# facebookresearch/videoseal

Hardware: AMD Instinct MI355X
Metric: frames/sec embed+extract 256-bit @768x768 (higher is better)
Workload: dtype f32 (2 x f16 operand split, 3 products on v_mfma_f32_32x32x16_f16, fp32 accumulate); 1 GPU; videoseal_1.0 256-bit, 32 frames 768x768 per GPU, image mode (embedder on every frame, full-res JND), embed + detect; card=videoseal_1.0, weights=random-init (seeded), no checkpoint offline, batch_per_gpu=32, mode=image

## Files before the change

### include/videoseal_hip.h

```cpp
#ifndef VIDEOSEAL_HIP_H
#define VIDEOSEAL_HIP_H

#include <stdint.h>

#ifdef __cplusplus
extern "C" {
#endif

#define VS_OK 0
#define VS_ERR_BAD_ARG (-1)
#define VS_ERR_UNSUPPORTED (-2)
#define VS_ERR_LAUNCH (-3)

#define VS_ACT_NONE 0
#define VS_ACT_RELU 1
#define VS_ACT_GELU 2
#define VS_ACT_TANH 3
#define VS_ACT_SILU 4

#define VS_PAD_ZERO 0
#define VS_PAD_REFLECT 1

#define VS_VIDEO_REPEAT 0
#define VS_VIDEO_ALTERNATE 1
// ... 112 lines not shown
int vs_vit_attention_bwd(const float* qkv, const float* out, const float* dout, int frames, int H, int W, int heads, int hd, int window,
                         const float* rel_h, const float* rel_w, float* dqkv, float* scratch, float* drel_h, float* drel_w, void* stream);
int vs_reflect_fold1(const float* dxp, int B, int H, int W, int64_t ld, float* out, void* stream);
int vs_dwconv7(const float* x, int B, int H, int W, int C, int64_t ld, const float* w, const float* bias, int flip, const float* add,
               int64_t add_ld, float* out, int64_t out_ld, void* stream);
int64_t vs_dwconv7_wgrad_partial_floats(int B, int H, int64_t ld);
int vs_dwconv7_wgrad(const float* x, int64_t ld, const float* dy, int64_t dy_ld, int B, int H, int W, int C, float* partial, float* dw,
                     void* stream);
int64_t vs_colreduce_partial_floats(int B, int64_t HW, int64_t ld);
int vs_layernorm_bwd(const float* x, int64_t ld, const float* dy, int64_t dy_ld, const float* w, int64_t rows, int C, float eps, float* dx,
                     int64_t dx_ld, float* stats, float* partial, float* dw, float* db, void* stream);
int vs_gelu_grn_bwd(const float* h1, int64_t ld, const float* d3, int64_t d3_ld, const float* gamma, int B, int HW, int C, float* partial,
                    float* coef, float* dh1, int64_t dh1_ld, float* dgamma, float* dbeta, void* stream);
int vs_patchify(const float* x, int B, int H, int W, int64_t pld, int P, float* cols, void* stream);
int vs_unpatch(const float* dcols, int B, int H, int W, int64_t pld, int P, float* dx, void* stream);
int vs_patchify_s(const float* x, int B, int H, int W, int64_t pld, int P, int S, float* cols, void* stream);
int vs_unpatch_s(const float* dcols, int B, int H, int W, int64_t pld, int P, int S, float* dx, void* stream);
int vs_col2im3x3_reflect(const float* dcols, int B, int H, int W, int64_t ld, float* dx, void* stream);
int vs_colmean(const float* x, int B, int HW, int64_t ld, float* out, void* stream);
int vs_pool_gelu_bwd(const float* z, int64_t ld, const float* dpooled, int64_t dp_ld, int B, int HW, int C, float* dz, int64_t dz_ld,
                     void* stream);
int vs_matmul_small(const float* A, int64_t lda, const float* Bm, int64_t ldb, int M, int N, int K, float* C, int64_t ldc, void* stream);
int vs_bce_logits(const float* preds, const int32_t* msgs, int msg_rows, int B, int k, float temperature, float gscale, float* dpreds,
                  float* loss, void* stream);

int vs_bn_mean_rstd(const double* sums, int C, int64_t ld, float eps, float* mean, float* rstd, void* stream);
int64_t vs_bn_bwd_partial_floats(int64_t rows, int64_t ld);
int vs_bn_relu_bwd_sums(const float* raw, int64_t ld, const float* dy, int64_t dy_ld, const float* mean, const float* rstd, const float* scale,
                        const float* shift, int relu, int64_t rows, int C, float* partial, double* sums, float* dgamma, float* dbeta,
                        void* stream);
int vs_bn_relu_bwd_apply(const float* raw, int64_t ld, const float* dy, int64_t dy_ld, const float* mean, const float* rstd, const float* scale,
                         const float* shift, int relu, const double* sums, int64_t rows, int C, float* dx, int64_t dx_ld, void* stream);
int vs_dilate2(const float* dy, int B, int Ho, int Wo, int64_t ld, int H, int W, float* out, void* stream);
int vs_im2col3x3_strided(const float* x, int B, int H, int W, int64_t ld, int stride, float* cols, void* stream);
int vs_upcat2x_bwd(const float* dhi, int64_t hi_ld, int B, int H, int W, int C1, int C2, float skip_scale, float* dx, int64_t ld1,
                   float* dskip, int64_t ld2, void* stream);
int vs_msg_table_grad(const float* dlat, const int32_t* msgs, int Bm, int nbits, int hidden, float* dtable, void* stream);
int vs_relu_bwd(const float* z, int64_t ld, const float* dy, int64_t dy_ld, int64_t rows, int C, float* dz, int64_t dz_ld, void* stream);
int vs_outc_tanh_bwd(const float* delta, const float* ddelta, int64_t rows_per_frame, int B, int C, const float* w, int Cout, int use_tanh,
                     float* dx, int64_t dx_ld, float* dv, void* stream);

typedef struct vs_resblock_thin_desc {
  const float* x; int64_t x_ld;
  int32_t B, H, W, Cin;
  const void *w0_split, *w1_split, *wr_split;
  const float *b0, *b1, *br;
  int32_t arith;
  int32_t Cout;
  float a_mul, acc_mul0, acc_mul1, acc_mulr;
  float* out; int64_t out_ld;
} vs_resblock_thin_desc_t;
int vs_resblock_thin_supported(int cin_ld, int cmid, int cout);
int vs_resblock_thin(const vs_resblock_thin_desc_t* d, void* stream);

int vs_check_finite(const float* x, int64_t n, int* flag, void* stream);

int vs_absmax(const float* x, int64_t n, unsigned* bits, void* stream);

int vs_cnx_block_supported(int C, int64_t rows, int HW);
int64_t vs_cnx_block_image_bytes(int C);
int vs_cnx_block(const void* tn_planes, const void* wimg, int C, int64_t rows, int HW, int stats, float acc_mul1, float acc_mul2, const float* scale,
                 int64_t scale_ld, const float* bias2, const float* res, int64_t res_ld, float* out, int64_t out_ld, float* part32, void* stream);

int vs_split_block(const float* wt, int N, int64_t K, int ntaps, int arith, float w_mul, void* split, void* blk, void* stream);
int vs_pack_conv(const float* w, int Co, int Ci, int KH, int KW, int cinp, int transpose, float* out, void* stream);

int vs_resize_nchw_bwd(const float* dy, float* dx, int planes, int H, int W, int oh, int ow, int antialias, float* tmp, void* stream);
int vs_embed_tail_bwd(const float* imgs, const float* preds, const float* hmap_full, const float* d_imgs_w, const float* d_preds_w, int F, int H, int W,
                      int Cd, int clamp, float scaling_i, float scaling_w, float* g_full, void* stream);
int vs_tail_key_reduce(const float* g_low, const float* hmap_low, int F, int Cd, int S_h, int S_w, int step, int video_mode, int total_key,
                       float* d_delta, void* stream);
int vs_aug_crop_flip_bwd(const float* dy, float* dx, int planes, int H, int W, int i0, int j0, int h, int w, int flip, void* stream);
int vs_mask_mul(const float* dy, const float* mask, float* dx, int F, int C, int H, int W, int complement, void* stream);
int64_t vs_aug_color_bwd_scratch_floats(int F, int H, int W);
int vs_aug_color_bwd(const float* x, const float* dy, float* dx, int F, int H, int W, int op, float factor, const float* means, float* scratch,
                     void* stream);
int vs_clamp01_bwd(const float* x, const float* dy, float* dx, int64_t n, void* stream);
int vs_aug_gather_frames_bwd(const float* dy, const int32_t* start, const int32_t* outs, float* dx, int n_src, int64_t frame_floats, void* stream);
int vs_aug_window_average_bwd(const float* dy, float* dx, int F, int64_t frame_floats, int half_window, float alpha, void* stream);
int vs_gaussian_blur_bwd(const float* dy, float* tmp, float* dx, int planes, int H, int W, int k, float sigma, void* stream);
int vs_aug_warp_bwd(const float* dy, float* dx, int planes, int H, int W, int oh, int ow, int kind, const float* coeffs, int bilinear,
                    const float* inv, void* stream);
int vs_nhwc_to_nchw_scaled(const float* src, int F, int H, int W, int C, int64_t ld, float mul, float* dst, void* stream);
int64_t vs_percep_partial_doubles(int F, int H, int W);
int vs_percep_mse(const float* imgs, const float* imgs_w, int F, int H, int W, int yuv, double* partial, float* loss, void* stream);
int vs_percep_mse_grad(const float* imgs, const float* imgs_w, int F, int H, int W, int yuv, float upstream, float* d_imgs_w, void* stream);

int64_t vs_ssim_partial_doubles(int P, int H, int W);
int vs_ssim_stats(const float* x, const float* y, int P, int H, int W, float data_range, const float* win11, double* partial, double* out, void* stream);
int vs_ssim_grad(const float* x, const float* y, const float* g_ssim, const float* g_cs, const float* g_coarse, int P, int H, int W, float data_range,
                 const float* win11, float* dy, void* stream);
int vs_avgpool2_pad(const float* x, const float* y, int P, int H, int W, float* xo, float* yo, void* stream);
int64_t vs_jnd_loss_partial_doubles(int F, int H, int W);
int vs_jnd_loss(const float* imgs, const float* imgs_w, const float* hmap, int F, int H, int W, double* partial, float* loss, void* stream);
int vs_jnd_loss_grad(const float* imgs, const float* imgs_w, const float* hmap, int F, int H, int W, float upstream, float* d_imgs_w, void* stream);

int vs_upcat2x(const float* x, int C1, int64_t ld1, const float* skip, int C2, int64_t ld2, float skip_scale,
               int B, int H, int W, float* out, int64_t out_ld, void* stream);

int vs_upconv_supported(int Co);
int vs_upconv_gather_ln(const float* z, int64_t z_ld, int B, int H, int W, int Co, const float* lnw, const float* lnb, float eps,
                        int act, float* out, int64_t out_ld, void* stream);
int vs_cat2_scale(const float* x, int C1, int64_t ld1, const float* skip, int C2, int64_t ld2, float skip_scale, int64_t rows,
                  float* out, int64_t out_ld, void* stream);

int vs_upconv_fused_supported(int C1, int C2, int Co);
// ... 92 lines not shown
```

### videoseal_amd/csrc/model_api.hip

```cpp
#include <algorithm>
#include <cmath>
#include <cstring>
#include <map>
#include <string>
#include <vector>

#include "vs_common.h"

#pragma clang fp contract(off)

namespace {

inline int rup(int v, int m) { return (v + m - 1) / m * m; }

struct HostT { const float* p; int64_t n; };

struct CW {
  float* wt = nullptr; float* bias = nullptr; void* split = nullptr; void* blk = nullptr;
  int N = 0, KH = 0, KW = 0, CinP = 0;
  float w_mul = 1.f;
};
struct RB { CW c0, c1, res; int cout = 0; };
struct Up { CW conv; CW gemm; bool lowres = false; float* lnw = nullptr; float* lnb = nullptr; RB rb; };
struct Down { float* lnw = nullptr; float* lnb = nullptr; CW conv, gemm; };
// ... 297 lines not shown
    const float am = a_mul_override > 0.f ? a_mul_override : ((a_scale && !pre_table) ? A_MUL_GRN : A_MUL);
    d.arith = m->arith; d.a_mul = am; d.acc_mul = 1.f / (am * w.w_mul);
    if (in2) { d.wt2_split = w2->split; d.wt2_blk = w2->blk; d.acc_mul2 = 1.f / (am * w2->w_mul); }
    int split_k = 1;
    const bool dense_rows = d.in_sy == (int64_t)d.W * d.in_sx && d.in_sb == (int64_t)d.H * d.in_sy;
    const bool gemm_pc = d.KH == 1 && d.KW == 1 && sh == 1 && sw == 1 && ph == 0 && pw == 0 && !in2 && d.Ho == d.H && d.Wo == d.W &&
                         d.Cin % 32 == 0 && d.CinP == d.Cin && dense_rows && (!a_scale || d.H * d.W >= 128 || d.H * d.W == 64);
    const bool patch_pc = d.KH == 3 && d.KW == 3 && sh == 1 && sw == 1 && ph == 1 && pw == 1 && d.Ho == d.H && d.Wo == d.W && !a_scale &&
                          d.W % 16 == 0 && d.H % 8 == 0;
    if (pre_table) {
      d.tile_hint = (d.N % 192 == 0 ? (VS_CONV_TILE_HI | 0) : 15) | VS_CONV_PRE;
    } else if (sumsq) {
      d.sumsq_part = sumsq;
    } else if (gemm_pc && a_scale && m->arith == 2 && d.N % 96 == 0 && d.H * d.W >= 128 && d.CinP <= 3072 &&
               (((int64_t)d.B * d.H * d.W + 127) / 128) * ((d.N + 127) / 128) < 256 && (((int64_t)d.B * d.H * d.W + 127) / 128) * ((d.N + 95) / 96) >= 200) {
      d.tile_hint = VS_CONV_TILE_HI | 10;
    } else if (gemm_pc) {
      const int64_t rows = (int64_t)d.B * d.H * d.W;
      const int64_t blocks = ((rows + 127) / 128) * ((d.N + 127) / 128);
      const int pairs = d.CinP / 32;
      int sk = 1;
      while (blocks * sk < 256 && pairs % (sk * 2) == 0 && pairs / (sk * 2) >= 4) sk *= 2;
      if (!a_scale || d.CinP / sk <= 3072) split_k = sk;
    } else if (patch_pc && d.N >= 128 && d.CinP >= 128) {
      const int64_t blocks = (int64_t)d.B * (d.H / 8) * (d.W / 16) * (d.N % 192 == 0 ? (d.N + 191) / 192 : (d.N + 127) / 128);
      const int spt = d.CinP / 16;
      const int cands[5] = {2, 3, 4, 6, 8};
      for (int cand : cands) {
        if (blocks * split_k >= 192) break;
        if (spt % cand == 0 && spt / cand >= 2) split_k = cand;
      }
    }
    if (split_k > 1) {
      const int ws_ld = rup(w.N, 4);
      const int slices = split_k + ((patch_pc && in2) ? 1 : 0);
      d.splitk_ws = alloc((int64_t)slices * out.rows() * ws_ld);
      d.splitk_ld = ws_ld;
      d.split_k = split_k;
      d.tile_hint = d.KH == 3 ? (d.N % 192 == 0 ? VS_CONV_TILE_HI | 0 : 15) : (VS_CONV_TILE_HI | (d.N % 192 == 0 ? 2 : 1));
    }
    if (grn_part) {
      const int t = (d.tile_hint & 0xf) + ((d.tile_hint & VS_CONV_TILE_HI) ? 16 : 0);
      if ((t == 17 || t == 18 || t == 26) && grn_hw % 32 == 0 && grn_hw / 32 <= 16 && d.CinP == grn_c4 && a_scale_ld == grn_c4) {
        d.grn_part = grn_part; d.grn_gamma = grn_gamma; d.grn_nchunk = grn_hw / 32;
      } else if (live()) {
        chk(vs_grn_scale_from_partials(grn_part, d.B, grn_hw, grn_c4, grn_gamma, const_cast<float*>(a_scale), a_scale_ld, st));
      }
    }
    if (live()) chk(vs_conv_gemm(&d, st));
  }
  void layernorm(const Act& x, const float* w, const float* b, const Act& out, int act_ = VS_ACT_NONE) {
    if (live()) chk(vs_layernorm_act(x.p, x.rows(), x.C, x.ld, w, b, 1e-6f, act_, out.p, out.ld, st));
  }
  Act resblock(const Act& x, const RB& p, const Act* out_in = nullptr) {
    const int tk = p.cout == 16 ? 16 : 32;
    if ((p.cout == 16 || (p.cout == 32 && m->arith == 2)) && x.ld <= tk && p.c0.CinP == tk && p.c1.CinP == tk && p.res.CinP == tk &&
        (!out_in || out_in->ld == p.cout) && vs_resblock_thin_supported(x.ld, p.cout, p.cout)) {
      Act out = out_in ? *out_in : act(x.B, x.H, x.W, p.cout);
      vs_resblock_thin_desc_t d;
      std::memset(&d, 0, sizeof(d));
      d.x = x.p; d.x_ld = x.ld; d.B = x.B; d.H = x.H; d.W = x.W; d.Cin = x.ld;
      d.w0_split = p.c0.split; d.w1_split = p.c1.split; d.wr_split = p.res.split;
      d.b0 = p.c0.bias; d.b1 = p.c1.bias; d.br = p.res.bias;
      d.arith = m->arith; d.Cout = p.cout; d.a_mul = A_MUL;
      d.acc_mul0 = 1.f / (A_MUL * p.c0.w_mul); d.acc_mul1 = 1.f / (A_MUL * p.c1.w_mul); d.acc_mulr = 1.f / (A_MUL * p.res.w_mul);
      d.out = out.p; d.out_ld = out.ld;
      if (live()) chk(vs_resblock_thin(&d, st));
      return out;
    }
    Act t = act(x.B, x.H, x.W, p.cout);
    conv(x, p.c0, t, 1, 1, VS_PAD_ZERO, VS_ACT_RELU);
    Act out = out_in ? *out_in : act(x.B, x.H, x.W, p.cout);
    conv(t, p.c1, out, 1, 1, VS_PAD_ZERO, VS_ACT_RELU, 0, out.ld != rup(p.cout, 4) ? p.cout : -1, nullptr, &x, &p.res);
    return out;
  }
  void gemm_pl(int B, int H, int W, const CW& w, const void* in_pl, const Act& out, int act_, const Act* res, float* sumsq, int split_k,
               float am = A_MUL, int sumsq_hw = 0) {
    vs_conv_desc_t d;
    std::memset(&d, 0, sizeof(d));
    d.B = B; d.H = H; d.W = W; d.Cin = w.CinP; d.KH = d.KW = 1; d.SH = d.SW = 1; d.Ho = H; d.Wo = W;
    d.wt = w.wt; d.CinP = w.CinP; d.N = w.N; d.bias = w.bias; d.act = act_;
    d.wt_split = w.split; d.wt_blk = w.blk; d.arith = 2; d.a_mul = am; d.acc_mul = 1.f / (am * w.w_mul);
    d.in_pl = in_pl;
    d.out = out.p; d.out_ld = out.ld; d.n_store = out.ld;
    if (res) { d.res = res->p; d.res_ld = res->ld; }
    d.sumsq_part = sumsq;
    d.sumsq_hw = sumsq_hw;
    if (split_k > 1) {
      const int ws_ld = rup(w.N, 4);
      d.splitk_ws = alloc((int64_t)split_k * out.rows() * ws_ld);
      d.splitk_ld = ws_ld;
      d.split_k = split_k;
    }
    d.tile_hint = VS_CONV_TILE_HI | 8;
    if (live()) chk(vs_conv_gemm(&d, st));
  }
  void conv_pl(int B, int H, int W, const CW& w, const void* in_pl, void* out_pl, const Act* out, const CW* w2 = nullptr,
               const void* in2_pl = nullptr, const float* pre_table = nullptr, int64_t pre_ld = 0) {
    vs_conv_desc_t d;
    std::memset(&d, 0, sizeof(d));
    d.B = B; d.H = H; d.W = W; d.Cin = w.CinP; d.KH = d.KW = 3; d.SH = d.SW = 1; d.PH = d.PW = 1; d.pad_mode = VS_PAD_ZERO; d.Ho = H; d.Wo = W;
    d.wt = w.wt; d.CinP = w.CinP; d.N = w.N; d.bias = w.bias; d.act = VS_ACT_RELU;
    d.wt_split = w.split; d.wt_blk = w.blk; d.arith = 2; d.a_mul = A_MUL; d.acc_mul = 1.f / (A_MUL * w.w_mul);
    d.in_pl = in_pl; d.out_pl = out_pl;
    if (w2) {
      d.in2_pl = in2_pl; d.Cin2 = d.Cin2P = w2->CinP; d.wt2 = w2->wt; d.bias2 = w2->bias; d.wt2_split = w2->split; d.wt2_blk = w2->blk;
      d.acc_mul2 = 1.f / (A_MUL * w2->w_mul);
    }
    d.n_store = w.N;
    if (out) { d.out = out->p; d.out_ld = out->ld; d.n_store = out->ld != rup(w.N, 4) ? w.N : out->ld; }
    d.tile_hint = VS_CONV_TILE_HI | 6;
    if (pre_table) { d.a_scale = pre_table; d.a_scale_ld = pre_ld; d.tile_hint |= VS_CONV_PRE; }
    if (live()) chk(vs_conv_gemm(&d, st));
  }
  Act bottleneck_planes(const Act& x, int j0, const Act* last_out, void* xpl_in = nullptr) {
    const int B = x.B, H = x.H, W = x.W, C = x.C;
    const int64_t pl_floats = x.rows() * C;
    void* xpl = xpl_in ? xpl_in : alloc(pl_floats);
// ... 81 lines not shown
            chk(vs_to_planes(h3.p, h3.rows(), h3.C, h3.ld, A_MUL, h3pl, st));
          }
          conv_pl(B, h3.H, h3.W, m->b0_lat, latpl, tpl, nullptr, nullptr, nullptr, table, n_msgs == 1 ? 0 : 9 * (int64_t)N);
          conv_pl(B, h3.H, h3.W, rb.c1, tpl, xpl, nullptr, &rb.res, h3pl);
          cur = nxt;
          cur_pl = xpl;
          continue;
        }
        Act t = act(B, h3.H, h3.W, N);
        conv(h3, m->b0_lat, t, 1, 1, VS_PAD_ZERO, VS_ACT_RELU, 0, -1, nullptr, nullptr, nullptr, table, n_msgs == 1 ? 0 : 9 * (int64_t)N, nullptr,
             nullptr, nullptr, m->zc.back(), true);
        Act out = act(B, h3.H, h3.W, N);
        conv(t, rb.c1, out, 1, 1, VS_PAD_ZERO, VS_ACT_RELU, 0, -1, nullptr, &h3, &rb.res);
        cur = out;
        continue;
      }
      if (j >= 1 && planes_ok(cur, j)) {
        Act v2 = view;
        const bool d2 = j == c.num_blocks - 1 ? direct : lowres_cat(0, cur, v2);
        cur = bottleneck_planes(cur, j, d2 ? &v2 : nullptr, cur_pl);
        break;
      }
      cur = resblock(cur, rb, direct ? &view : nullptr);
    }
    for (int k = 0; k < nlev; ++k) {
      const Act skip = hid.back();
      hid.pop_back();
      const Up& up = m->ups[k];
      Act ln{};
      if (up.lowres && cur.ld == cur.C && fused_ok(k, cur.C, skip.C)) {
        const int co = up.gemm.N / 9;
        ln = act(B, 2 * cur.H, 2 * cur.W, co);
        if (live()) chk(vs_upconv_fused(cur.p, cur.C, cur.ld, skip.p, skip.C, skip.ld, 0.70710678118654752440f, up.gemm.split, B, cur.H, cur.W, co,
                                        up.lnw, up.lnb, 1e-6f, VS_ACT_RELU, ln.p, ln.ld, m->arith, A_MUL, 1.f / (A_MUL * up.gemm.w_mul), st));
      } else if (up.lowres) {
        const int co = up.gemm.N / 9;
        const bool direct = cur.ld == cur.C + skip.C;
        Act lc = direct ? Act{cur.p, B, cur.H, cur.W, cur.C + skip.C, cur.ld} : act(B, cur.H, cur.W, cur.C + skip.C);
        if (live()) chk(vs_cat2_scale(direct ? nullptr : cur.p, cur.C, cur.ld, skip.p, skip.C, skip.ld, 0.70710678118654752440f, lc.rows(), lc.p, lc.ld, st));
        Act z = act(B, lc.H, lc.W, 9 * co);
        conv(lc, up.gemm, z);
        ln = act(B, 2 * lc.H, 2 * lc.W, co);
        if (live()) chk(vs_upconv_gather_ln(z.p, z.ld, B, lc.H, lc.W, co, up.lnw, up.lnb, 1e-6f, VS_ACT_RELU, ln.p, ln.ld, st));
      } else {
        Act cat = act(B, 2 * cur.H, 2 * cur.W, cur.C + skip.C);
        if (live()) chk(vs_upcat2x(cur.p, cur.C, cur.ld, skip.p, skip.C, skip.ld, 0.70710678118654752440f, B, cur.H, cur.W, cat.p, cat.ld, st));
        Act cv = act(B, cat.H, cat.W, up.conv.N);
        conv(cat, up.conv, cv, 1, 1, VS_PAD_REFLECT);
        ln = act(B, cat.H, cat.W, up.conv.N);
        layernorm(cv, up.lnw, up.lnb, ln, VS_ACT_RELU);
      }
      Act view{};
      const bool direct = lowres_cat(k + 1, Act{nullptr, B, ln.H, ln.W, up.rb.cout, 0}, view);
      cur = resblock(ln, up.rb, direct ? &view : nullptr);
    }
    float* delta = alloc((int64_t)B * c.out_ch * cur.H * cur.W);
    if (live()) chk(vs_outc_tanh(cur.p, (int64_t)cur.H * cur.W, B, cur.C, cur.ld, m->outc_w, m->outc_b, c.out_ch, c.last_tanh ? 1 : 0, delta, st));
    Sh = cur.H; Sw = cur.W;
    return delta;
  }
  void extractor(const Act& x, float* logits) {
    const vs_model_cfg_t& c = m->c;
    const int B = x.B, s = c.stem_stride;
    int Ho = (x.H - 4) / s + 1, Wo = (x.W - 4) / s + 1;
    Act cur = act(B, Ho, Wo, c.dims[0], xld(c.dims[0]));
    const int co = c.dims[0];
    static const bool stem_fused = [] { const char* e = getenv("VIDEOSEAL_STEM_FUSED"); return e && e[0] == '1'; }();
    if (stem_fused && x.ld == 4 && cur.ld == co && (co == 64 || co == 96 || co == 128) && m->stem.bias) {
      if (live()) chk(vs_stem_conv_ln(x.p, B, x.H, x.W, s, m->stem.wt, m->stem.bias, m->stem_lnw, m->stem_lnb, 1e-6f, co, cur.p, cur.ld, st));
    } else {
      Act t = act(B, Ho, Wo, c.dims[0]);
      { const int geom[7] = {Wo, s * 4, 16, s, 1, 0, 0}; conv(x, m->stem, t, 1, 0, VS_PAD_ZERO, VS_ACT_NONE, 0, -1, nullptr, nullptr, nullptr, nullptr, 0, nullptr, geom); }
      layernorm(t, m->stem_lnw, m->stem_lnb, cur);
    }
    for (int sti = 0; sti < 4; ++sti) {
      if (sti > 0) {
        const Down& dn = m->down[sti - 1];
        Ho = cur.H / 2; Wo = cur.W / 2;
        if (cur.ld == cur.C && cur.C % 8 == 0 && dn.gemm.CinP == 4 * cur.C && Ho > 0 && Wo > 0) {
          Act lnp = act(B, Ho, Wo, 4 * cur.C, 4 * cur.C);
          Act nxt = act(B, Ho, Wo, c.dims[sti], xld(c.dims[sti]));
          if (live()) chk(vs_layernorm_patch2x2(cur.p, B, cur.H, cur.W, cur.C, cur.ld, dn.lnw, dn.lnb, 1e-6f, lnp.p, st));
          conv(lnp, dn.gemm, nxt);
          cur = nxt;
        } else {
          Act ln = act(B, cur.H, cur.W, cur.C, cur.ld);
          layernorm(cur, dn.lnw, dn.lnb, ln);
          Act nxt = act(B, Ho, Wo, c.dims[sti], xld(c.dims[sti]));
          const int geom[7] = {Wo, 2 * ln.ld, 2 * ln.ld, 2, 1, 0, 0};
          conv(ln, dn.conv, nxt, 1, 0, VS_PAD_ZERO, VS_ACT_NONE, 0, -1, nullptr, nullptr, nullptr, nullptr, 0, nullptr, geom);
          cur = nxt;
        }
      }
      const int Cc = c.dims[sti], HW = cur.H * cur.W;
      Act tn = act(B, cur.H, cur.W, Cc, xld(Cc));
      Act hh = act(B, cur.H, cur.W, 4 * Cc, xld(4 * Cc));
      float* part = alloc((int64_t)((HW + 63) / 64) * B * 4 * Cc);
      float* part32 = alloc((int64_t)B * ((HW + 31) / 32) * 4 * Cc);
      float* scale = alloc((int64_t)B * hh.ld + 16);
      float* parts = (HW % 32 != 0 && HW >= 32) ? alloc((((int64_t)B * HW + 31) / 32) * 2 * 4 * Cc) : nullptr;
      const int64_t rows = cur.rows();
      const CW& pw1w = m->stages[sti].empty() ? m->stem : m->stages[sti][0].pw1;
      const bool pl1 = m->arith == 2 && ((rows + 255) / 256) * ((4 * Cc + 191) / 192) >= 200 && pw1w.CinP % 16 == 0 && !m->stages[sti].empty();
      bool pl2 = false;
      int sk2 = 1;
      if (m->arith == 2 && hh.ld >= 2048 && hh.ld % 16 == 0) {
// ... 258 lines not shown
```

### videoseal_amd/csrc/net_ops.hip

```cpp
#include <algorithm>
#include <cstdlib>
#include <cstring>

#include "conv_common.h"

namespace {

__global__ __launch_bounds__(256) void layernorm_act_kernel(const float* __restrict__ x, int64_t rows, int C, int64_t ld,
                                                            const float* __restrict__ w, const float* __restrict__ b,
                                                            float eps, int act, float* __restrict__ out, int64_t out_ld) {
  const int lane = threadIdx.x & 63;
  const int64_t row = (int64_t)blockIdx.x * 4 + (threadIdx.x >> 6);
  if (row >= rows) return;
  const float* xr = x + row * ld;
  float s = 0.f;
  for (int c = lane; c < C; c += 64) s += xr[c];
  const float mean = wave_sum(s) / (float)C;
  float v = 0.f;
  for (int c = lane; c < C; c += 64) {
    const float dlt = xr[c] - mean;
    v += dlt * dlt;
  }
  const float var = wave_sum(v) / (float)C;
  const float den = sqrtf(var + eps);
  float* orow = out + row * out_ld;
  for (int c = lane; c < (int)out_ld; c += 64) {
    float y = 0.f;
    if (c < C) y = vs_apply_act(w[c] * ((xr[c] - mean) / den) + b[c], act);
    orow[c] = y;
  }
}

template <int LPP, int VMAX>
__global__ __launch_bounds__(256) void layernorm_act_lanes_kernel(const float* __restrict__ x, int64_t rows, int C, int64_t ld,
                                                                  const float* __restrict__ w, const float* __restrict__ b, float eps, int act,
                                                                  float* __restrict__ out, int64_t out_ld, int pH, int pW) {
  constexpr int RPB = 256 / LPP;
  const int q = threadIdx.x & (LPP - 1);
  const int64_t row = (int64_t)blockIdx.x * RPB + (threadIdx.x / LPP);
  bool live = row < rows;
  const int C4 = (C + 3) >> 2, O4 = (int)(out_ld >> 2);
  const float* xr = x + (live ? row : rows - 1) * ld;
  f32x4 v[VMAX];
  float s = 0.f;
#pragma unroll
  for (int k = 0; k < VMAX; ++k) {
    const int c4 = q + k * LPP;
    v[k] = f32x4{0.f, 0.f, 0.f, 0.f};
    if (c4 < C4) {
      v[k] = *reinterpret_cast<const f32x4*>(xr + 4 * c4);
#pragma unroll
      for (int e = 0; e < 4; ++e)
        if (4 * c4 + e < C) s += v[k][e];
    }
  }
#pragma unroll
  for (int o = LPP / 2; o > 0; o >>= 1) s += __shfl_xor(s, o, 64);
// ... 484 lines not shown
          scale[(int64_t)b * sld + c] = gx;
          local += gx;
        }
      }
    }
    __syncthreads();
  }
  if (kg == 0) red[cl] = local;
  __syncthreads();
  for (int o = 128; o > 0; o >>= 1) {
    if (threadIdx.x < o) red[threadIdx.x] += red[threadIdx.x + o];
    __syncthreads();
  }
  const float mean = red[0] / (float)C;
  for (int c = threadIdx.x; c < (int)sld; c += 1024) {
    float v = 0.f;
    if (c < C) v = 1.0f + gamma[c] * (scale[(int64_t)b * sld + c] / (mean + 1e-6f));
    scale[(int64_t)b * sld + c] = v;
  }
}

__global__ __launch_bounds__(256) void upcat2x_kernel(const float* __restrict__ x, int C1, int64_t ld1,
                                                      const float* __restrict__ skip, int C2, int64_t ld2, float sscale,
                                                      int B, int H, int W, float* __restrict__ out, int64_t old, int64_t total) {
  const int G = (int)(old >> 2);
  for (int64_t i = (int64_t)blockIdx.x * 256 + threadIdx.x; i < total; i += (int64_t)gridDim.x * 256) {
    const int cg = (int)(i % G);
    int64_t p = i / G;
    const int X = (int)(p % (2 * W)); p /= (2 * W);
    const int Y = (int)(p % (2 * H));
    const int b = (int)(p / (2 * H));
    const int c = cg * 4;
    float sy = fmaxf((Y + 0.5f) * 0.5f - 0.5f, 0.f), sx = fmaxf((X + 0.5f) * 0.5f - 0.5f, 0.f);
    const int y0 = (int)sy, x0 = (int)sx;
    const int y1 = y0 + (y0 < H - 1), x1 = x0 + (x0 < W - 1);
    const float ly1 = sy - y0, lx1 = sx - x0, ly0 = 1.f - ly1, lx0 = 1.f - lx1;
    const float* src; int64_t ld; int cc; float mul;
    if (c < C1) { src = x; ld = ld1; cc = c; mul = 1.f; }
    else { src = skip; ld = ld2; cc = c - C1; mul = sscale; }
    f32x4 v = {0.f, 0.f, 0.f, 0.f};
    if (c < C1 + C2) {
      const float* fb = src + (int64_t)b * H * W * ld + cc;
      const f32x4 p00 = *reinterpret_cast<const f32x4*>(fb + ((int64_t)y0 * W + x0) * ld);
      const f32x4 p01 = *reinterpret_cast<const f32x4*>(fb + ((int64_t)y0 * W + x1) * ld);
      const f32x4 p10 = *reinterpret_cast<const f32x4*>(fb + ((int64_t)y1 * W + x0) * ld);
      const f32x4 p11 = *reinterpret_cast<const f32x4*>(fb + ((int64_t)y1 * W + x1) * ld);
      v = (ly0 * (lx0 * (p00 * mul) + lx1 * (p01 * mul)) + ly1 * (lx0 * (p10 * mul) + lx1 * (p11 * mul)));
    }
    *reinterpret_cast<f32x4*>(out + (((int64_t)b * 2 * H + Y) * 2 * W + X) * old + c) = v;
  }
}

template <int CG>
__global__ __launch_bounds__(256) void upconv_gather_ln_kernel(const float* __restrict__ z, int64_t zld, int H, int W, int Co,
                                                               int tpp_log2, const float* __restrict__ lnw,
                                                               const float* __restrict__ lnb, float eps, int act,
                                                               float* __restrict__ out, int64_t old, int64_t npix, int nblk) {
  const int per = (nblk + 7) >> 3;
  const int64_t vb = (int64_t)(blockIdx.x & 7) * per + (blockIdx.x >> 3);
  const int64_t gid = vb * 256 + threadIdx.x;
  const int64_t pq = gid >> tpp_log2;
  const int g = (int)(gid & ((1 << tpp_log2) - 1));
  const bool live = pq < npix && vb < nblk;
  const int64_t p = live ? pq : 0;
  constexpr int NVP = CG / 4;
  f32x4 lwv[NVP], lbv[NVP];
#pragma unroll
  for (int j = 0; j < NVP; ++j) {
    lwv[j] = *reinterpret_cast<const f32x4*>(lnw + g * CG + 4 * j);
    lbv[j] = *reinterpret_cast<const f32x4*>(lnb + g * CG + 4 * j);
  }
  const int W2 = 2 * W, H2 = 2 * H;
  const int X = (int)(p % W2);
  const int64_t t0 = p / W2;
  const int Y = (int)(t0 % H2);
  const int64_t b = t0 / H2;
  int ys[3][2], xs[3][2];
  float wy[3][2], wx[3][2];
#pragma unroll
  for (int k = 0; k < 3; ++k) {
    int yr = Y + k - 1, xr = X + k - 1;
    yr = yr < 0 ? -yr : (yr >= H2 ? 2 * H2 - 2 - yr : yr);
    xr = xr < 0 ? -xr : (xr >= W2 ? 2 * W2 - 2 - xr : xr);
    const float sy = fmaxf((yr + 0.5f) * 0.5f - 0.5f, 0.f), sx = fmaxf((xr + 0.5f) * 0.5f - 0.5f, 0.f);
    const int y0 = (int)sy, x0 = (int)sx;
    ys[k][0] = y0; ys[k][1] = y0 + (y0 < H - 1);
    xs[k][0] = x0; xs[k][1] = x0 + (x0 < W - 1);
    wy[k][1] = sy - y0; wy[k][0] = 1.f - wy[k][1];
    wx[k][1] = sx - x0; wx[k][0] = 1.f - wx[k][1];
  }
  constexpr int NV = CG / 4;
  f32x4 acc[NV];
#pragma unroll
  for (int j = 0; j < NV; ++j) acc[j] = f32x4{0.f, 0.f, 0.f, 0.f};
  const float* zb = z + b * H * W * zld + g * CG;
#pragma unroll
  for (int ky = 0; ky < 3; ++ky)
#pragma unroll
    for (int a = 0; a < 2; ++a) {
      const float* zr = zb + (int64_t)ys[ky][a] * W * zld + ky * 3 * Co;
#pragma unroll
      for (int kx = 0; kx < 3; ++kx)
#pragma unroll
        for (int c = 0; c < 2; ++c) {
          const float w = wy[ky][a] * wx[kx][c];
          const float* q = zr + (int64_t)xs[kx][c] * zld + kx * Co;
#pragma unroll
          for (int j = 0; j < NV; ++j) acc[j] += w * *reinterpret_cast<const f32x4*>(q + 4 * j);
        }
    }
  float s = 0.f;
#pragma unroll
  for (int j = 0; j < NV; ++j) s += (acc[j][0] + acc[j][1]) + (acc[j][2] + acc[j][3]);
  for (int o = 1; o < (1 << tpp_log2); o <<= 1) s += __shfl_xor(s, o, 64);
  const float mean = s / (float)Co;
  float v = 0.f;
#pragma unroll
  for (int j = 0; j < NV; ++j)
#pragma unroll
    for (int e = 0; e < 4; ++e) { const float dl = acc[j][e] - mean; v += dl * dl; }
  for (int o = 1; o < (1 << tpp_log2); o <<= 1) v += __shfl_xor(v, o, 64);
  const float den = sqrtf(v / (float)Co + eps);
  if (!live) return;
  float* orow = out + p * old + g * CG;
#pragma unroll
  for (int j = 0; j < NV; ++j) {
    const f32x4 wv = lwv[j], bv = lbv[j];
    f32x4 o;
#pragma unroll
    for (int e = 0; e < 4; ++e) o[e] = vs_apply_act(wv[e] * ((acc[j][e] - mean) / den) + bv[e], act);
    *reinterpret_cast<f32x4*>(orow + 4 * j) = o;
  }
}

__global__ __launch_bounds__(256) void im2col3x3_kernel(const float* __restrict__ x, int H, int W, int64_t ld, int reflect,
                                                        float* __restrict__ out, int64_t total) {
  const int G = (int)(ld >> 2);
  for (int64_t i = (int64_t)blockIdx.x * 256 + threadIdx.x; i < total; i += (int64_t)gridDim.x * 256) {
    const int cg = (int)(i % G);
    int64_t r = i / G;
    const int t = (int)(r % 9);
    r /= 9;
    const int xx = (int)(r % W);
    const int yy = (int)((r / W) % H);
    const int64_t b = r / ((int64_t)W * H);
    int sy = yy + t / 3 - 1, sx = xx + t % 3 - 1;
    bool ok = true;
    if (reflect) {
      sy = sy < 0 ? -sy : (sy >= H ? 2 * H - 2 - sy : sy);
      sx = sx < 0 ? -sx : (sx >= W ? 2 * W - 2 - sx : sx);
    } else {
      ok = sy >= 0 && sy < H && sx >= 0 && sx < W;
    }
    f32x4 v = {0.f, 0.f, 0.f, 0.f};
    if (ok) v = *reinterpret_cast<const f32x4*>(x + ((b * H + sy) * W + sx) * ld + cg * 4);
    *reinterpret_cast<f32x4*>(out + (r * 9 + t) * ld + cg * 4) = v;
  }
}

__global__ __launch_bounds__(256) void msg_pre_kernel(const float* __restrict__ P, int N, float* __restrict__ T, int64_t total) {
  for (int64_t i = (int64_t)blockIdx.x * 256 + threadIdx.x; i < total; i += (int64_t)gridDim.x * 256) {
    const int n = (int)(i % N);
    const int cls = (int)((i / N) % 9);
    const int64_t bm = i / ((int64_t)9 * N);
    const int cy = cls / 3, cx = cls % 3;
    const float* pb = P + bm * 9 * N + n;
    float v = 0.f;
    for (int ky = (cy == 0 ? 1 : 0); ky <= (cy == 2 ? 1 : 2); ++ky)
      for (int kx = (cx == 0 ? 1 : 0); kx <= (cx == 2 ? 1 : 2); ++kx) v += pb[(ky * 3 + kx) * N];
    T[i] = v;
  }
}

__global__ __launch_bounds__(256) void cat2_scale_kernel(const float* __restrict__ x, int C1, int64_t ld1, const float* __restrict__ skip,
                                                         int C2, int64_t ld2, float s, int64_t rows, float* __restrict__ out,
                                                         int64_t old) {
  const int g1 = x ? C1 >> 2 : 0, G = g1 + (C2 >> 2);
  const int64_t total = rows * G;
  for (int64_t i = (int64_t)blockIdx.x * 256 + threadIdx.x; i < total; i += (int64_t)gridDim.x * 256) {
    const int cg = (int)(i % G);
    const int64_t r = i / G;
    f32x4 v;
    int c;
    if (cg < g1) { c = cg * 4; v = *reinterpret_cast<const f32x4*>(x + r * ld1 + c); }
    else { const int c2 = (cg - g1) * 4; c = C1 + c2; v = *reinterpret_cast<const f32x4*>(skip + r * ld2 + c2) * s; }
// ... 1 lines not shown
  }
}

__global__ __launch_bounds__(256) void msg_latent_kernel(const float* __restrict__ table, const int32_t* __restrict__ msgs,
                                                         int nbits, int hidden, float* __restrict__ lat) {
  __shared__ int rowsel[1024];
  const int b = blockIdx.y;
  for (int k = threadIdx.x; k < nbits; k += 256) rowsel[k] = 2 * k + (msgs[(int64_t)b * nbits + k] != 0);
  __syncthreads();
  const int c = blockIdx.x * 256 + threadIdx.x;
  if (c >= hidden) return;
  float s = 0.f;
  int k = 0;
  for (; k + 16 <= nbits; k += 16) {
    float v[16];
#pragma unroll
    for (int j = 0; j < 16; ++j) v[j] = table[(int64_t)rowsel[k + j] * hidden + c];
#pragma unroll
    for (int j = 0; j < 16; ++j) s += v[j];
  }
  for (; k < nbits; ++k) s += table[(int64_t)rowsel[k] * hidden + c];
  lat[(int64_t)b * hidden + c] = s;
}
__global__ __launch_bounds__(256) void broadcast_channels4_kernel(const float* __restrict__ lat, int Bm, int hidden4,
                                                                  float* __restrict__ dst, int HW, int64_t ld, int coff,
                                                                  int64_t total4) {
  for (int64_t i = (int64_t)blockIdx.x * 256 + threadIdx.x; i < total4; i += (int64_t)gridDim.x * 256) {
    const int c4 = (int)(i % hidden4);
    const int64_t p = i / hidden4;
    const int b = (int)(p / HW);
    *reinterpret_cast<f32x4*>(dst + p * ld + coff + 4 * c4) = *reinterpret_cast<const f32x4*>(lat + ((int64_t)(Bm == 1 ? 0 : b) * hidden4 + c4) * 4);
  }
}
__global__ __launch_bounds__(256) void broadcast_channels_kernel(const float* __restrict__ lat, int Bm, int hidden,
                                                                 float* __restrict__ dst, int HW, int64_t ld, int coff,
                                                                 int64_t total) {
  for (int64_t i = (int64_t)blockIdx.x * 256 + threadIdx.x; i < total; i += (int64_t)gridDim.x * 256) {
    const int c = (int)(i % hidden);
    const int64_t p = i / hidden;
    const int b = (int)(p / HW);
    dst[p * ld + coff + c] = lat[(int64_t)(Bm == 1 ? 0 : b) * hidden + c];
  }
}

__global__ __launch_bounds__(256) void outc_tanh_kernel(const float* __restrict__ x, int64_t rpf, int64_t rows, int C,
                                                        int64_t ld, const float* __restrict__ w, const float* __restrict__ bias,
                                                        int Cout, int use_tanh, float* __restrict__ out) {
  const int64_t row = (int64_t)blockIdx.x * 256 + threadIdx.x;
  if (row >= rows) return;
  float acc[4] = {0.f, 0.f, 0.f, 0.f};
  const float* xr = x + row * ld;
  for (int c = 0; c < C; c += 4) {
    const f32x4 v = *reinterpret_cast<const f32x4*>(xr + c);
    for (int o = 0; o < Cout; ++o) {
      const float* wr = w + (int64_t)o * C + c;
      acc[o] += v[0] * wr[0];
      if (c + 1 < C) acc[o] += v[1] * wr[1];
      if (c + 2 < C) acc[o] += v[2] * wr[2];
      if (c + 3 < C) acc[o] += v[3] * wr[3];
    }
  }
  const int64_t b = row / rpf, p = row - b * rpf;
  for (int o = 0; o < Cout; ++o) {
    float v = acc[o] + bias[o];
    out[(b * Cout + o) * rpf + p] = use_tanh ? tanhf(v) : v;
  }
}

__global__ __launch_bounds__(256) void pool_linear_kernel(const float* __restrict__ x, int HW, int C, int64_t ld,
                                                          const float* __restrict__ w, const float* __restrict__ bias, int N,
                                                          float* __restrict__ out) {
  extern __shared__ float pooled[];
  const int b = blockIdx.x;
  const float* xb = x + (int64_t)b * HW * ld;
  const int C4 = (C + 3) >> 2;
  const bool vec = (ld & 3) == 0 && (reinterpret_cast<uintptr_t>(x) & 15) == 0;
  if (vec) {
    for (int g = threadIdx.x; g < C4; g += 256) {
      f32x4 s = {0.f, 0.f, 0.f, 0.f};
      const float* xg = xb + 4 * g;
      int r = 0;
      for (; r + 16 <= HW; r += 16) {
        f32x4 v[16];
#pragma unroll
        for (int q = 0; q < 16; ++q) v[q] = *reinterpret_cast<const f32x4*>(xg + (int64_t)(r + q) * ld);
#pragma unroll
        for (int q = 0; q < 16; ++q) s += v[q];
      }
      for (; r < HW; ++r) s += *reinterpret_cast<const f32x4*>(xg + (int64_t)r * ld);
#pragma unroll
      for (int e = 0; e < 4; ++e)
        if (4 * g + e < C) pooled[4 * g + e] = s[e] / (float)HW;
    }
  } else {
    for (int c = threadIdx.x; c < C; c += 256) {
      float s = 0.f;
      for (int r = 0; r < HW; ++r) s += xb[(int64_t)r * ld + c];
      pooled[c] = s / (float)HW;
    }
  }
  __syncthreads();
  const int lane = threadIdx.x & 63, wv = threadIdx.x >> 6;
  constexpr int CM = 16;
  for (int n = blockIdx.y * 4 + wv; n < N; n += 4 * gridDim.y) {
    const float* wr = w + (int64_t)n * C;
    float s = 0.f;
    if (C <= 64 * CM) {
      float wv_[CM];
#pragma unroll
      for (int j = 0; j < CM; ++j) {
        const int c = lane + 64 * j;
        wv_[j] = c < C ? wr[c] : 0.f;
      }
#pragma unroll
      for (int j = 0; j < CM; ++j) {
        const int c = lane + 64 * j;
        if (c < C) s += pooled[c] * wv_[j];
      }
    } else {
// ... 454 lines not shown
  return vs_launch_status();
}

extern "C" int vs_upcat2x(const float* x, int C1, int64_t ld1, const float* skip, int C2, int64_t ld2, float skip_scale,
                          int B, int H, int W, float* out, int64_t out_ld, void* stream) {
  VS_REQUIRE(x && skip && out && C1 > 0 && C2 > 0 && C1 % 4 == 0 && C2 % 4 == 0 && ld1 % 4 == 0 && ld2 % 4 == 0);
  VS_REQUIRE(out_ld % 4 == 0 && out_ld >= C1 + C2 && B > 0 && H > 0 && W > 0);
  const int64_t total = (int64_t)B * 2 * H * 2 * W * (out_ld / 4);
  hipLaunchKernelGGL(upcat2x_kernel, dim3(grid_for(total, 256, 1 << 20)), dim3(256), 0, (hipStream_t)stream, x, C1, ld1, skip,
                     C2, ld2, skip_scale, B, H, W, out, out_ld, total);
  return vs_launch_status();
}

extern "C" int vs_cat2_scale(const float* x, int C1, int64_t ld1, const float* skip, int C2, int64_t ld2, float skip_scale,
                             int64_t rows, float* out, int64_t out_ld, void* stream) {
  VS_REQUIRE(skip && out && rows > 0 && C1 >= 0 && C2 > 0 && C1 % 4 == 0 && C2 % 4 == 0 && ld2 % 4 == 0 && out_ld % 4 == 0 &&
             out_ld >= C1 + C2 && (!x || (ld1 % 4 == 0 && ld1 >= C1)));
  const int64_t total = rows * ((x ? C1 : 0) + C2) / 4;
  hipLaunchKernelGGL(cat2_scale_kernel, dim3((unsigned)std::min<int64_t>(cdiv64(total, 256), 1 << 16)), dim3(256), 0, (hipStream_t)stream,
                     x, C1, ld1, skip, C2, ld2, skip_scale, rows, out, out_ld);
  return vs_launch_status();
}

extern "C" int vs_im2col3x3(const float* x, int B, int H, int W, int64_t ld, int pad_mode, float* out, void* stream) {
  VS_REQUIRE(x && out && B > 0 && H > 1 && W > 1 && ld > 0 && ld % 4 == 0);
  const int64_t total = (int64_t)B * H * W * 9 * (ld / 4);
  hipLaunchKernelGGL(im2col3x3_kernel, dim3((unsigned)std::min<int64_t>(cdiv64(total, 256), 1 << 16)), dim3(256), 0, (hipStream_t)stream, x, H,
                     W, ld, pad_mode == VS_PAD_REFLECT ? 1 : 0, out, total);
  return vs_launch_status();
}

extern "C" int vs_msg_pre(const float* P, int Bm, int N, float* table, void* stream) {
  VS_REQUIRE(P && table && Bm > 0 && N > 0);
  const int64_t total = (int64_t)Bm * 9 * N;
  hipLaunchKernelGGL(msg_pre_kernel, dim3((unsigned)std::min<int64_t>(cdiv64(total, 256), 1 << 16)), dim3(256), 0, (hipStream_t)stream, P, N, table,
                     total);
  return vs_launch_status();
}

extern "C" int vs_upconv_supported(int Co) {
  if (Co < 16 || Co % 16) return 0;
  const int cg = Co >= 64 ? 16 : Co / 4;
  const int tpp = Co / cg;
  return (cg == 4 || cg == 8 || cg == 16) && tpp <= 64 && (tpp & (tpp - 1)) == 0;
}

extern "C" int vs_upconv_gather_ln(const float* z, int64_t z_ld, int B, int H, int W, int Co, const float* lnw, const float* lnb,
                                   float eps, int act, float* out, int64_t out_ld, void* stream) {
  VS_REQUIRE(z && lnw && lnb && out && B > 0 && H > 0 && W > 0 && vs_upconv_supported(Co) && z_ld >= 9 * (int64_t)Co && z_ld % 4 == 0 &&
             out_ld >= Co && out_ld % 4 == 0);
  const int cg = Co >= 64 ? 16 : Co / 4;
  int tl = 0;
  while ((cg << tl) < Co) ++tl;
  const int64_t npix = (int64_t)B * 4 * H * W;
  const int64_t nblk64 = cdiv64(npix << tl, 256);
  VS_REQUIRE(nblk64 < (1 << 30));
  const int nblk = (int)nblk64;
  const int grid = ((nblk + 7) / 8) * 8;
  hipStream_t st = (hipStream_t)stream;
#define VS_UPG(CG_) hipLaunchKernelGGL(upconv_gather_ln_kernel<CG_>, dim3(grid), dim3(256), 0, st, z, z_ld, H, W, Co, tl, lnw, lnb, eps, act, out, out_ld, npix, nblk)
  if (cg == 4) VS_UPG(4);
  else if (cg == 8) VS_UPG(8);
  else VS_UPG(16);
#undef VS_UPG
  return vs_launch_status();
}

extern "C" int vs_msg_latent(const float* table, const int32_t* msgs, int Bm, int nbits, int hidden, float* lat, void* stream) {
  VS_REQUIRE(table && msgs && lat && Bm > 0 && nbits > 0 && nbits <= 1024 && hidden > 0);
  hipLaunchKernelGGL(msg_latent_kernel, dim3((unsigned)((hidden + 255) / 256), (unsigned)Bm), dim3(256), 0, (hipStream_t)stream,
                     table, msgs, nbits, hidden, lat);
  return vs_launch_status();
}

extern "C" int vs_broadcast_channels(const float* lat, int Bm, int hidden, float* dst, int B, int HW, int64_t ld, int coff,
                                     void* stream) {
  VS_REQUIRE(lat && dst && (Bm == 1 || Bm == B) && hidden > 0 && B > 0 && HW > 0 && coff >= 0 && coff + hidden <= ld);
  const int64_t total = (int64_t)B * HW * hidden;
  if ((hidden & 3) == 0 && (ld & 3) == 0 && (coff & 3) == 0 && (((uintptr_t)lat | (uintptr_t)dst) & 15) == 0) {
    hipLaunchKernelGGL(broadcast_channels4_kernel, dim3(grid_for(total / 4, 256, 1 << 20)), dim3(256), 0, (hipStream_t)stream, lat, Bm,
                       hidden / 4, dst, HW, ld, coff, total / 4);
    return vs_launch_status();
  }
  hipLaunchKernelGGL(broadcast_channels_kernel, dim3(grid_for(total, 256, 1 << 20)), dim3(256), 0, (hipStream_t)stream, lat, Bm,
                     hidden, dst, HW, ld, coff, total);
  return vs_launch_status();
}

extern "C" int vs_outc_tanh(const float* x, int64_t rows_per_frame, int B, int C, int64_t ld, const float* w, const float* bias,
                            int Cout, int use_tanh, float* out, void* stream) {
  VS_REQUIRE(x && w && bias && out && rows_per_frame > 0 && B > 0 && C > 0 && ld % 4 == 0 && ld >= C && Cout > 0 && Cout <= 4);
  const int64_t rows = rows_per_frame * B;
  hipLaunchKernelGGL(outc_tanh_kernel, dim3((unsigned)cdiv64(rows, 256)), dim3(256), 0, (hipStream_t)stream, x, rows_per_frame,
                     rows, C, ld, w, bias, Cout, use_tanh, out);
  return vs_launch_status();
}

extern "C" int vs_pool_linear(const float* x, int B, int HW, int C, int64_t ld, const float* w, const float* bias, int N,
                              float* out, void* stream) {
  VS_REQUIRE(x && w && bias && out && B > 0 && HW > 0 && C > 0 && ld >= C && N > 0);
  const size_t smem = (size_t)C * sizeof(float);
  if (smem > 64 * 1024) return VS_ERR_UNSUPPORTED;
  hipLaunchKernelGGL(pool_linear_kernel, dim3((unsigned)B, 16), dim3(256), smem, (hipStream_t)stream, x, HW, C, ld, w, bias, N, out);
  return vs_launch_status();
}

extern "C" int64_t vs_bn_partial_doubles(int64_t rows, int64_t ld) { return ld >= 4 ? cdiv64(rows, bn_chunk_rows(ld)) * 2 * ld : 0; }

extern "C" int vs_bn_batch_stats(const float* x, int64_t rows, int C, int64_t ld, const float* gamma, const float* beta, float eps,
                                 float momentum, float* running_mean, float* running_var, double* partial, float* scale, float* shift,
                                 void* stream) {
  VS_REQUIRE(x && gamma && beta && partial && scale && shift && rows > 0 && C > 0 && ld >= C && (ld & 3) == 0);
// ... 50 lines not shown
```

### videoseal_amd/csrc/resblock_thin.hip

```cpp
#include "conv_common.h"

namespace {

using namespace vsconv;

constexpr int TH = 8, TW = 16;
constexpr int T_W = TW + 2, T_H = TH + 2, T_PX = T_W * T_H;
constexpr int X_W = TW + 4, X_H = TH + 4, X_PX = X_W * X_H;
constexpr int XITEMS = X_PX * 4;
constexpr int NXI = (XITEMS + 255) / 256;
constexpr int G0_PER_WAVE = 3;
constexpr int G1_PER_WAVE = 2;
constexpr int ROWB16 = 32;

template <int NP> struct Arith16;
template <> struct Arith16<3> {
  static __device__ __forceinline__ f32x4 mfma(const bf16x8& a, const bf16x8& b, const f32x4& c) {
    return __builtin_amdgcn_mfma_f32_16x16x32_bf16(a, b, c, 0, 0, 0);
  }
};
template <> struct Arith16<2> {
  static __device__ __forceinline__ f32x4 mfma(const bf16x8& a, const bf16x8& b, const f32x4& c) {
    return __builtin_amdgcn_mfma_f32_16x16x32_f16(__builtin_bit_cast(f16x8, a), __builtin_bit_cast(f16x8, b), c, 0, 0, 0);
  }
};

struct RbArgs {
  const float* x; int64_t x_sb, x_sy, x_sx; int B, H, W, Cin;
  const void *w0, *w1, *wr;
  const float *b0, *b1, *br;
  float a_mul, acc_mul0, acc_mul1, acc_mulr;
  float* out; int64_t out_ld;
};

__device__ __forceinline__ bf16x8 zero_frag() {
  const u32x4 z = {0u, 0u, 0u, 0u};
  return __builtin_bit_cast(bf16x8, z);
}

template <int NP, int NBUF, int OCC>
__global__ __launch_bounds__(256, OCC) void resblock_thin_kernel(const RbArgs d, const int tiles_x, const int tiles_y, const int ntiles_total,
                                                                 const int tiles_per_wg) {
  using AR = Arith<NP>;
  using A16 = Arith16<NP>;
  constexpr int XP_BYTES = NP * X_PX * ROWB16;
  constexpr int TT_BYTES = NP * T_PX * ROWB16;
  __shared__ __attribute__((aligned(16))) unsigned char smem[NBUF * XP_BYTES + TT_BYTES];
  unsigned char* const Tt = smem + NBUF * XP_BYTES;
  const int tid = threadIdx.x;
  const int lane = tid & 63;
  const int wave = tid >> 6;
  const int n = lane & 15, kb = lane >> 4;
  const int hi = kb >> 1;
  const int kh = (kb & 1) * 8;

  bf16x8 w0f[5][NP], w1f[5][NP], wrf[NP];
#pragma unroll
  for (int s = 0; s < 5; ++s) {
    const int tap = 2 * s + hi;
#pragma unroll
    for (int p = 0; p < NP; ++p) {
      if (tap < 9) {
        w0f[s][p] = *reinterpret_cast<const bf16x8*>(static_cast<const char*>(d.w0) + ((int64_t)p * 16 * 144 + n * 144 + tap * 16 + kh) * 2);
        w1f[s][p] = *reinterpret_cast<const bf16x8*>(static_cast<const char*>(d.w1) + ((int64_t)p * 16 * 144 + n * 144 + tap * 16 + kh) * 2);
      } else {
        w0f[s][p] = zero_frag();
        w1f[s][p] = zero_frag();
      }
    }
  }
#pragma unroll
  for (int p = 0; p < NP; ++p)
    wrf[p] = hi == 0 ? *reinterpret_cast<const bf16x8*>(static_cast<const char*>(d.wr) + ((int64_t)p * 16 * 16 + n * 16 + kh) * 2) : zero_frag();
  float b0v[4], b1v[4], brv[4];
#pragma unroll
  for (int e = 0; e < 4; ++e) {
    b0v[e] = d.b0 ? d.b0[4 * kb + e] : 0.f;
    b1v[e] = d.b1 ? d.b1[4 * kb + e] : 0.f;
    brv[e] = d.br ? d.br[4 * kb + e] : 0.f;
  }

  int p_dy[NXI], p_dx[NXI], p_lds[NXI];
  bool p_have[NXI];
  const int k4 = (tid & 3) * 4;
  const bool cok = k4 < d.Cin;
#pragma unroll
  for (int i = 0; i < NXI; ++i) {
    const int item = tid + i * 256;
    p_have[i] = item < XITEMS;
    const int prow = p_have[i] ? item >> 2 : 0;
    p_dy[i] = prow / X_W - 2;
    p_dx[i] = prow % X_W - 2;
    p_lds[i] = prow * ROWB16 + k4 * 2;
  }
  int toffx[5], tofft[5];
#pragma unroll
  for (int s5 = 0; s5 < 5; ++s5) {
    const int tap = 2 * s5 + hi < 9 ? 2 * s5 + hi : 8;
    toffx[s5] = ((tap / 3) * X_W + tap % 3) * ROWB16;
    tofft[s5] = ((tap / 3) * T_W + tap % 3) * ROWB16;
  }
  int a0[G0_PER_WAVE], t_i[G0_PER_WAVE];
#pragma unroll
  for (int gi = 0; gi < G0_PER_WAVE; ++gi) {
    int i = 16 * (wave * G0_PER_WAVE + gi) + n;
    t_i[gi] = i;
    i = i < T_PX ? i : T_PX - 1;
    a0[gi] = ((i / T_W) * X_W + (i % T_W)) * ROWB16 + kh * 2;
  }
  int a1[G1_PER_WAVE], ar[G1_PER_WAVE];
#pragma unroll
  for (int gi = 0; gi < G1_PER_WAVE; ++gi) {
    const int row = wave * G1_PER_WAVE + gi;
    a1[gi] = (row * T_W + n) * ROWB16 + kh * 2;
    ar[gi] = ((row + 2) * X_W + (n + 2)) * ROWB16 + kh * 2;
  }
  const float amul = NP == 2 ? d.a_mul : 1.f;
  const float am0 = NP == 2 ? d.acc_mul0 : 1.f, am1 = NP == 2 ? d.acc_mul1 : 1.f, amr = NP == 2 ? d.acc_mulr : 1.f;

  f32x4 rp[NXI];
  auto load_tile = [&](const int fb, const int y0, const int x0) __attribute__((always_inline)) {
#pragma unroll
    for (int i = 0; i < NXI; ++i) {
      const int iy = y0 + p_dy[i], ix = x0 + p_dx[i];
      const bool ok = p_have[i] && cok && iy >= 0 && iy < d.H && ix >= 0 && ix < d.W;
      const int cy = iy < 0 ? 0 : (iy >= d.H ? d.H - 1 : iy), cx = ix < 0 ? 0 : (ix >= d.W ? d.W - 1 : ix);
      const f32x4 v = *reinterpret_cast<const f32x4*>(d.x + (int64_t)fb * d.x_sb + (int64_t)cy * d.x_sy + (int64_t)cx * d.x_sx + (cok ? k4 : 0));
      rp[i] = ok ? v : f32x4{0.f, 0.f, 0.f, 0.f};
    }
  };
  auto store_tile = [&](const int buf) __attribute__((always_inline)) {
    unsigned char* Ps = smem + buf * XP_BYTES;
#pragma unroll
    for (int i = 0; i < NXI; ++i)
      if (p_have[i]) {
        u32x2 pl[NP];
        split4n<NP>(rp[i], amul, pl);
#pragma unroll
        for (int p = 0; p < NP; ++p) *reinterpret_cast<u32x2*>(Ps + p * X_PX * ROWB16 + p_lds[i]) = pl[p];
      }
  };

  const int t_begin = blockIdx.x * tiles_per_wg;
  const int t_end = min(ntiles_total, t_begin + tiles_per_wg);
  if (t_begin >= t_end) return;
  int tx = t_begin % tiles_x, ty = (t_begin / tiles_x) % tiles_y, fb = t_begin / (tiles_x * tiles_y);
  load_tile(fb, ty * TH, tx * TW);
  store_tile(0);
  __syncthreads();
  for (int t = t_begin; t < t_end; ++t) {
    const int buf = NBUF == 2 ? (t - t_begin) & 1 : 0;
    int ntx = tx + 1, nty = ty, nfb = fb;
    if (ntx == tiles_x) { ntx = 0; if (++nty == tiles_y) { nty = 0; ++nfb; } }
    {
      const bool more = t + 1 < t_end;
      load_tile(more ? nfb : fb, (more ? nty : ty) * TH, (more ? ntx : tx) * TW);
    }
    const unsigned char* Ps = smem + buf * XP_BYTES;
    const int y0 = ty * TH, x0 = tx * TW;

#pragma unroll
    for (int gi = 0; gi < G0_PER_WAVE; ++gi) {
      f32x4 acc = {0.f, 0.f, 0.f, 0.f};
#pragma unroll
      for (int s = 0; s < 5; ++s) {
        const int off = a0[gi] + toffx[s];
        bf16x8 xf[NP];
#pragma unroll
        for (int p = 0; p < NP; ++p) xf[p] = *reinterpret_cast<const bf16x8*>(Ps + p * X_PX * ROWB16 + off);
#pragma unroll
        for (int q = 0; q < AR::NPROD; ++q) acc = A16::mfma(w0f[s][AR::PB[q]], xf[AR::PA[q]], acc);
      }
      const int i = t_i[gi];
      if (i < T_PX) {
        const int gy = y0 - 1 + i / T_W, gx = x0 - 1 + i % T_W;
        const bool in = gy >= 0 && gy < d.H && gx >= 0 && gx < d.W;
        f32x4 v;
#pragma unroll
        for (int e = 0; e < 4; ++e) {
          const float a = NP == 2 ? acc[e] * am0 : acc[e];
          v[e] = in ? vs_relu(a + b0v[e]) : 0.f;
        }
        u32x2 pl[NP];
        split4n<NP>(v, amul, pl);
#pragma unroll
        for (int p = 0; p < NP; ++p) *reinterpret_cast<u32x2*>(Tt + p * T_PX * ROWB16 + i * ROWB16 + 8 * kb) = pl[p];
      }
    }
    if (NBUF == 2 && t + 1 < t_end) store_tile(buf ^ 1);
    __syncthreads();

#pragma unroll
    for (int gi = 0; gi < G1_PER_WAVE; ++gi) {
      f32x4 acc = {0.f, 0.f, 0.f, 0.f}, accr = {0.f, 0.f, 0.f, 0.f};
#pragma unroll
      for (int s = 0; s < 5; ++s) {
        const int off = a1[gi] + tofft[s];
        bf16x8 tf[NP];
#pragma unroll
        for (int p = 0; p < NP; ++p) tf[p] = *reinterpret_cast<const bf16x8*>(Tt + p * T_PX * ROWB16 + off);
#pragma unroll
        for (int q = 0; q < AR::NPROD; ++q) acc = A16::mfma(w1f[s][AR::PB[q]], tf[AR::PA[q]], acc);
      }
      {
        bf16x8 xf[NP];
#pragma unroll
        for (int p = 0; p < NP; ++p) xf[p] = *reinterpret_cast<const bf16x8*>(Ps + p * X_PX * ROWB16 + ar[gi]);
#pragma unroll
        for (int q = 0; q < AR::NPROD; ++q) accr = A16::mfma(wrf[AR::PB[q]], xf[AR::PA[q]], accr);
      }
      const int y = y0 + wave * G1_PER_WAVE + gi, x = x0 + n;
      if (y < d.H && x < d.W) {
        f32x4 v;
#pragma unroll
        for (int e = 0; e < 4; ++e) {
          const float a = NP == 2 ? acc[e] * am1 : acc[e];
          const float r = NP == 2 ? accr[e] * amr : accr[e];
          v[e] = vs_relu(a + b1v[e]) + (r + brv[e]);
        }
        *reinterpret_cast<f32x4*>(d.out + (((int64_t)fb * d.H + y) * d.W + x) * d.out_ld + 4 * kb) = v;
      }
    }
    if (NBUF == 1) {
      __syncthreads();
      if (t + 1 < t_end) store_tile(0);
    }
    __syncthreads();
    tx = ntx; ty = nty; fb = nfb;
  }
}

constexpr int ROWB32 = 96;
constexpr int NW32 = 8, NT32 = NW32 * 64;
constexpr int XITEMS32 = X_PX * 8;
constexpr int NXI32 = (XITEMS32 + NT32 - 1) / NT32;
constexpr int G0N = (12 + NW32 - 1) / NW32, G1N = 8 / NW32;
constexpr int XP32_BYTES = 2 * X_PX * ROWB32, TT32_BYTES = 2 * T_PX * ROWB32;
constexpr int W32_CONV = 9 * 2 * 2 * 16 * 64, W32_RES = 2 * 2 * 16 * 64;

__global__ __launch_bounds__(NT32) void resblock_thin32_kernel(const RbArgs d, const int tiles_x, const int tiles_y, const int ntiles_total,
                                                               const int tiles_per_wg) {
  using AR = Arith<2>;
  using A16 = Arith16<2>;
  __shared__ __attribute__((aligned(16))) unsigned char smem[XP32_BYTES + TT32_BYTES + 2 * W32_CONV + W32_RES];
  unsigned char* const Ps = smem;
  unsigned char* const Tt = smem + XP32_BYTES;
  unsigned char* const Wl = Tt + TT32_BYTES;
  const int tid = threadIdx.x;
  const int lane = tid & 63;
  const int wave = __builtin_amdgcn_readfirstlane(tid >> 6);
  const int n = lane & 15, kb = lane >> 4;

  for (int u = tid; u < 2 * 2304; u += NT32) {
    const int conv = u / 2304, r = u - conv * 2304;
    const int tap = r >> 8, r2 = r & 255;
    const int half = r2 >> 7, plane = (r2 >> 6) & 1, nn = (r2 >> 2) & 15, kbu = r2 & 3;
    const char* src = static_cast<const char*>(conv ? d.w1 : d.w0) + ((int64_t)(plane * 32 + half * 16 + nn) * 288 + tap * 32 + kbu * 8) * 2;
    unsigned char* dst = Wl + conv * W32_CONV + ((((tap * 2 + half) * 2 + plane) * 16 + nn) * 64) + ((kbu ^ ((nn >> 3) << 1)) * 16);
    *reinterpret_cast<u32x4*>(dst) = *reinterpret_cast<const u32x4*>(src);
  }
  if (tid < 256) {
    const int u = tid;
    const int half = u >> 7, plane = (u >> 6) & 1, nn = (u >> 2) & 15, kbu = u & 3;
    const char* src = static_cast<const char*>(d.wr) + ((int64_t)(plane * 32 + half * 16 + nn) * 32 + kbu * 8) * 2;
    *reinterpret_cast<u32x4*>(Wl + 2 * W32_CONV + (((half * 2 + plane) * 16 + nn) * 64) + ((kbu ^ ((nn >> 3) << 1)) * 16)) = *reinterpret_cast<const u32x4*>(src);
  }
  const int aw = n * 64 + ((kb ^ ((n >> 3) << 1)) * 16);
  float b0v[2][4], b1v[2][4], brv[2][4];
#pragma unroll
  for (int h = 0; h < 2; ++h)
#pragma unroll
    for (int e = 0; e < 4; ++e) {
      const int c = h * 16 + 4 * kb + e;
      b0v[h][e] = d.b0 ? d.b0[c] : 0.f;
      b1v[h][e] = d.b1 ? d.b1[c] : 0.f;
      brv[h][e] = d.br ? d.br[c] : 0.f;
    }

  const int k4 = (tid & 7) * 4;
  const bool cok = k4 < d.Cin;
  int p_dy[NXI32], p_dx[NXI32], p_lds[NXI32];
  bool p_have[NXI32];
// ... 119 lines not shown
        bf16x8 tf[2];
#pragma unroll
        for (int p = 0; p < 2; ++p) tf[p] = *reinterpret_cast<const bf16x8*>(Tt + p * T_PX * ROWB32 + a1 + toff);
#pragma unroll
        for (int h = 0; h < 2; ++h) {
          bf16x8 wf[2];
#pragma unroll
          for (int p = 0; p < 2; ++p) wf[p] = *reinterpret_cast<const bf16x8*>(Wl + W32_CONV + ((tap * 2 + h) * 2 + p) * 1024 + aw);
#pragma unroll
          for (int q = 0; q < AR::NPROD; ++q) acc[h] = A16::mfma(wf[AR::PB[q]], tf[AR::PA[q]], acc[h]);
        }
      }
      {
        bf16x8 xf[2];
#pragma unroll
        for (int p = 0; p < 2; ++p) xf[p] = *reinterpret_cast<const bf16x8*>(Ps + p * X_PX * ROWB32 + ar);
#pragma unroll
        for (int h = 0; h < 2; ++h) {
          bf16x8 wf[2];
#pragma unroll
          for (int p = 0; p < 2; ++p) wf[p] = *reinterpret_cast<const bf16x8*>(Wl + 2 * W32_CONV + (h * 2 + p) * 1024 + aw);
#pragma unroll
          for (int q = 0; q < AR::NPROD; ++q) accr[h] = A16::mfma(wf[AR::PB[q]], xf[AR::PA[q]], accr[h]);
        }
      }
#pragma unroll
      for (int h = 0; h < 2; ++h)
#pragma unroll
        for (int e = 0; e < 4; ++e) outv[h][e] = vs_relu(acc[h][e] * am1 + b1v[h][e]) + (accr[h][e] * amr + brv[h][e]);
    }
    __syncthreads();
    if (t + 1 < t_end) store_tile();
    __syncthreads();
    {
      const int y = y0 + row1, x = x0 + n;
      if (y < d.H && x < d.W) {
        float* orow = d.out + (((int64_t)fb * d.H + y) * d.W + x) * d.out_ld;
#pragma unroll
        for (int h = 0; h < 2; ++h) *reinterpret_cast<f32x4*>(orow + h * 16 + 4 * kb) = outv[h];
      }
    }
    tx = ntx; ty = nty; fb = nfb;
  }
}

}

extern "C" int vs_resblock_thin_supported(int cin_ld, int cmid, int cout) {
  if (cin_ld < 4 || (cin_ld & 3)) return 0;
  if (cmid == 32 && cout == 32 && cin_ld <= 32) return vs_max_lds_bytes() >= (int)(XP32_BYTES + TT32_BYTES + 2 * W32_CONV + W32_RES) ? 1 : 0;
  return (cmid == 16 && cout == 16 && cin_ld <= 16) ? 1 : 0;
}

extern "C" int vs_resblock_thin(const vs_resblock_thin_desc_t* d, void* stream) {
  VS_REQUIRE(d && d->x && d->out && d->w0_split && d->w1_split && d->wr_split && d->B > 0 && d->H > 0 && d->W > 0);
  const int C = d->Cout == 32 ? 32 : 16;
  VS_REQUIRE(d->Cout == 0 || d->Cout == 16 || d->Cout == 32);
  VS_REQUIRE(vs_resblock_thin_supported(d->Cin, C, C) && d->x_ld >= d->Cin && (d->x_ld & 3) == 0 && d->out_ld >= C && (d->out_ld & 3) == 0);
  VS_REQUIRE(d->arith == 2 || (d->arith == 3 && C == 16));
  VS_REQUIRE((((uintptr_t)d->x | (uintptr_t)d->out | (uintptr_t)d->w0_split | (uintptr_t)d->w1_split | (uintptr_t)d->wr_split) & 15) == 0);
  RbArgs a{d->x, (int64_t)d->H * d->W * d->x_ld, (int64_t)d->W * d->x_ld, d->x_ld, d->B, d->H, d->W, d->Cin,
           d->w0_split, d->w1_split, d->wr_split, d->b0, d->b1, d->br, d->a_mul, d->acc_mul0, d->acc_mul1, d->acc_mulr, d->out, d->out_ld};
  const int tiles_x = (d->W + TW - 1) / TW, tiles_y = (d->H + TH - 1) / TH;
  const int64_t nt = (int64_t)d->B * tiles_x * tiles_y;
  if (nt > 0x7fffffffLL) return VS_ERR_UNSUPPORTED;
  const int64_t want = (int64_t)vs_num_cus() * (C == 32 ? 1 : 2);
  const int per = (int)((nt + want - 1) / want);
  const int tpw = per < 1 ? 1 : per;
  const unsigned grid = (unsigned)((nt + tpw - 1) / tpw);
  if (C == 32) hipLaunchKernelGGL(resblock_thin32_kernel, dim3(grid), dim3(NT32), 0, (hipStream_t)stream, a, tiles_x, tiles_y, (int)nt, tpw);
  else if (d->arith == 2) hipLaunchKernelGGL((resblock_thin_kernel<2, 2, 2>), dim3(grid), dim3(256), 0, (hipStream_t)stream, a, tiles_x, tiles_y, (int)nt, tpw);
  else hipLaunchKernelGGL((resblock_thin_kernel<3, 1, 2>), dim3(grid), dim3(256), 0, (hipStream_t)stream, a, tiles_x, tiles_y, (int)nt, tpw);
  return vs_launch_status();
}
```

### videoseal_amd/csrc/upconv_fused.hip

```cpp
#include <algorithm>
#include <cstdlib>

#include "conv_common.h"

namespace {

using namespace vsconv;

constexpr int UT = 8;
constexpr int UH = UT + 2;
constexpr int UROWS = 128;

template <int NB, int CG, int NP>
__global__ __launch_bounds__(256, (NB <= 5 ? 2 : 1)) void upconv_fused_kernel(const float* __restrict__ x, int C1, int64_t ld1, const float* __restrict__ skip,
                                                           int C2, int64_t ld2, float sscale, const unsigned short* __restrict__ wsplit,
                                                           int H, int W, int Co, const float* __restrict__ lnw,
                                                           const float* __restrict__ lnb, float eps, int act, float* __restrict__ out,
                                                           int64_t old, int tiles_x, int tiles_y, int nblk, int abl, float a_mul, float acc_mul) {
  using AR = Arith<NP>;
  constexpr int BN = NB * 32;
  constexpr int A_BYTES = NP * UROWS * ROWB;
  extern __shared__ __attribute__((aligned(16))) unsigned char smem_u[];
  unsigned char* const As = smem_u;
  unsigned char* const Bs = smem_u + A_BYTES;
  float* const Z = reinterpret_cast<float*>(smem_u);
  const int N = 9 * Co, K = C1 + C2, ZS = N + 4;
  const int tid = threadIdx.x, lane = tid & 63, wave = tid >> 6;
  const int r = lane & 31, g = lane >> 5;
  const int per = (nblk + 7) >> 3;
  const int vb = (blockIdx.x & 7) * per + (blockIdx.x >> 3);
  if (vb >= nblk) return;
  const int tx = vb % tiles_x;
  const int t1 = vb / tiles_x;
  const int ty = t1 % tiles_y;
  const int b = t1 / tiles_y;
  const int y0 = ty * UT - 1, x0 = tx * UT - 1;

  int64_t a_pix[2];
  int a_lds[2];
#pragma unroll
  for (int i = 0; i < 2; ++i) {
    const int s = tid + i * 256;
    const int row = s >> 2;
    const int hy = row < UH * UH ? row / UH : 0, hx = row < UH * UH ? row % UH : 0;
    const int py = min(max(y0 + hy, 0), H - 1), px = min(max(x0 + hx, 0), W - 1);
    a_pix[i] = ((int64_t)b * H + py) * W + px;
    a_lds[i] = row * ROWB + (s & 3) * 8;
  }
  const int k4 = (tid & 3) * 4;
  constexpr int BSLOT = BN * 2;
  constexpr int NBL = (BSLOT + 255) / 256;

  f32x16 acc[NB];
#pragma unroll
  for (int j = 0; j < NB; ++j)
#pragma unroll
    for (int e = 0; e < 16; ++e) acc[j][e] = 0.f;

  constexpr int KG = NB <= 5 ? 4 : 8;
  u32x4 rb[NBL][NP];
  auto fetch_b = [&](const int kc) __attribute__((always_inline)) {
#pragma unroll
    for (int i = 0; i < NBL; ++i) {
      const int s = tid + i * 256;
      const int row = s >> 1, sub = s & 1;
#pragma unroll
      for (int p = 0; p < NP; ++p) {
        rb[i][p] = u32x4{0u, 0u, 0u, 0u};
        if (s < BSLOT && row < N) rb[i][p] = *reinterpret_cast<const u32x4*>(wsplit + ((int64_t)p * N + row) * K + kc + sub * 8);
      }
    }
// ... 21 lines not shown
        for (int i = 0; i < 2; ++i) {
          u32x2 pl[NP];
          split4n<NP>(ra[c][i], a_mul, pl);
#pragma unroll
          for (int p = 0; p < NP; ++p) *reinterpret_cast<u32x2*>(As + p * UROWS * ROWB + a_lds[i]) = pl[p];
        }
#pragma unroll
        for (int i = 0; i < NBL; ++i) {
          const int s = tid + i * 256;
          if (s < BSLOT) {
#pragma unroll
            for (int p = 0; p < NP; ++p) *reinterpret_cast<u32x4*>(Bs + p * BN * ROWB + (s >> 1) * ROWB + (s & 1) * 16) = rb[i][p];
          }
        }
        __syncthreads();
        if (kc + BK < K) fetch_b(kc + BK);
        bf16x8 af[NP], bf[NB][NP];
#pragma unroll
        for (int p = 0; p < NP; ++p) af[p] = *reinterpret_cast<const bf16x8*>(As + p * UROWS * ROWB + (wave * 32 + r) * ROWB + g * 16);
#pragma unroll
        for (int j = 0; j < NB; ++j)
#pragma unroll
          for (int p = 0; p < NP; ++p) bf[j][p] = *reinterpret_cast<const bf16x8*>(Bs + p * BN * ROWB + (j * 32 + r) * ROWB + g * 16);
#pragma unroll
        for (int q = 0; q < AR::NPROD; ++q) {
#pragma unroll
          for (int j = 0; j < NB; ++j) acc[j] = AR::mfma(af[AR::PA[q]], bf[j][AR::PB[q]], acc[j]);
        }
      }
    }
  }
  __syncthreads();
#pragma unroll
  for (int j = 0; j < NB; ++j) {
    const int n = j * 32 + r;
#pragma unroll
    for (int e = 0; e < 16; ++e) {
      const int m = wave * 32 + (e & 3) + 8 * (e >> 2) + 4 * g;
      if (m < UH * UH && n < N) Z[m * ZS + n] = NP == 2 ? acc[j][e] * acc_mul : acc[j][e];
    }
  }
  __syncthreads();

  constexpr int NV = CG / 4;
  const int q4 = tid & 3;
  f32x4 lwv[NV], lbv[NV];
#pragma unroll
  for (int j = 0; j < NV; ++j) {
    lwv[j] = *reinterpret_cast<const f32x4*>(lnw + q4 * CG + 4 * j);
    lbv[j] = *reinterpret_cast<const f32x4*>(lnb + q4 * CG + 4 * j);
  }
  const int H2 = 2 * H, W2 = 2 * W;
  const float invC = 1.0f / (float)Co;
  for (int it = tid >> 2; it < ((abl & 2) ? 0 : 4 * UT * UT); it += 64) {
    const int oy = it / (2 * UT), ox = it % (2 * UT);
    const int Y = (y0 + 1) * 2 + oy, X = (x0 + 1) * 2 + ox;
    const bool live = Y < H2 && X < W2;
    const int Yc = min(Y, H2 - 1), Xc = min(X, W2 - 1);
    int ys[3][2], xs[3][2];
    float wy[3][2], wx[3][2];
#pragma unroll
    for (int k = 0; k < 3; ++k) {
      int yr = Yc + k - 1, xr = Xc + k - 1;
      yr = yr < 0 ? -yr : (yr >= H2 ? 2 * H2 - 2 - yr : yr);
      xr = xr < 0 ? -xr : (xr >= W2 ? 2 * W2 - 2 - xr : xr);
      const float sy = fmaxf((yr + 0.5f) * 0.5f - 0.5f, 0.f), sx = fmaxf((xr + 0.5f) * 0.5f - 0.5f, 0.f);
      const int yl = (int)sy, xl = (int)sx;
      ys[k][0] = yl - y0; ys[k][1] = yl + (yl < H - 1) - y0;
      xs[k][0] = xl - x0; xs[k][1] = xl + (xl < W - 1) - x0;
      wy[k][1] = sy - yl; wy[k][0] = 1.f - wy[k][1];
      wx[k][1] = sx - xl; wx[k][0] = 1.f - wx[k][1];
    }
    f32x4 v[NV];
#pragma unroll
    for (int j = 0; j < NV; ++j) v[j] = f32x4{0.f, 0.f, 0.f, 0.f};
    const float* zb = Z + q4 * CG;
#pragma unroll
    for (int ky = 0; ky < 3; ++ky)
#pragma unroll
      for (int a = 0; a < 2; ++a) {
        const float* zr = zb + ys[ky][a] * UH * ZS + ky * 3 * Co;
#pragma unroll
        for (int kx = 0; kx < 3; ++kx)
#pragma unroll
          for (int c = 0; c < 2; ++c) {
            const float w = wy[ky][a] * wx[kx][c];
            const float* qz = zr + xs[kx][c] * ZS + kx * Co;
#pragma unroll
            for (int j = 0; j < NV; ++j) v[j] += w * *reinterpret_cast<const f32x4*>(qz + 4 * j);
          }
      }
    float s = 0.f;
#pragma unroll
    for (int j = 0; j < NV; ++j) s += (v[j][0] + v[j][1]) + (v[j][2] + v[j][3]);
    s += __shfl_xor(s, 1, 64);
    s += __shfl_xor(s, 2, 64);
    const float mean = s * invC;
    float var = 0.f;
#pragma unroll
    for (int j = 0; j < NV; ++j)
#pragma unroll
      for (int e = 0; e < 4; ++e) { const float dl = v[j][e] - mean; var += dl * dl; }
    var += __shfl_xor(var, 1, 64);
    var += __shfl_xor(var, 2, 64);
    const float den = sqrtf(var * invC + eps);
    if (!live) continue;
    float* orow = out + (((int64_t)b * H2 + Y) * W2 + X) * old + q4 * CG;
#pragma unroll
    for (int j = 0; j < NV; ++j) {
      const f32x4 wv = lwv[j], bv = lbv[j];
      f32x4 o;
#pragma unroll
      for (int e = 0; e < 4; ++e) o[e] = vs_apply_act(wv[e] * ((v[j][e] - mean) / den) + bv[e], act);
      *reinterpret_cast<f32x4*>(orow + 4 * j) = o;
    }
  }
}

template <int NB, int CG>
int launch_fused(const float* x, int C1, int64_t ld1, const float* skip, int C2, int64_t ld2, float s, const void* wsplit, int B, int H, int W,
                 int Co, const float* lnw, const float* lnb, float eps, int act, float* out, int64_t old, int arith, float a_mul, float acc_mul,
                 hipStream_t st) {
  const size_t stage = 3 * (size_t)(UROWS + NB * 32) * ROWB, ztile = (size_t)UH * UH * (9 * Co + 4) * sizeof(float);
  const size_t smem = std::max(stage, ztile);
  if (smem > 160 * 1024) return VS_ERR_UNSUPPORTED;
  auto kern = arith == 2 ? upconv_fused_kernel<NB, CG, 2> : upconv_fused_kernel<NB, CG, 3>;
  static bool attr[2] = {false, false};
  if (smem > 64 * 1024 && !attr[arith == 2]) {
    (void)hipFuncSetAttribute((const void*)kern, hipFuncAttributeMaxDynamicSharedMemorySize, 160 * 1024);
    attr[arith == 2] = true;
  }
  const int tiles_x = (W + UT - 1) / UT, tiles_y = (H + UT - 1) / UT;
  const int64_t nblk = (int64_t)B * tiles_x * tiles_y;
  if (nblk >= (1 << 30)) return VS_ERR_UNSUPPORTED;
  static const int abl = [] { const char* e = getenv("VS_UPCONV_ABL"); return e ? atoi(e) : 0; }();
  hipLaunchKernelGGL(kern, dim3((unsigned)((nblk + 7) / 8 * 8)), dim3(256), smem, st, x, C1, ld1, skip, C2, ld2, s,
                     static_cast<const unsigned short*>(wsplit), H, W, Co, lnw, lnb, eps, act, out, old, tiles_x, tiles_y, (int)nblk, abl, a_mul, acc_mul);
  return vs_launch_status();
}

}

extern "C" int vs_upconv_fused_supported(int C1, int C2, int Co) {
  return (Co == 16 || Co == 32) && C1 > 0 && C2 > 0 && C1 % 16 == 0 && C2 % 16 == 0 && C1 + C2 <= 256;
}
extern "C" int vs_upconv_fused_preferred(int C1, int C2, int Co) { return vs_upconv_fused_supported(C1, C2, Co) && Co == 16; }

extern "C" int vs_upconv_fused(const float* x, int C1, int64_t ld1, const float* skip, int C2, int64_t ld2, float skip_scale,
                               const void* wt_split, int B, int H, int W, int Co, const float* lnw, const float* lnb, float eps, int act,
                               float* out, int64_t out_ld, int arith, float a_mul, float acc_mul, void* stream) {
  VS_REQUIRE((arith == 0 || arith == 3) || (arith == 2 && a_mul > 0.f && acc_mul > 0.f));
  VS_REQUIRE(x && skip && wt_split && lnw && lnb && out && B > 0 && H > 0 && W > 0 && vs_upconv_fused_supported(C1, C2, Co));
  VS_REQUIRE(ld1 % 4 == 0 && ld2 % 4 == 0 && ld1 >= C1 && ld2 >= C2 && out_ld % 4 == 0 && out_ld >= Co && ((uintptr_t)wt_split & 15) == 0);
  hipStream_t st = (hipStream_t)stream;
  if (Co == 16) return launch_fused<5, 4>(x, C1, ld1, skip, C2, ld2, skip_scale, wt_split, B, H, W, Co, lnw, lnb, eps, act, out, out_ld, arith, a_mul, acc_mul, st);
  return launch_fused<9, 8>(x, C1, ld1, skip, C2, ld2, skip_scale, wt_split, B, H, W, Co, lnw, lnb, eps, act, out, out_ld, arith, a_mul, acc_mul, st);
}
```

### videoseal_amd/csrc/vs_common.h

```cpp
#pragma once
#include <hip/hip_runtime.h>
#include <stdint.h>
#include <stdlib.h>
#include <string.h>

#include "videoseal_hip.h"

typedef float f32x4 __attribute__((ext_vector_type(4)));
typedef float f32x16 __attribute__((ext_vector_type(16)));

#define VS_REQUIRE(cond)                  \
  do {                                    \
    if (!(cond)) return VS_ERR_BAD_ARG;   \
  } while (0)

static inline int vs_launch_status() { return hipGetLastError() == hipSuccess ? VS_OK : VS_ERR_LAUNCH; }

static inline int64_t cdiv64(int64_t a, int64_t b) { return (a + b - 1) / b; }

#define VS_DEFAULT_ARITH 2
static inline int vs_default_arith() {
  static const int a = [] {
    const char* e = getenv("VIDEOSEAL_CONV");
    if (e && !strcmp(e, "f16x2")) return 2;
    if (e && !strcmp(e, "bf16x3")) return 3;
    return VS_DEFAULT_ARITH;
  }();
  return a;
}

enum { VS_DBG_RESIZE_FORM = 0 , VS_DBG_RESIZE_STRIP = 1 , VS_DBG_TAIL_STRIP = 2 , VS_DBG_JPEG_FORM = 3 , VS_DBG_CROP_RESIZE_FORM = 4 , VS_DBG_TO_PLANES_FORM = 5 , VS_DBG_DWCONV_ROWS = 6 , VS_DBG_LN_FORM = 7 , VS_DBG_SPLITK_EPI = 8 , VS_DBG_COUNT = 9 };
int vs_debug_get(int key);

static inline int vs_max_lds_bytes() {
  static const int n = [] {
    int dev = 0, v = 0;
    if (hipGetDevice(&dev) != hipSuccess || hipDeviceGetAttribute(&v, hipDeviceAttributeMaxSharedMemoryPerBlock, dev) != hipSuccess || v <= 0) v = 64 * 1024;
    return v;
  }();
  return n;
}

static inline int vs_num_cus() {
  static const int n = [] {
    int dev = 0, v = 0;
    if (hipGetDevice(&dev) != hipSuccess || hipDeviceGetAttribute(&v, hipDeviceAttributeMultiprocessorCount, dev) != hipSuccess || v <= 0) v = 256;
    return v;
  }();
  return n;
}

__device__ __forceinline__ float vs_erfc_sqrt2(float a) {
  const float u = fminf(a, 5.65685424949238f);
  float q = 5.128553084e-07f;
  q = __builtin_fmaf(q, u, -9.560153558e-06f);
  q = __builtin_fmaf(q, u, 7.497344632e-05f);
  q = __builtin_fmaf(q, u, -2.843466646e-04f);
  q = __builtin_fmaf(q, u, 1.498938855e-05f);
  q = __builtin_fmaf(q, u, 6.931120995e-03f);
  q = __builtin_fmaf(q, u, -5.243476480e-02f);
  q = __builtin_fmaf(q, u, -4.592214525e-01f);
  q = __builtin_fmaf(q, u, -1.151104212e+00f);
  return __builtin_amdgcn_exp2f(q * u);
}
__device__ __forceinline__ float vs_gelu(float v) {
  const float a = fabsf(v);
  const float e = vs_erfc_sqrt2(a);
  return fmaxf(v, 0.f) - (0.5f * a) * e;
}
typedef float vs_f32x2 __attribute__((ext_vector_type(2)));
__device__ __forceinline__ vs_f32x2 vs_gelu2(const vs_f32x2 v) {
#pragma clang fp contract(off)
  const vs_f32x2 a = {fabsf(v[0]), fabsf(v[1])};
  const vs_f32x2 u = {fminf(a[0], 5.65685424949238f), fminf(a[1], 5.65685424949238f)};
  vs_f32x2 q = {5.128553084e-07f, 5.128553084e-07f};
  q = __builtin_elementwise_fma(q, u, vs_f32x2{-9.560153558e-06f, -9.560153558e-06f});
  q = __builtin_elementwise_fma(q, u, vs_f32x2{7.497344632e-05f, 7.497344632e-05f});
  q = __builtin_elementwise_fma(q, u, vs_f32x2{-2.843466646e-04f, -2.843466646e-04f});
  q = __builtin_elementwise_fma(q, u, vs_f32x2{1.498938855e-05f, 1.498938855e-05f});
  q = __builtin_elementwise_fma(q, u, vs_f32x2{6.931120995e-03f, 6.931120995e-03f});
  q = __builtin_elementwise_fma(q, u, vs_f32x2{-5.243476480e-02f, -5.243476480e-02f});
  q = __builtin_elementwise_fma(q, u, vs_f32x2{-4.592214525e-01f, -4.592214525e-01f});
  q = __builtin_elementwise_fma(q, u, vs_f32x2{-1.151104212e+00f, -1.151104212e+00f});
  const vs_f32x2 t = q * u;
  const vs_f32x2 e = {__builtin_amdgcn_exp2f(t[0]), __builtin_amdgcn_exp2f(t[1])};
  const vs_f32x2 m = {fmaxf(v[0], 0.f), fmaxf(v[1], 0.f)};
  return __builtin_elementwise_fma(a * -0.5f, e, m);
}
__device__ __forceinline__ float vs_gelu_grad(float v) {
  const float e = vs_erfc_sqrt2(fabsf(v));
  const float Phi = v >= 0.f ? 1.f - 0.5f * e : 0.5f * e;
  return Phi + v * (0.3989422804014327f * __expf(-0.5f * v * v));
}

__device__ __forceinline__ float vs_relu(float v) { return v <= 0.f ? 0.f : v; }

__device__ __forceinline__ float vs_apply_act(float v, int act) {
  switch (act) {
    case VS_ACT_RELU: return vs_relu(v);
    case VS_ACT_GELU: return vs_gelu(v);
    case VS_ACT_TANH: return tanhf(v);
    case VS_ACT_SILU: return v / (1.0f + __expf(-v));
    default: return v;
  }
}

__device__ __forceinline__ float wave_sum(float v) {
#pragma unroll
  for (int o = 32; o > 0; o >>= 1) v += __shfl_xor(v, o, 64);
  return v;
}
```

### videoseal_amd/engine.py

```python
from __future__ import annotations

import ctypes as C
import math
import os
from dataclasses import dataclass
from typing import Dict, List, Optional, Tuple

import torch

from . import native as N


def rup(x: int, m: int) -> int:
    return (x + m - 1) // m * m


TUNED_TILES = os.path.join(os.path.dirname(os.path.abspath(__file__)), "tuned_tiles_gfx950.json")


@dataclass
class Act:
    t: torch.Tensor
    B: int
    H: int
# ... 680 lines not shown
            tpl = self.buf("bott.plt", h3.rows * cout).view(torch.int16)
            xpl = self.buf("bott.pl0", h3.rows * cout).view(torch.int16)
            if sk == 1:
                latpl = self.buf(tag + ".latpl", h3.rows * nlat).view(torch.int16)[: 2 * h3.rows * nlat]
                N.check(self.lib.vs_to_planes(N.ptr(h3.t), h3.rows, nlat, h3.ld, A_MUL, N.ptr(latpl), N.stream()), "vs_to_planes")
                self.conv(Act(None, h3.B, h3.H, h3.W, nlat, nlat), p["c0_lat"], ghost, pad=1, act=N.ACT_RELU, a_scale=pre, a_scale_ld=pre_ld,
                          tile_hint=ptile | N.CONV_PRE, in_pl=latpl, out_pl=tpl, prof=prof0)
            else:
                t = self.new_act(tag + ".t", h3.B, h3.H, h3.W, cout)
                self.conv(h3, p["c0_lat"], t, pad=1, act=N.ACT_RELU, cin=nlat, a_scale=pre, a_scale_ld=pre_ld, tile_hint=tile | N.CONV_PRE, prof=prof0)
                N.check(self.lib.vs_to_planes(N.ptr(t.t), t.rows, cout, t.ld, A_MUL, N.ptr(tpl), N.stream()), "vs_to_planes")
            self.conv(ghost, p["c1"], ghost, pad=1, act=N.ACT_RELU, in2=Act(None, h3.B, h3.H, h3.W, h3.C, h3.C), w2=p["res"], tile_hint=ptile,
                      in_pl=tpl, in2_pl=h3pl, out_pl=xpl, **(dict(split_k=sk) if sk > 1 else {}))
            self.planes_chain_ran = True
            return ghost, xpl
        t = self.new_act(tag + ".t", h3.B, h3.H, h3.W, cout)
        self.conv(h3, p["c0_lat"], t, pad=1, act=N.ACT_RELU, cin=nlat, a_scale=pre, a_scale_ld=pre_ld, tile_hint=tile | N.CONV_PRE, prof=prof0)
        out = self.new_act(tag + ".o", h3.B, h3.H, h3.W, cout)
        self.conv(t, p["c1"], out, pad=1, act=N.ACT_RELU, in2=h3, w2=p["res"])
        return (out, None) if planes_out else out

    def _msg0_ok(self, h3: Act, p, nlat: int) -> bool:
        hidden = h3.C - nlat
        return (self.use_split and self.msg_table_conv and "bn" not in p and "rms" not in p and nlat % 16 == 0 and hidden % 32 == 0 and
                h3.ld == h3.C and p["c0"].CinP == h3.C and h3.W % 16 == 0 and h3.H % 8 == 0 and p["cout"] >= 128 and
                h3.B * (h3.H // 8) * (h3.W // 16) >= 128)

    def resblock(self, x: Act, p, tag: str, out: Optional[Act] = None, out_coff=0) -> Act:
        if "rms" in p:
            assert out_coff == 0
            return self.resblock_rms(x, p, tag, out)
        if "bn" in p:
            assert out_coff == 0
            return self.resblock_train(x, p, tag, out)
        cout = p["cout"]
        if out_coff == 0 and self._thin_ok(x, p, out):
            return self.resblock_thin(x, p, tag, out)
        t = self.new_act(tag + ".t", x.B, x.H, x.W, cout)
        self.conv(x, p["c0"], t, pad=1, act=N.ACT_RELU, prof=("bott.conv3x3" if tag.startswith("bott") else None))
        if out is None:
            out = self.new_act(tag + ".o", x.B, x.H, x.W, cout)
        self.conv(t, p["c1"], out, pad=1, act=N.ACT_RELU, in2=x, w2=p["res"], out_coff=out_coff,
                  n_store=(cout if out.ld != rup(cout, 4) else None))
        return out

    def _thin_ok(self, x: Act, p, out: Optional[Act]) -> bool:
        c = p["cout"]
        if not (self.thin_fused and self.use_split and "bn" not in p and "rms" not in p and c in (16, 32)):
            return False
        k = 16 if c == 16 else 32
        return (x.ld <= k and p["c0"].CinP == k and p["c1"].CinP == k and p["res"].CinP == k and (out is None or out.ld == c) and
                (c == 16 or self.arith == 2) and bool(self.lib.vs_resblock_thin_supported(x.ld, c, c)))

    def resblock_thin(self, x: Act, p, tag: str, out: Optional[Act] = None) -> Act:
        ar, c = self.arith, p["cout"]
        c0, c1, cr = p["c0"].with_split(ar), p["c1"].with_split(ar), p["res"].with_split(ar)
        if out is None:
            out = self.new_act(tag + ".o", x.B, x.H, x.W, c)
        d = N.ResblockThinDesc()
        d.x, d.x_ld, d.B, d.H, d.W, d.Cin = N.ptr(x.t), x.ld, x.B, x.H, x.W, x.ld
        d.w0_split, d.w1_split, d.wr_split = N.ptr(c0.split), N.ptr(c1.split), N.ptr(cr.split)
        d.b0, d.b1, d.br = N.ptr(c0.bias), N.ptr(c1.bias), N.ptr(cr.bias)
        d.arith, d.Cout, d.a_mul = ar, c, A_MUL
        d.acc_mul0, d.acc_mul1, d.acc_mulr = 1.0 / (A_MUL * c0.w_mul), 1.0 / (A_MUL * c1.w_mul), 1.0 / (A_MUL * cr.w_mul)
        d.out, d.out_ld = N.ptr(out.t), out.ld
        timed = self.kernel_timers is not None and self.time_all_convs and not torch.cuda.is_current_stream_capturing()
        if timed:
            ev0, ev1 = torch.cuda.Event(enable_timing=True), torch.cuda.Event(enable_timing=True)
            ev0.record()
        N.check(self.lib.vs_resblock_thin(C.byref(d), N.stream()), "vs_resblock_thin")
        if timed:
            ev1.record()
            self.kernel_timers.append((f"resblock_thin {x.C}->{c}->{c} @{x.H}x{x.W}", ev0, ev1, 2.0 * x.rows * c * (2 * 9 * c + c)))
        return out

    _WHY = (f"with the 2 x f16 arithmetic an activation outside the f16 range of the operand split (|a| >= {65520.0 / A_MUL:.0f}; "
            f"{65520.0 / A_MUL_GRN:.0f} for the GRN-scaled pwconv2 input) becomes inf; VIDEOSEAL_CONV=bf16x3 selects the range-free exact split")

    def _guard(self, net: str, t: torch.Tensor) -> bool:
        idx = 0 if net == "E" else 1
        guarded = self.use_split and self.arith_net[net] == 2 and self.auto_arith
        if not guarded:
            if self.check_finite and not bool(torch.isfinite(t).all()):
                raise N.NativeError(f"{'embedder' if net == 'E' else 'extractor'}: non-finite output -- " + self._WHY)
            return True
        N.check(self.lib.vs_check_finite(N.ptr(t), t.numel(), self._nf_flag.data_ptr() + 4 * idx, N.stream()), "vs_check_finite")
        if torch.cuda.is_current_stream_capturing():
            return True
        if not self.verified[net]:
            if int(self._nf_flag[idx].item()):
                self._nf_flag[idx] = 0
                self.arith_net[net] = 3
                import warnings
                warnings.warn(f"{'embedder' if net == 'E' else 'extractor'}: activations leave the f16 range of the 2 x f16 operand split with these "
                              f"weights; this network now runs on the exact, range-free 3 x bf16 split (twice the matrix work)")
                return False
            self.verified[net] = True
            return True
        self.note_guard()
        return True

    def note_guard(self) -> None:
        if not (self.use_split and self.auto_arith) or self._nf_host is None:
            return
        self._nf_host.copy_(self._nf_flag, non_blocking=True)
        self._nf_event = torch.cuda.Event()
        self._nf_event.record()

    def _take_guard(self) -> List[str]:
        self._nf_event = None
        bad = [n for i, n in enumerate(("E", "X")) if int(self._nf_host[i]) and self.arith_net[n] == 2]
        if bad:
            for n in bad:
                self.arith_net[n] = 3
            self._nf_flag.zero_()
            self._nf_host.zero_()
        return bad
# ... 119 lines not shown
            return bool(self.upconv_fused and self.use_split and "gemm" in up_ and L.vs_upconv_fused_preferred(c1, c2, up_["gemm"].N // 9)
                        and up_["gemm"].CinP == c1 + c2)

        def lowres_cat(k: int, like: Act) -> Optional[Act]:
            if k >= nlev or "gemm" not in E["ups"][k] or bn_train or rms or fused_ok(k, like.C, hid[nlev - k].C):
                return None
            return self.new_act(f"up{k}.lcat", B, like.H, like.W, like.C + hid[nlev - k].C)

        xcur_pl = None
        for j in range(c.num_blocks):
            lc = lowres_cat(0, xcur) if j == c.num_blocks - 1 else None
            if j == 0 and lc is None and self._msg0_ok(h3, E["bott"][0], c.zc[-1]):
                nxt = Act(None, B, h3.H, h3.W, E["bott"][0]["cout"], E["bott"][0]["cout"])
                chain = c.num_blocks > 1 and not bn_train and self._planes_ok(nxt, E["bott"][1:])
                r0 = self.resblock_msg0(h3, E["bott"][0], "bott0", lat, Bm, c.zc[-1], planes_out=chain)
                xcur, xcur_pl = r0 if chain else (r0, None)
                continue
            if j >= 1 and not bn_train and self._planes_ok(xcur, E["bott"][j:]):
                lc = lowres_cat(0, xcur)
                xcur = self.bottleneck_planes(xcur, E["bott"][j:], Act(lc.t, B, lc.H, lc.W, xcur.C, lc.ld) if lc else None, xpl=xcur_pl)
                break
            xcur = self.resblock(xcur, E["bott"][j], f"bott{j & 1}", out=(Act(lc.t, B, lc.H, lc.W, xcur.C, lc.ld) if lc else None))
        for k in range(nlev):
            skip = hid.pop()
            up = E["ups"][k]
            if "gemm" in up and xcur.ld == xcur.C and fused_ok(k, xcur.C, skip.C):
                co = up["gemm"].N // 9
                ln = self.new_act(f"up{k}.ln", B, 2 * xcur.H, 2 * xcur.W, co)
                gw = up["gemm"].with_split(self.arith)
                N.check(L.vs_upconv_fused(N.ptr(xcur.t), xcur.C, xcur.ld, N.ptr(skip.t), skip.C, skip.ld, 2 ** -0.5,
                                          N.ptr(gw.split), B, xcur.H, xcur.W, co, N.ptr(up["lnw"]), N.ptr(up["lnb"]),
                                          1e-6, up_act, N.ptr(ln.t), ln.ld, self.arith, A_MUL, 1.0 / (A_MUL * gw.w_mul), st), "vs_upconv_fused")
            elif "gemm" in up:
                co = up["gemm"].N // 9
                direct = xcur.ld == xcur.C + skip.C
                lc = Act(xcur.t, B, xcur.H, xcur.W, xcur.C + skip.C, xcur.ld) if direct else \
                    self.new_act(f"up{k}.lcat", B, xcur.H, xcur.W, xcur.C + skip.C)
                N.check(L.vs_cat2_scale(None if direct else N.ptr(xcur.t), xcur.C, xcur.ld, N.ptr(skip.t), skip.C, skip.ld, 2 ** -0.5,
                                        lc.rows, N.ptr(lc.t), lc.ld, st), "vs_cat2_scale")
                z = self.new_act(f"up{k}.z", B, lc.H, lc.W, 9 * co)
                self.conv(lc, up["gemm"], z, prof=(f"up{k}.gemm9" if self.time_all_convs else None))
                ln = self.new_act(f"up{k}.ln", B, 2 * lc.H, 2 * lc.W, co)
                N.check(L.vs_upconv_gather_ln(N.ptr(z.t), z.ld, B, lc.H, lc.W, co, N.ptr(up["lnw"]), N.ptr(up["lnb"]), 1e-6, up_act,
                                              N.ptr(ln.t), ln.ld, st), "vs_upconv_gather_ln")
            else:
                cat = self.new_act(f"up{k}.cat", B, 2 * xcur.H, 2 * xcur.W, xcur.C + skip.C)
                N.check(L.vs_upcat2x(N.ptr(xcur.t), xcur.C, xcur.ld, N.ptr(skip.t), skip.C, skip.ld, 2 ** -0.5, B, xcur.H, xcur.W,
                                     N.ptr(cat.t), cat.ld, st), "vs_upcat2x")
                cv = self.new_act(f"up{k}.conv", B, cat.H, cat.W, up["conv"].N)
                self.conv(cat, up["conv"], cv, pad=1, pad_mode=N.PAD_REFLECT)
                ln = self.new_act(f"up{k}.ln", B, cat.H, cat.W, up["conv"].N)
                self.layernorm(cv, up["lnw"], up["lnb"], ln, act=up_act)
            lc = lowres_cat(k + 1, ln)
            xcur = self.resblock(ln, up["rb"], f"up{k}", out=(Act(lc.t, B, lc.H, lc.W, up["rb"]["cout"], lc.ld) if lc else None))
        delta = self.buf("delta", B * c.out_ch * xcur.H * xcur.W)
        N.check(L.vs_outc_tanh(N.ptr(xcur.t), xcur.H * xcur.W, B, xcur.C, xcur.ld, N.ptr(E["outc_w"]), N.ptr(E["outc_b"]), c.out_ch,
                               1 if c.last_tanh else 0, N.ptr(delta), st), "vs_outc_tanh")
        return delta.view(B, c.out_ch, xcur.H, xcur.W)

    def extractor_forward(self, x: Act) -> torch.Tensor:
        for attempt in range(3):
            self.arith = self.arith_net["X"]
            logits = self.vit_extractor_forward(x) if self.cfg.extractor == "sam" else self._extractor_forward(x)
            if self._guard("X", logits):
                break
            if self.layer_arith:
                self.layer_arith.clear()
            elif attempt == 0 and self.per_layer_arith and self.cfg.extractor != "sam":
                self._calibrate_extractor(x)
        return logits

    def _note_absmax(self, key: tuple, t: torch.Tensor, numel: int) -> None:
        if self._calib is None:
            return
        slot = self._calib.setdefault(key, len(self._calib))
        N.check(self.lib.vs_absmax(N.ptr(t), numel, self._calib_bits.data_ptr() + 4 * slot, N.stream()), "vs_absmax")

    def _calibrate_extractor(self, x: Act) -> None:
        self._calib, self._calib_bits = {}, torch.zeros(4096, dtype=torch.int32, device=self.dev)
        try:
            self.arith = 3
            self._extractor_forward(x)
            bits = self._calib_bits.cpu()
            keys = dict(self._calib)
        finally:
            self._calib = self._calib_bits = None
        amax = {k: float(bits[slot:slot + 1].view(torch.float32)) for k, slot in keys.items()}
        limit = 65504.0 / 4.0
        over = {k for k, v in amax.items() if not (v * (A_MUL_GRN if k[-1] == "pw2" else A_MUL) < limit)}
        self.calib_absmax = amax
        if over and len(over) < len(amax):
            self.layer_arith = {k: 3 for k in over}
            self.arith_net["X"], self.verified["X"] = 2, False
            import warnings
            warnings.warn(f"extractor: {len(over)} of {len(amax)} block GEMMs keep the exact 3 x bf16 split (operands beyond the f16 range of the "
                          f"2 x f16 split: {sorted(over)[:6]}{' ...' if len(over) > 6 else ''}); the other layers stay on the fast split")

    def _extractor_forward(self, x: Act) -> torch.Tensor:
        if self.X is None:
            self._pack_extractor(self._g)
        c, X, L = self.cfg, self.X, self.lib
        st = N.stream()
        B = x.B
        s = c.stem_stride
        Ho, Wo = (x.H - 4) // s + 1, (x.W - 4) // s + 1
        d = c.dims
# ... 306 lines not shown
```

### videoseal_amd/native.py

```python
from __future__ import annotations

import ctypes as C
import os
from typing import Optional

import torch

_HERE = os.path.dirname(os.path.abspath(__file__))
LIB_PATH = os.environ.get("VIDEOSEAL_LIB") or os.path.join(_HERE, "csrc", "libvideoseal_hip.so")

ACT_NONE, ACT_RELU, ACT_GELU, ACT_TANH, ACT_SILU = 0, 1, 2, 3, 4
PAD_ZERO, PAD_REFLECT = 0, 1
CONV_FORCE_F32, CONV_FORCE_SPLIT, CONV_TILE_HI, CONV_PRE = 0x10, 0x20, 0x40, 0x80
VIDEO_MODES = {"repeat": 0, "alternate": 1, "interpolate": 2}

EXPORTS = [
    "vs_version", "vs_arch", "vs_error_string", "vs_sizeof_conv_desc", "vs_sizeof_tail_desc", "vs_debug_set",
    "vs_model_create", "vs_model_destroy", "vs_model_workspace_bytes", "vs_model_embed", "vs_model_detect", "vs_conv_gemm", "vs_to_planes", "vs_to_planes_affine", "vs_layernorm_act", "vs_layernorm_patch2x2", "vs_stem_conv_ln", "vs_rmsnorm_act", "vs_vit_attention", "vs_dwconv7_ln", "vs_dwconv7_ln_planes", "vs_grn_scale", "vs_grn_scale_from_partials", "vs_grn_scale_from_straddle_partials", "vs_grn_apply",
    "vs_upcat2x", "vs_upconv_supported", "vs_upconv_gather_ln", "vs_cat2_scale", "vs_msg_pre", "vs_upconv_fused_supported", "vs_upconv_fused_preferred", "vs_upconv_fused", "vs_im2col3x3", "vs_msg_latent", "vs_broadcast_channels", "vs_outc_tanh", "vs_pool_linear", "vs_resize_pre", "vs_resize_pre_u8",
    "vs_jnd_heatmap", "vs_embed_tail", "vs_aug_color_scratch_floats", "vs_aug_color", "vs_aug_color_chain", "vs_aug_crop_resize_color", "vs_aug_crop_flip", "vs_aug_warp", "vs_resize_nchw",
    "vs_gaussian_blur", "vs_median_filter", "vs_jpeg_workspace_bytes", "vs_jpeg_roundtrip", "vs_h264_proxy_workspace_bytes", "vs_h264_proxy_roundtrip",
    "vs_bn_partial_doubles", "vs_bn_batch_stats", "vs_bn_partial_sums", "vs_bn_finish_sums", "vs_scale_shift_act", "vs_aug_mask_blend", "vs_aug_add_scaled", "vs_aug_gather_frames", "vs_aug_window_average",
    "vs_gemm_wgrad_partial_floats", "vs_gemm_wgrad", "vs_conv3x3_wgrad", "vs_conv3x3_wgrad_supported", "vs_conv3x3_wgrad_partial_floats", "vs_pad_embed1", "vs_reflect_fold1", "vs_pack_conv", "vs_gaussian_blur_bwd", "vs_aug_warp_bwd", "vs_aug_gather_frames_bwd", "vs_aug_window_average_bwd", "vs_gelu_bwd", "vs_act_bwd", "vs_rmsnorm_act_bwd", "vs_vit_attention_bwd_scratch_floats", "vs_vit_attention_bwd", "vs_dwconv7", "vs_dwconv7_wgrad_partial_floats", "vs_dwconv7_wgrad", "vs_colreduce_partial_floats",
    "vs_layernorm_bwd", "vs_gelu_grn_bwd", "vs_patchify", "vs_unpatch", "vs_patchify_s", "vs_unpatch_s", "vs_col2im3x3_reflect", "vs_colmean", "vs_pool_gelu_bwd", "vs_matmul_small",
    "vs_bce_logits",
    "vs_bn_mean_rstd", "vs_bn_bwd_partial_floats", "vs_bn_relu_bwd_sums", "vs_bn_relu_bwd_apply", "vs_dilate2", "vs_im2col3x3_strided", "vs_upcat2x_bwd",
    "vs_msg_table_grad", "vs_outc_tanh_bwd", "vs_relu_bwd",
    "vs_resize_nchw_bwd", "vs_embed_tail_bwd", "vs_tail_key_reduce", "vs_aug_crop_flip_bwd", "vs_mask_mul", "vs_aug_color_bwd_scratch_floats",
    "vs_aug_color_bwd", "vs_clamp01_bwd", "vs_nhwc_to_nchw_scaled", "vs_percep_partial_doubles", "vs_percep_mse", "vs_percep_mse_grad",
    "vs_ssim_partial_doubles", "vs_ssim_stats", "vs_ssim_grad", "vs_avgpool2_pad", "vs_jnd_loss_partial_doubles", "vs_jnd_loss", "vs_jnd_loss_grad",
    "vs_split_block", "vs_check_finite", "vs_absmax", "vs_resblock_thin", "vs_resblock_thin_supported", "vs_cnx_block_supported", "vs_cnx_block_image_bytes", "vs_cnx_block",
]


class NativeError(RuntimeError):
    pass


class ConvDesc(C.Structure):
    _fields_ = [
        ("inp", C.c_void_p), ("in_sb", C.c_int64), ("in_sy", C.c_int64), ("in_sx", C.c_int64),
        ("B", C.c_int32), ("H", C.c_int32), ("W", C.c_int32), ("Cin", C.c_int32),
        ("KH", C.c_int32), ("KW", C.c_int32), ("SH", C.c_int32), ("SW", C.c_int32), ("PH", C.c_int32), ("PW", C.c_int32),
        ("pad_mode", C.c_int32), ("Ho", C.c_int32), ("Wo", C.c_int32),
        ("wt", C.c_void_p), ("CinP", C.c_int32), ("N", C.c_int32),
        ("a_scale", C.c_void_p), ("a_scale_ld", C.c_int64), ("a_shift", C.c_void_p),
        ("bias", C.c_void_p), ("act", C.c_int32), ("n_store", C.c_int32),
        ("res", C.c_void_p), ("res_ld", C.c_int64),
        ("in2", C.c_void_p), ("in2_ld", C.c_int64), ("Cin2", C.c_int32), ("Cin2P", C.c_int32),
        ("wt2", C.c_void_p), ("bias2", C.c_void_p),
        ("out", C.c_void_p), ("out_ld", C.c_int64), ("out_coff", C.c_int32), ("tile_hint", C.c_int32),
        ("wt_split", C.c_void_p), ("wt2_split", C.c_void_p), ("wt_blk", C.c_void_p), ("wt2_blk", C.c_void_p),
        ("splitk_ws", C.c_void_p), ("splitk_ld", C.c_int64), ("split_k", C.c_int32), ("arith", C.c_int32),
        ("sumsq_part", C.c_void_p), ("in_pl", C.c_void_p), ("in2_pl", C.c_void_p), ("out_pl", C.c_void_p), ("a_mul", C.c_float), ("acc_mul", C.c_float), ("acc_mul2", C.c_float), ("grn_nchunk", C.c_int32), ("grn_part", C.c_void_p), ("grn_gamma", C.c_void_p), ("sumsq_hw", C.c_int32), ("reserved_", C.c_int32),
    ]


class TailDesc(C.Structure):
    _fields_ = [
        ("imgs", C.c_void_p), ("out", C.c_void_p), ("preds_w", C.c_void_p),
        ("delta", C.c_void_p), ("hmap_lowres", C.c_void_p), ("taps43", C.c_void_p),
        ("F", C.c_int32), ("H", C.c_int32), ("W", C.c_int32), ("S_h", C.c_int32), ("S_w", C.c_int32), ("Cd", C.c_int32),
        ("step", C.c_int32), ("video_mode", C.c_int32), ("total_key", C.c_int32),
        ("attenuate", C.c_int32), ("clamp", C.c_int32), ("antialias", C.c_int32),
        ("scaling_i", C.c_float), ("scaling_w", C.c_float), ("io_u8", C.c_int32), ("variant", C.c_int32),
    ]


class ResblockThinDesc(C.Structure):
    _fields_ = [
        ("x", C.c_void_p), ("x_ld", C.c_int64), ("B", C.c_int32), ("H", C.c_int32), ("W", C.c_int32), ("Cin", C.c_int32),
        ("w0_split", C.c_void_p), ("w1_split", C.c_void_p), ("wr_split", C.c_void_p),
        ("b0", C.c_void_p), ("b1", C.c_void_p), ("br", C.c_void_p),
        ("arith", C.c_int32), ("Cout", C.c_int32),
        ("a_mul", C.c_float), ("acc_mul0", C.c_float), ("acc_mul1", C.c_float), ("acc_mulr", C.c_float),
        ("out", C.c_void_p), ("out_ld", C.c_int64),
    ]


_lib: Optional[C.CDLL] = None


def lib() -> C.CDLL:
    global _lib
# ... 64 lines not shown
        "vs_pad_embed1": [P, I, I, I, I64, P, P],
        "vs_reflect_fold1": [P, I, I, I, I64, P, P],
        "vs_pack_conv": [P, I, I, I, I, I, I, P, P],
        "vs_gaussian_blur_bwd": [P, P, P, I, I, I, I, F, P],
        "vs_aug_warp_bwd": [P, P, I, I, I, I, I, I, P, I, P, P],
        "vs_aug_gather_frames_bwd": [P, P, P, P, I, I64, P],
        "vs_aug_window_average_bwd": [P, P, I, I64, I, F, P],
        "vs_gelu_bwd": [P, I64, P, I64, I64, I, P, I64, P],
        "vs_act_bwd": [P, I64, P, I64, I64, I, I, P, I64, P],
        "vs_rmsnorm_act_bwd": [P, I64, I, I64, P, I, P, I64, P, I64, P, I64, P],
        "vs_vit_attention_bwd": [P, P, P, I, I, I, I, I, I, P, P, P, P, P, P, P],
        "vs_dwconv7": [P, I, I, I, I, I64, P, P, I, P, I64, P, I64, P],
        "vs_dwconv7_wgrad": [P, I64, P, I64, I, I, I, I, P, P, P],
        "vs_layernorm_bwd": [P, I64, P, I64, P, I64, I, F, P, I64, P, P, P, P, P],
        "vs_gelu_grn_bwd": [P, I64, P, I64, P, I, I, I, P, P, P, I64, P, P, P],
        "vs_patchify": [P, I, I, I, I64, I, P, P],
        "vs_unpatch": [P, I, I, I, I64, I, P, P],
        "vs_patchify_s": [P, I, I, I, I64, I, I, P, P],
        "vs_unpatch_s": [P, I, I, I, I64, I, I, P, P],
        "vs_col2im3x3_reflect": [P, I, I, I, I64, P, P],
        "vs_colmean": [P, I, I, I64, P, P],
        "vs_pool_gelu_bwd": [P, I64, P, I64, I, I, I, P, I64, P],
        "vs_matmul_small": [P, I64, P, I64, I, I, I, P, I64, P],
        "vs_bce_logits": [P, P, I, I, I, F, F, P, P, P],
        "vs_bn_mean_rstd": [P, I, I64, F, P, P, P],
        "vs_bn_relu_bwd_sums": [P, I64, P, I64, P, P, P, P, I, I64, I, P, P, P, P, P],
        "vs_bn_relu_bwd_apply": [P, I64, P, I64, P, P, P, P, I, P, I64, I, P, I64, P],
        "vs_dilate2": [P, I, I, I, I64, I, I, P, P],
        "vs_im2col3x3_strided": [P, I, I, I, I64, I, P, P],
        "vs_upcat2x_bwd": [P, I64, I, I, I, I, I, F, P, I64, P, I64, P],
        "vs_msg_table_grad": [P, P, I, I, I, P, P],
        "vs_outc_tanh_bwd": [P, P, I64, I, I, P, I, I, P, I64, P, P],
        "vs_relu_bwd": [P, I64, P, I64, I64, I, P, I64, P],
        "vs_resize_nchw_bwd": [P, P, I, I, I, I, I, I, P, P],
        "vs_embed_tail_bwd": [P, P, P, P, P, I, I, I, I, I, F, F, P, P],
        "vs_tail_key_reduce": [P, P, I, I, I, I, I, I, I, P, P],
        "vs_aug_crop_flip_bwd": [P, P, I, I, I, I, I, I, I, I, P],
        "vs_mask_mul": [P, P, P, I, I, I, I, I, P],
        "vs_aug_color_bwd": [P, P, P, I, I, I, I, F, P, P, P],
        "vs_clamp01_bwd": [P, P, P, I64, P],
        "vs_nhwc_to_nchw_scaled": [P, I, I, I, I, I64, F, P, P],
        "vs_percep_mse": [P, P, I, I, I, I, P, P, P],
        "vs_percep_mse_grad": [P, P, I, I, I, I, F, P, P],
        "vs_ssim_stats": [P, P, I, I, I, F, P, P, P, P],
        "vs_ssim_grad": [P, P, P, P, P, I, I, I, F, P, P, P],
        "vs_avgpool2_pad": [P, P, I, I, I, P, P, P],
        "vs_jnd_loss": [P, P, P, I, I, I, P, P, P],
        "vs_jnd_loss_grad": [P, P, P, I, I, I, F, P, P],
        "vs_split_block": [P, I, I64, I, I, F, P, P, P],
        "vs_check_finite": [P, I64, P, P],
        "vs_absmax": [P, I64, P, P],
        "vs_resblock_thin": [P, P],
        "vs_resblock_thin_supported": [I, I, I],
        "vs_cnx_block": [P, P, I, I64, I, I, F, F, P, I64, P, P, I64, P, I64, P, P],
        "vs_cnx_block_supported": [I, I64, I],
    }
    for name, args in sig.items():
        fn = getattr(L, name)
        fn.argtypes = args
        fn.restype = C.c_int
    L.vs_aug_color_scratch_floats.restype = C.c_int64
    L.vs_aug_color_scratch_floats.argtypes = [I, I, I]
    L.vs_jpeg_workspace_bytes.restype = C.c_int64
    L.vs_jpeg_workspace_bytes.argtypes = [I, I, I]
    L.vs_h264_proxy_workspace_bytes.restype = C.c_int64
    L.vs_h264_proxy_workspace_bytes.argtypes = [I, I, I]
    L.vs_vit_attention_bwd_scratch_floats.restype = C.c_int64
    L.vs_vit_attention_bwd_scratch_floats.argtypes = [I, I, I, I, I]
    for name in ("vs_aug_color_bwd_scratch_floats", "vs_percep_partial_doubles", "vs_ssim_partial_doubles", "vs_jnd_loss_partial_doubles"):
        getattr(L, name).restype = C.c_int64
        getattr(L, name).argtypes = [I, I, I]
    L.vs_cnx_block_image_bytes.restype = C.c_int64
    L.vs_cnx_block_image_bytes.argtypes = [I]
    L.vs_bn_partial_doubles.restype = C.c_int64
    L.vs_bn_partial_doubles.argtypes = [I64, I64]
    for name, args in (("vs_gemm_wgrad_partial_floats", [I64, I, I]), ("vs_conv3x3_wgrad_partial_floats", [I, I64, I, I, I, I]), ("vs_dwconv7_wgrad_partial_floats", [I, I, I64]),
                       ("vs_colreduce_partial_floats", [I, I64, I64]), ("vs_bn_bwd_partial_floats", [I64, I64])):
        getattr(L, name).restype = C.c_int64
        getattr(L, name).argtypes = args
    L.vs_sizeof_conv_desc.restype = C.c_int
    L.vs_sizeof_tail_desc.restype = C.c_int
    if L.vs_version() != 3:
        raise NativeError(f"{LIB_PATH} has ABI version {L.vs_version()}, this binding is written for 3: rebuild (make -C videoseal_amd/csrc)")
    if L.vs_sizeof_conv_desc() != C.sizeof(ConvDesc) or L.vs_sizeof_tail_desc() != C.sizeof(TailDesc):
        raise NativeError("ctypes mirrors of vs_conv_desc_t / vs_tail_desc_t are out of date with the shared library")
    _lib = L
    return L


ERR_UNSUPPORTED = -2


def check(code: int, what: str) -> None:
    if code != 0:
        raise NativeError(f"{what} failed: {lib().vs_error_string(code).decode()} (code {code})")


def ptr(t: Optional[torch.Tensor]) -> Optional[int]:
    if t is None:
        return None
    if not t.is_cuda:
        raise NativeError("HIP kernels need device tensors (got a CPU tensor); move the model/inputs to cuda first")
    return t.data_ptr()


def stream() -> int:
# ... 8 lines not shown
```

Baseline: 4076 frames/s.

## Fuse final thin resblock with output conv and block upconv-gather LayerNorm by 2x2 cells

Adds a resblock_thin_outc path that computes the last decoder resblock and the 1x1 output conv with optional tanh in one kernel. This removes the intermediate activation write and read and one launch at full resolution. It also adds a blocked upconv-gather+LayerNorm kernel: each thread handles a 2x2 output cell from interior low-res positions with fixed bilinear weights, reusing loaded z values across four outputs, while border ring pixels take the per-pixel path. The blocked kernel raises register pressure and changes FMA ordering, so results may differ slightly from the old path.

```diff
diff --git a/include/videoseal_hip.h b/include/videoseal_hip.h
--- a/include/videoseal_hip.h
+++ b/include/videoseal_hip.h
@@ -188,6 +188,9 @@
 } vs_resblock_thin_desc_t;
 int vs_resblock_thin_supported(int cin_ld, int cmid, int cout);
 int vs_resblock_thin(const vs_resblock_thin_desc_t* d, void* stream);
+int vs_resblock_thin_outc_supported(int cin_ld, int cmid, int cout, int out_ch);
+int vs_resblock_thin_outc(const vs_resblock_thin_desc_t* d, const float* outc_w, const float* outc_b, int out_ch, int use_tanh, float* delta,
+                          void* stream);
 
 int vs_check_finite(const float* x, int64_t n, int* flag, void* stream);
 
diff --git a/videoseal_amd/csrc/model_api.hip b/videoseal_amd/csrc/model_api.hip
--- a/videoseal_amd/csrc/model_api.hip
+++ b/videoseal_amd/csrc/model_api.hip
@@ -373,18 +373,34 @@
   void layernorm(const Act& x, const float* w, const float* b, const Act& out, int act_ = VS_ACT_NONE) {
     if (live()) chk(vs_layernorm_act(x.p, x.rows(), x.C, x.ld, w, b, 1e-6f, act_, out.p, out.ld, st));
   }
+  bool thin_ok(const Act& x, const RB& p, const Act* out_in) const {
+    const int tk = p.cout == 16 ? 16 : 32;
+    return (p.cout == 16 || (p.cout == 32 && m->arith == 2)) && x.ld <= tk && p.c0.CinP == tk && p.c1.CinP == tk && p.res.CinP == tk &&
+           (!out_in || out_in->ld == p.cout) && vs_resblock_thin_supported(x.ld, p.cout, p.cout);
+  }
+  vs_resblock_thin_desc_t thin_desc(const Act& x, const RB& p) const {
+    vs_resblock_thin_desc_t d;
+    std::memset(&d, 0, sizeof(d));
+    d.x = x.p; d.x_ld = x.ld; d.B = x.B; d.H = x.H; d.W = x.W; d.Cin = x.ld;
+    d.w0_split = p.c0.split; d.w1_split = p.c1.split; d.wr_split = p.res.split;
+    d.b0 = p.c0.bias; d.b1 = p.c1.bias; d.br = p.res.bias;
+    d.arith = m->arith; d.Cout = p.cout; d.a_mul = A_MUL;
+    d.acc_mul0 = 1.f / (A_MUL * p.c0.w_mul); d.acc_mul1 = 1.f / (A_MUL * p.c1.w_mul); d.acc_mulr = 1.f / (A_MUL * p.res.w_mul);
+    return d;
+  }
+  bool thin_outc_ok(const Act& x, const RB& p) const {
+    return thin_ok(x, p, nullptr) && vs_resblock_thin_outc_supported(x.ld, p.cout, p.cout, m->c.out_ch);
+  }
+  float* resblock_outc(const Act& x, const RB& p) {
+    float* delta = alloc((int64_t)x.B * m->c.out_ch * x.H * x.W);
+    const vs_resblock_thin_desc_t d = thin_desc(x, p);
+    if (live()) chk(vs_resblock_thin_outc(&d, m->outc_w, m->outc_b, m->c.out_ch, m->c.last_tanh ? 1 : 0, delta, st));
+    return delta;
+  }
   Act resblock(const Act& x, const RB& p, const Act* out_in = nullptr) {
-    const int tk = p.cout == 16 ? 16 : 32;
-    if ((p.cout == 16 || (p.cout == 32 && m->arith == 2)) && x.ld <= tk && p.c0.CinP == tk && p.c1.CinP == tk && p.res.CinP == tk &&
-        (!out_in || out_in->ld == p.cout) && vs_resblock_thin_supported(x.ld, p.cout, p.cout)) {
+    if (thin_ok(x, p, out_in)) {
       Act out = out_in ? *out_in : act(x.B, x.H, x.W, p.cout);
-      vs_resblock_thin_desc_t d;
-      std::memset(&d, 0, sizeof(d));
-      d.x = x.p; d.x_ld = x.ld; d.B = x.B; d.H = x.H; d.W = x.W; d.Cin = x.ld;
-      d.w0_split = p.c0.split; d.w1_split = p.c1.split; d.wr_split = p.res.split;
-      d.b0 = p.c0.bias; d.b1 = p.c1.bias; d.br = p.res.bias;
-      d.arith = m->arith; d.Cout = p.cout; d.a_mul = A_MUL;
-      d.acc_mul0 = 1.f / (A_MUL * p.c0.w_mul); d.acc_mul1 = 1.f / (A_MUL * p.c1.w_mul); d.acc_mulr = 1.f / (A_MUL * p.res.w_mul);
+      vs_resblock_thin_desc_t d = thin_desc(x, p);
       d.out = out.p; d.out_ld = out.ld;
       if (live()) chk(vs_resblock_thin(&d, st));
       return out;
@@ -572,6 +588,10 @@
       }
       Act view{};
       const bool direct = lowres_cat(k + 1, Act{nullptr, B, ln.H, ln.W, up.rb.cout, 0}, view);
+      if (k == nlev - 1 && !direct && thin_outc_ok(ln, up.rb)) {
+        Sh = ln.H; Sw = ln.W;
+        return resblock_outc(ln, up.rb);
+      }
       cur = resblock(ln, up.rb, direct ? &view : nullptr);
     }
     float* delta = alloc((int64_t)B * c.out_ch * cur.H * cur.W);
diff --git a/videoseal_amd/csrc/net_ops.hip b/videoseal_amd/csrc/net_ops.hip
--- a/videoseal_amd/csrc/net_ops.hip
+++ b/videoseal_amd/csrc/net_ops.hip
@@ -3,6 +3,7 @@
 #include <cstring>
 
 #include "conv_common.h"
+#include "upconv_gather.h"
 
 namespace {
 
@@ -593,6 +594,105 @@
 }
 
 template <int CG>
+__device__ __forceinline__ void upg_pixel_gather(const float* __restrict__ z, const int64_t zld, const int H, const int W, const int Co, const int64_t b,
+                                                 const int Y, const int X, const int g, f32x4 (&acc)[CG / 4]) {
+  const int W2 = 2 * W, H2 = 2 * H;
+  int ys[3][2], xs[3][2];
+  float wy[3][2], wx[3][2];
+#pragma unroll
+  for (int k = 0; k < 3; ++k) {
+    int yr = Y + k - 1, xr = X + k - 1;
+    yr = yr < 0 ? -yr : (yr >= H2 ? 2 * H2 - 2 - yr : yr);
+    xr = xr < 0 ? -xr : (xr >= W2 ? 2 * W2 - 2 - xr : xr);
+    const float sy = fmaxf((yr + 0.5f) * 0.5f - 0.5f, 0.f), sx = fmaxf((xr + 0.5f) * 0.5f - 0.5f, 0.f);
+    const int y0 = (int)sy, x0 = (int)sx;
+    ys[k][0] = y0; ys[k][1] = y0 + (y0 < H - 1);
+    xs[k][0] = x0; xs[k][1] = x0 + (x0 < W - 1);
+    wy[k][1] = sy - y0; wy[k][0] = 1.f - wy[k][1];
+    wx[k][1] = sx - x0; wx[k][0] = 1.f - wx[k][1];
+  }
+  constexpr int NV = CG / 4;
+#pragma unroll
+  for (int j = 0; j < NV; ++j) acc[j] = f32x4{0.f, 0.f, 0.f, 0.f};
+  const float* zb = z + b * H * W * zld + g * CG;
+#pragma unroll
+  for (int ky = 0; ky < 3; ++ky)
+#pragma unroll
+    for (int a = 0; a < 2; ++a) {
+      const float* zr = zb + (int64_t)ys[ky][a] * W * zld + ky * 3 * Co;
+#pragma unroll
+      for (int kx = 0; kx < 3; ++kx)
+#pragma unroll
+        for (int c = 0; c < 2; ++c) {
+          const float w = wy[ky][a] * wx[kx][c];
+          const float* q = zr + (int64_t)xs[kx][c] * zld + kx * Co;
+#pragma unroll
+          for (int j = 0; j < NV; ++j) acc[j] = vs_upconv_fma(w, *reinterpret_cast<const f32x4*>(q + 4 * j), acc[j]);
+        }
+    }
+}
+__device__ __attribute__((noinline)) f32x4 upg_act4(f32x4 v, const int act) {
+#pragma unroll
+  for (int e = 0; e < 4; ++e) v[e] = vs_apply_act(v[e], act);
+  return v;
+}
+template <int CG, int NPX>
+__device__ __forceinline__ void upg_ln_store(const f32x4 (&acc)[NPX][CG / 4], const int tpp_log2, const int Co, const float eps, const int act,
+                                             const f32x4 (&lwv)[CG / 4], const f32x4 (&lbv)[CG / 4], const bool live, float* const (&orow)[NPX]) {
+#pragma clang fp contract(off)
+  constexpr int NV = CG / 4;
+  constexpr int NFUSED = CG == 16 ? 4 : 1;
+  float s[NPX], v[NPX], mean[NPX], den[NPX];
+#pragma unroll
+  for (int q = 0; q < NPX; ++q) {
+    s[q] = 0.f;
+#pragma unroll
+    for (int j = 0; j < NV; ++j) s[q] += (acc[q][j][0] + acc[q][j][1]) + (acc[q][j][2] + acc[q][j][3]);
+  }
+  for (int o = 1; o < (1 << tpp_log2); o <<= 1) {
+#pragma unroll
+    for (int q = 0; q < NPX; ++q) s[q] += __shfl_xor(s[q], o, 64);
+  }
+#pragma unroll
+  for (int q = 0; q < NPX; ++q) {
+    mean[q] = s[q] / (float)Co;
+    v[q] = 0.f;
+#pragma unroll
+    for (int j = 0; j < NV; ++j)
+#pragma unroll
+      for (int e = 0; e < 4; ++e) {
+        const float dl = acc[q][j][e] - mean[q];
+        if (4 * j + e == 0) v[q] = dl * dl;
+        else if (4 * j + e < NFUSED) v[q] = __builtin_fmaf(dl, dl, v[q]);
+        else v[q] = v[q] + dl * dl;
+      }
+  }
+  for (int o = 1; o < (1 << tpp_log2); o <<= 1) {
+#pragma unroll
+    for (int q = 0; q < NPX; ++q) v[q] += __shfl_xor(v[q], o, 64);
+  }
+#pragma unroll
+  for (int q = 0; q < NPX; ++q) den[q] = sqrtf(v[q] / (float)Co + eps);
+  if (!live) return;
+#pragma unroll
+  for (int q = 0; q < NPX; ++q)
+#pragma unroll
+    for (int j = 0; j < NV; ++j) {
+      const f32x4 wv = lwv[j], bv = lbv[j];
+      f32x4 o;
+#pragma unroll
+      for (int e = 0; e < 4; ++e) o[e] = __builtin_fmaf(wv[e], (acc[q][j][e] - mean[q]) / den[q], bv[e]);
+      if (act == VS_ACT_RELU) {
+#pragma unroll
+        for (int e = 0; e < 4; ++e) o[e] = vs_relu(o[e]);
+      } else {
+        o = upg_act4(o, act);
+      }
+      *reinterpret_cast<f32x4*>(orow[q] + 4 * j) = o;
+    }
+}
+
+template <int CG>
 __global__ __launch_bounds__(256) void upconv_gather_ln_kernel(const float* __restrict__ z, int64_t zld, int H, int W, int Co,
                                                                int tpp_log2, const float* __restrict__ lnw,
                                                                const float* __restrict__ lnb, float eps, int act,
@@ -604,10 +704,10 @@
   const int g = (int)(gid & ((1 << tpp_log2) - 1));
   const bool live = pq < npix && vb < nblk;
   const int64_t p = live ? pq : 0;
-  constexpr int NVP = CG / 4;
-  f32x4 lwv[NVP], lbv[NVP];
-#pragma unroll
-  for (int j = 0; j < NVP; ++j) {
+  constexpr int NV = CG / 4;
+  f32x4 lwv[NV], lbv[NV];
+#pragma unroll
+  for (int j = 0; j < NV; ++j) {
     lwv[j] = *reinterpret_cast<const f32x4*>(lnw + g * CG + 4 * j);
     lbv[j] = *reinterpret_cast<const f32x4*>(lnb + g * CG + 4 * j);
   }
@@ -616,62 +716,64 @@
   const int64_t t0 = p / W2;
   const int Y = (int)(t0 % H2);
   const int64_t b = t0 / H2;
-  int ys[3][2], xs[3][2];
-  float wy[3][2], wx[3][2];
-#pragma unroll
-  for (int k = 0; k < 3; ++k) {
-    int yr = Y + k - 1, xr = X + k - 1;
-    yr = yr < 0 ? -yr : (yr >= H2 ? 2 * H2 - 2 - yr : yr);
-    xr = xr < 0 ? -xr : (xr >= W2 ? 2 * W2 - 2 - xr : xr);
-    const float sy = fmaxf((yr + 0.5f) * 0.5f - 0.5f, 0.f), sx = fmaxf((xr + 0.5f) * 0.5f - 0.5f, 0.f);
-    const int y0 = (int)sy, x0 = (int)sx;
-    ys[k][0] = y0; ys[k][1] = y0 + (y0 < H - 1);
-    xs[k][0] = x0; xs[k][1] = x0 + (x0 < W - 1);
-    wy[k][1] = sy - y0; wy[k][0] = 1.f - wy[k][1];
-    wx[k][1] = sx - x0; wx[k][0] = 1.f - wx[k][1];
-  }
+  f32x4 acc[1][NV];
+  float* const orow[1] = {out + p * old + g * CG};
+  upg_pixel_gather<CG>(z, zld, H, W, Co, b, Y, X, g, acc[0]);
+  upg_ln_store<CG, 1>(acc, tpp_log2, Co, eps, act, lwv, lbv, live, orow);
+}
+
+template <int CG>
+__global__ __launch_bounds__(256, (CG == 4 ? 7 : CG == 8 ? 4 : 2)) void upconv_gather_ln_blocked_kernel(const float* __restrict__ z, int64_t zld, int H, int W, int Co,
+                                                                       int tpp_log2, const float* __restrict__ lnw,
+                                                                       const float* __restrict__ lnb, float eps, int act,
+                                                                       float* __restrict__ out, int64_t old, int64_t ncell, int grid_int,
+                                                                       int64_t nring) {
   constexpr int NV = CG / 4;
-  f32x4 acc[NV];
-#pragma unroll
-  for (int j = 0; j < NV; ++j) acc[j] = f32x4{0.f, 0.f, 0.f, 0.f};
-  const float* zb = z + b * H * W * zld + g * CG;
-#pragma unroll
-  for (int ky = 0; ky < 3; ++ky)
-#pragma unroll
-    for (int a = 0; a < 2; ++a) {
-      const float* zr = zb + (int64_t)ys[ky][a] * W * zld + ky * 3 * Co;
-#pragma unroll
-      for (int kx = 0; kx < 3; ++kx)
-#pragma unroll
-        for (int c = 0; c < 2; ++c) {
-          const float w = wy[ky][a] * wx[kx][c];
-          const float* q = zr + (int64_t)xs[kx][c] * zld + kx * Co;
-#pragma unroll
-          for (int j = 0; j < NV; ++j) acc[j] += w * *reinterpret_cast<const f32x4*>(q + 4 * j);
-        }
-    }
-  float s = 0.f;
-#pragma unroll
-  for (int j = 0; j < NV; ++j) s += (acc[j][0] + acc[j][1]) + (acc[j][2] + acc[j][3]);
-  for (int o = 1; o < (1 << tpp_log2); o <<= 1) s += __shfl_xor(s, o, 64);
-  const float mean = s / (float)Co;
-  float v = 0.f;
-#pragma unroll
-  for (int j = 0; j < NV; ++j)
-#pragma unroll
-    for (int e = 0; e < 4; ++e) { const float dl = acc[j][e] - mean; v += dl * dl; }
-  for (int o = 1; o < (1 << tpp_log2); o <<= 1) v += __shfl_xor(v, o, 64);
-  const float den = sqrtf(v / (float)Co + eps);
-  if (!live) return;
-  float* orow = out + p * old + g * CG;
+  const int g = (int)(threadIdx.x & ((1 << tpp_log2) - 1));
+  f32x4 lwv[NV], lbv[NV];
 #pragma unroll
   for (int j = 0; j < NV; ++j) {
-    const f32x4 wv = lwv[j], bv = lbv[j];
-    f32x4 o;
-#pragma unroll
-    for (int e = 0; e < 4; ++e) o[e] = vs_apply_act(wv[e] * ((acc[j][e] - mean) / den) + bv[e], act);
-    *reinterpret_cast<f32x4*>(orow + 4 * j) = o;
-  }
+    lwv[j] = *reinterpret_cast<const f32x4*>(lnw + g * CG + 4 * j);
+    lbv[j] = *reinterpret_cast<const f32x4*>(lnb + g * CG + 4 * j);
+  }
+  const int W2 = 2 * W, H2 = 2 * H;
+  if ((int)blockIdx.x < grid_int) {
+    const int per = grid_int >> 3;
+    const int64_t vb = (int64_t)(blockIdx.x & 7) * per + (blockIdx.x >> 3);
+    const int64_t cq = (vb * 256 + threadIdx.x) >> tpp_log2;
+    const bool live = cq < ncell;
+    const int64_t cidx = live ? cq : 0;
+    const int Wi = W - 2, Hi = H - 2;
+    const int j = 1 + (int)(cidx % Wi);
+    const int64_t t0 = cidx / Wi;
+    const int i = 1 + (int)(t0 % Hi);
+    const int64_t b = t0 / Hi;
+    f32x4 acc[4][NV];
+#pragma unroll
+    for (int q = 0; q < 4; ++q)
+#pragma unroll
+      for (int jv = 0; jv < NV; ++jv) acc[q][jv] = f32x4{0.f, 0.f, 0.f, 0.f};
+    vs_upconv_gather_cell<NV, false, int64_t>(z + ((b * H + i) * W + j) * zld + g * CG, (int64_t)W * zld, zld, Co, acc);
+    float* const o00 = out + ((b * H2 + 2 * i) * W2 + 2 * j) * old + g * CG;
+    float* const orow[4] = {o00, o00 + old, o00 + W2 * old, o00 + (W2 + 1) * old};
+    upg_ln_store<CG, 4>(acc, tpp_log2, Co, eps, act, lwv, lbv, live, orow);
+    return;
+  }
+  const int64_t pq = ((int64_t)((int)blockIdx.x - grid_int) * 256 + threadIdx.x) >> tpp_log2;
+  const bool live = pq < nring;
+  const int64_t pr = live ? pq : 0;
+  const int R = 2 * W + 2 * (H - 2);
+  const int c = (int)((pr >> 2) % R);
+  const int64_t b = (pr >> 2) / R;
+  int i, j;
+  if (c < W) { i = 0; j = c; }
+  else if (c < 2 * W) { i = H - 1; j = c - W; }
+  else { i = 1 + ((c - 2 * W) >> 1); j = ((c - 2 * W) & 1) ? W - 1 : 0; }
+  const int Y = 2 * i + (int)((pr >> 1) & 1), X = 2 * j + (int)(pr & 1);
+  f32x4 acc[1][NV];
+  float* const orow[1] = {out + ((b * H2 + Y) * W2 + X) * old + g * CG};
+  upg_pixel_gather<CG>(z, zld, H, W, Co, b, Y, X, g, acc[0]);
+  upg_ln_store<CG, 1>(acc, tpp_log2, Co, eps, act, lwv, lbv, live, orow);
 }
 
 __global__ __launch_bounds__(256) void im2col3x3_kernel(const float* __restrict__ x, int H, int W, int64_t ld, int reflect,
@@ -779,19 +881,10 @@
   const float* xr = x + row * ld;
   for (int c = 0; c < C; c += 4) {
     const f32x4 v = *reinterpret_cast<const f32x4*>(xr + c);
-    for (int o = 0; o < Cout; ++o) {
-      const float* wr = w + (int64_t)o * C + c;
-      acc[o] += v[0] * wr[0];
-      if (c + 1 < C) acc[o] += v[1] * wr[1];
-      if (c + 2 < C) acc[o] += v[2] * wr[2];
-      if (c + 3 < C) acc[o] += v[3] * wr[3];
-    }
+    for (int o = 0; o < Cout; ++o) acc[o] = vs_outc_mac4(acc[o], v, w + (int64_t)o * C + c, C - c);
   }
   const int64_t b = row / rpf, p = row - b * rpf;
-  for (int o = 0; o < Cout; ++o) {
-    float v = acc[o] + bias[o];
-    out[(b * Cout + o) * rpf + p] = use_tanh ? tanhf(v) : v;
-  }
+  for (int o = 0; o < Cout; ++o) out[(b * Cout + o) * rpf + p] = vs_outc_act(acc[o], bias[o], use_tanh);
 }
 
 __global__ __launch_bounds__(256) void pool_linear_kernel(const float* __restrict__ x, int HW, int C, int64_t ld,
@@ -1352,12 +1445,24 @@
   const int cg = Co >= 64 ? 16 : Co / 4;
   int tl = 0;
   while ((cg << tl) < Co) ++tl;
+  hipStream_t st = (hipStream_t)stream;
+  if (H >= 3 && W >= 3 && vs_debug_get(VS_DBG_UPCONV_GATHER) != 1) {
+    const int64_t ncell = (int64_t)B * (H - 2) * (W - 2);
+    const int64_t nring = (int64_t)B * (2 * W + 2 * (H - 2)) * 4;
+    const int64_t nbi = cdiv64(cdiv64(ncell << tl, 256), 8) * 8, nbr = cdiv64(nring << tl, 256);
+    VS_REQUIRE(nbi + nbr < (1 << 30));
+#define VS_UPGB(CG_) hipLaunchKernelGGL(upconv_gather_ln_blocked_kernel<CG_>, dim3((unsigned)(nbi + nbr)), dim3(256), 0, st, z, z_ld, H, W, Co, tl, lnw, lnb, eps, act, out, out_ld, ncell, (int)nbi, nring)
+    if (cg == 4) VS_UPGB(4);
+    else if (cg == 8) VS_UPGB(8);
+    else VS_UPGB(16);
+#undef VS_UPGB
+    return vs_launch_status();
+  }
   const int64_t npix = (int64_t)B * 4 * H * W;
   const int64_t nblk64 = cdiv64(npix << tl, 256);
   VS_REQUIRE(nblk64 < (1 << 30));
   const int nblk = (int)nblk64;
   const int grid = ((nblk + 7) / 8) * 8;
-  hipStream_t st = (hipStream_t)stream;
 #define VS_UPG(CG_) hipLaunchKernelGGL(upconv_gather_ln_kernel<CG_>, dim3(grid), dim3(256), 0, st, z, z_ld, H, W, Co, tl, lnw, lnb, eps, act, out, out_ld, npix, nblk)
   if (cg == 4) VS_UPG(4);
   else if (cg == 8) VS_UPG(8);
diff --git a/videoseal_amd/csrc/resblock_thin.hip b/videoseal_amd/csrc/resblock_thin.hip
--- a/videoseal_amd/csrc/resblock_thin.hip
+++ b/videoseal_amd/csrc/resblock_thin.hip
@@ -38,196 +38,20 @@
   return __builtin_bit_cast(bf16x8, z);
 }
 
+struct OutcArgs { const float* w; const float* bias; int out_ch, use_tanh; float* delta; };
+
 template <int NP, int NBUF, int OCC>
 __global__ __launch_bounds__(256, OCC) void resblock_thin_kernel(const RbArgs d, const int tiles_x, const int tiles_y, const int ntiles_total,
                                                                  const int tiles_per_wg) {
-  using AR = Arith<NP>;
-  using A16 = Arith16<NP>;
-  constexpr int XP_BYTES = NP * X_PX * ROWB16;
-  constexpr int TT_BYTES = NP * T_PX * ROWB16;
-  __shared__ __attribute__((aligned(16))) unsigned char smem[NBUF * XP_BYTES + TT_BYTES];
-  unsigned char* const Tt = smem + NBUF * XP_BYTES;
-  const int tid = threadIdx.x;
-  const int lane = tid & 63;
-  const int wave = tid >> 6;
-  const int n = lane & 15, kb = lane >> 4;
-  const int hi = kb >> 1;
-  const int kh = (kb & 1) * 8;
-
-  bf16x8 w0f[5][NP], w1f[5][NP], wrf[NP];
-#pragma unroll
-  for (int s = 0; s < 5; ++s) {
-    const int tap = 2 * s + hi;
-#pragma unroll
-    for (int p = 0; p < NP; ++p) {
-      if (tap < 9) {
-        w0f[s][p] = *reinterpret_cast<const bf16x8*>(static_cast<const char*>(d.w0) + ((int64_t)p * 16 * 144 + n * 144 + tap * 16 + kh) * 2);
-        w1f[s][p] = *reinterpret_cast<const bf16x8*>(static_cast<const char*>(d.w1) + ((int64_t)p * 16 * 144 + n * 144 + tap * 16 + kh) * 2);
-      } else {
-        w0f[s][p] = zero_frag();
-        w1f[s][p] = zero_frag();
-      }
-    }
-  }
-#pragma unroll
-  for (int p = 0; p < NP; ++p)
-    wrf[p] = hi == 0 ? *reinterpret_cast<const bf16x8*>(static_cast<const char*>(d.wr) + ((int64_t)p * 16 * 16 + n * 16 + kh) * 2) : zero_frag();
-  float b0v[4], b1v[4], brv[4];
-#pragma unroll
-  for (int e = 0; e < 4; ++e) {
-    b0v[e] = d.b0 ? d.b0[4 * kb + e] : 0.f;
-    b1v[e] = d.b1 ? d.b1[4 * kb + e] : 0.f;
-    brv[e] = d.br ? d.br[4 * kb + e] : 0.f;
-  }
-
-  int p_dy[NXI], p_dx[NXI], p_lds[NXI];
-  bool p_have[NXI];
-  const int k4 = (tid & 3) * 4;
-  const bool cok = k4 < d.Cin;
-#pragma unroll
-  for (int i = 0; i < NXI; ++i) {
-    const int item = tid + i * 256;
-    p_have[i] = item < XITEMS;
-    const int prow = p_have[i] ? item >> 2 : 0;
-    p_dy[i] = prow / X_W - 2;
-    p_dx[i] = prow % X_W - 2;
-    p_lds[i] = prow * ROWB16 + k4 * 2;
-  }
-  int toffx[5], tofft[5];
-#pragma unroll
-  for (int s5 = 0; s5 < 5; ++s5) {
-    const int tap = 2 * s5 + hi < 9 ? 2 * s5 + hi : 8;
-    toffx[s5] = ((tap / 3) * X_W + tap % 3) * ROWB16;
-    tofft[s5] = ((tap / 3) * T_W + tap % 3) * ROWB16;
-  }
-  int a0[G0_PER_WAVE], t_i[G0_PER_WAVE];
-#pragma unroll
-  for (int gi = 0; gi < G0_PER_WAVE; ++gi) {
-    int i = 16 * (wave * G0_PER_WAVE + gi) + n;
-    t_i[gi] = i;
-    i = i < T_PX ? i : T_PX - 1;
-    a0[gi] = ((i / T_W) * X_W + (i % T_W)) * ROWB16 + kh * 2;
-  }
-  int a1[G1_PER_WAVE], ar[G1_PER_WAVE];
-#pragma unroll
-  for (int gi = 0; gi < G1_PER_WAVE; ++gi) {
-    const int row = wave * G1_PER_WAVE + gi;
-    a1[gi] = (row * T_W + n) * ROWB16 + kh * 2;
-    ar[gi] = ((row + 2) * X_W + (n + 2)) * ROWB16 + kh * 2;
-  }
-  const float amul = NP == 2 ? d.a_mul : 1.f;
-  const float am0 = NP == 2 ? d.acc_mul0 : 1.f, am1 = NP == 2 ? d.acc_mul1 : 1.f, amr = NP == 2 ? d.acc_mulr : 1.f;
-
-  f32x4 rp[NXI];
-  auto load_tile = [&](const int fb, const int y0, const int x0) __attribute__((always_inline)) {
-#pragma unroll
-    for (int i = 0; i < NXI; ++i) {
-      const int iy = y0 + p_dy[i], ix = x0 + p_dx[i];
-      const bool ok = p_have[i] && cok && iy >= 0 && iy < d.H && ix >= 0 && ix < d.W;
-      const int cy = iy < 0 ? 0 : (iy >= d.H ? d.H - 1 : iy), cx = ix < 0 ? 0 : (ix >= d.W ? d.W - 1 : ix);
-      const f32x4 v = *reinterpret_cast<const f32x4*>(d.x + (int64_t)fb * d.x_sb + (int64_t)cy * d.x_sy + (int64_t)cx * d.x_sx + (cok ? k4 : 0));
-      rp[i] = ok ? v : f32x4{0.f, 0.f, 0.f, 0.f};
-    }
-  };
-  auto store_tile = [&](const int buf) __attribute__((always_inline)) {
-    unsigned char* Ps = smem + buf * XP_BYTES;
-#pragma unroll
-    for (int i = 0; i < NXI; ++i)
-      if (p_have[i]) {
-        u32x2 pl[NP];
-        split4n<NP>(rp[i], amul, pl);
-#pragma unroll
-        for (int p = 0; p < NP; ++p) *reinterpret_cast<u32x2*>(Ps + p * X_PX * ROWB16 + p_lds[i]) = pl[p];
-      }
-  };
-
-  const int t_begin = blockIdx.x * tiles_per_wg;
-  const int t_end = min(ntiles_total, t_begin + tiles_per_wg);
-  if (t_begin >= t_end) return;
-  int tx = t_begin % tiles_x, ty = (t_begin / tiles_x) % tiles_y, fb = t_begin / (tiles_x * tiles_y);
-  load_tile(fb, ty * TH, tx * TW);
-  store_tile(0);
-  __syncthreads();
-  for (int t = t_begin; t < t_end; ++t) {
-    const int buf = NBUF == 2 ? (t - t_begin) & 1 : 0;
-    int ntx = tx + 1, nty = ty, nfb = fb;
-    if (ntx == tiles_x) { ntx = 0; if (++nty == tiles_y) { nty = 0; ++nfb; } }
-    {
-      const bool more = t + 1 < t_end;
-      load_tile(more ? nfb : fb, (more ? nty : ty) * TH, (more ? ntx : tx) * TW);
-    }
-    const unsigned char* Ps = smem + buf * XP_BYTES;
-    const int y0 = ty * TH, x0 = tx * TW;
-
-#pragma unroll
-    for (int gi = 0; gi < G0_PER_WAVE; ++gi) {
-      f32x4 acc = {0.f, 0.f, 0.f, 0.f};
-#pragma unroll
-      for (int s = 0; s < 5; ++s) {
-        const int off = a0[gi] + toffx[s];
-        bf16x8 xf[NP];
-#pragma unroll
-        for (int p = 0; p < NP; ++p) xf[p] = *reinterpret_cast<const bf16x8*>(Ps + p * X_PX * ROWB16 + off);
-#pragma unroll
-        for (int q = 0; q < AR::NPROD; ++q) acc = A16::mfma(w0f[s][AR::PB[q]], xf[AR::PA[q]], acc);
-      }
-      const int i = t_i[gi];
-      if (i < T_PX) {
-        const int gy = y0 - 1 + i / T_W, gx = x0 - 1 + i % T_W;
-        const bool in = gy >= 0 && gy < d.H && gx >= 0 && gx < d.W;
-        f32x4 v;
-#pragma unroll
-        for (int e = 0; e < 4; ++e) {
-          const float a = NP == 2 ? acc[e] * am0 : acc[e];
-          v[e] = in ? vs_relu(a + b0v[e]) : 0.f;
-        }
-        u32x2 pl[NP];
-        split4n<NP>(v, amul, pl);
-#pragma unroll
-        for (int p = 0; p < NP; ++p) *reinterpret_cast<u32x2*>(Tt + p * T_PX * ROWB16 + i * ROWB16 + 8 * kb) = pl[p];
-      }
-    }
-    if (NBUF == 2 && t + 1 < t_end) store_tile(buf ^ 1);
-    __syncthreads();
-
-#pragma unroll
-    for (int gi = 0; gi < G1_PER_WAVE; ++gi) {
-      f32x4 acc = {0.f, 0.f, 0.f, 0.f}, accr = {0.f, 0.f, 0.f, 0.f};
-#pragma unroll
-      for (int s = 0; s < 5; ++s) {
-        const int off = a1[gi] + tofft[s];
-        bf16x8 tf[NP];
-#pragma unroll
-        for (int p = 0; p < NP; ++p) tf[p] = *reinterpret_cast<const bf16x8*>(Tt + p * T_PX * ROWB16 + off);
-#pragma unroll
-        for (int q = 0; q < AR::NPROD; ++q) acc = A16::mfma(w1f[s][AR::PB[q]], tf[AR::PA[q]], acc);
-      }
-      {
-        bf16x8 xf[NP];
-#pragma unroll
-        for (int p = 0; p < NP; ++p) xf[p] = *reinterpret_cast<const bf16x8*>(Ps + p * X_PX * ROWB16 + ar[gi]);
-#pragma unroll
-        for (int q = 0; q < AR::NPROD; ++q) accr = A16::mfma(wrf[AR::PB[q]], xf[AR::PA[q]], accr);
-      }
-      const int y = y0 + wave * G1_PER_WAVE + gi, x = x0 + n;
-      if (y < d.H && x < d.W) {
-        f32x4 v;
-#pragma unroll
-        for (int e = 0; e < 4; ++e) {
-          const float a = NP == 2 ? acc[e] * am1 : acc[e];
-          const float r = NP == 2 ? accr[e] * amr : accr[e];
-          v[e] = vs_relu(a + b1v[e]) + (r + brv[e]);
-        }
-        *reinterpret_cast<f32x4*>(d.out + (((int64_t)fb * d.H + y) * d.W + x) * d.out_ld + 4 * kb) = v;
-      }
-    }
-    if (NBUF == 1) {
-      __syncthreads();
-      if (t + 1 < t_end) store_tile(0);
-    }
-    __syncthreads();
-    tx = ntx; ty = nty; fb = nfb;
-  }
+  constexpr bool OUTC = false;
+  const OutcArgs oc{};
+#include "resblock_thin_body.inc"
+}
+template <int NP, int NBUF, int OCC>
+__global__ __launch_bounds__(256, OCC) void resblock_thin_outc_kernel(const RbArgs d, const OutcArgs oc, const int tiles_x, const int tiles_y,
+                                                                      const int ntiles_total, const int tiles_per_wg) {
+  constexpr bool OUTC = true;
+#include "resblock_thin_body.inc"
 }
 
 constexpr int ROWB32 = 96;
@@ -453,15 +277,16 @@
   return (cmid == 16 && cout == 16 && cin_ld <= 16) ? 1 : 0;
 }
 
-extern "C" int vs_resblock_thin(const vs_resblock_thin_desc_t* d, void* stream) {
-  VS_REQUIRE(d && d->x && d->out && d->w0_split && d->w1_split && d->wr_split && d->B > 0 && d->H > 0 && d->W > 0);
+static int launch_thin(const vs_resblock_thin_desc_t* d, const OutcArgs* oc, void* stream) {
+  VS_REQUIRE(d && d->x && (oc || d->out) && d->w0_split && d->w1_split && d->wr_split && d->B > 0 && d->H > 0 && d->W > 0);
   const int C = d->Cout == 32 ? 32 : 16;
   VS_REQUIRE(d->Cout == 0 || d->Cout == 16 || d->Cout == 32);
-  VS_REQUIRE(vs_resblock_thin_supported(d->Cin, C, C) && d->x_ld >= d->Cin && (d->x_ld & 3) == 0 && d->out_ld >= C && (d->out_ld & 3) == 0);
+  VS_REQUIRE(vs_resblock_thin_supported(d->Cin, C, C) && d->x_ld >= d->Cin && (d->x_ld & 3) == 0 && (oc || (d->out_ld >= C && (d->out_ld & 3) == 0)));
   VS_REQUIRE(d->arith == 2 || (d->arith == 3 && C == 16));
-  VS_REQUIRE((((uintptr_t)d->x | (uintptr_t)d->out | (uintptr_t)d->w0_split | (uintptr_t)d->w1_split | (uintptr_t)d->wr_split) & 15) == 0);
+  VS_REQUIRE((((uintptr_t)d->x | (uintptr_t)(oc ? nullptr : d->out) | (uintptr_t)d->w0_split | (uintptr_t)d->w1_split | (uintptr_t)d->wr_split) & 15) == 0);
+  if (oc) VS_REQUIRE(C == 16 && oc->w && oc->bias && oc->delta && oc->out_ch >= 1 && oc->out_ch <= 4);
   RbArgs a{d->x, (int64_t)d->H * d->W * d->x_ld, (int64_t)d->W * d->x_ld, d->x_ld, d->B, d->H, d->W, d->Cin,
-           d->w0_split, d->w1_split, d->wr_split, d->b0, d->b1, d->br, d->a_mul, d->acc_mul0, d->acc_mul1, d->acc_mulr, d->out, d->out_ld};
+           d->w0_split, d->w1_split, d->wr_split, d->b0, d->b1, d->br, d->a_mul, d->acc_mul0, d->acc_mul1, d->acc_mulr, oc ? nullptr : d->out, d->out_ld};
   const int tiles_x = (d->W + TW - 1) / TW, tiles_y = (d->H + TH - 1) / TH;
   const int64_t nt = (int64_t)d->B * tiles_x * tiles_y;
   if (nt > 0x7fffffffLL) return VS_ERR_UNSUPPORTED;
@@ -469,8 +294,24 @@
   const int per = (int)((nt + want - 1) / want);
   const int tpw = per < 1 ? 1 : per;
   const unsigned grid = (unsigned)((nt + tpw - 1) / tpw);
-  if (C == 32) hipLaunchKernelGGL(resblock_thin32_kernel, dim3(grid), dim3(NT32), 0, (hipStream_t)stream, a, tiles_x, tiles_y, (int)nt, tpw);
-  else if (d->arith == 2) hipLaunchKernelGGL((resblock_thin_kernel<2, 2, 2>), dim3(grid), dim3(256), 0, (hipStream_t)stream, a, tiles_x, tiles_y, (int)nt, tpw);
-  else hipLaunchKernelGGL((resblock_thin_kernel<3, 1, 2>), dim3(grid), dim3(256), 0, (hipStream_t)stream, a, tiles_x, tiles_y, (int)nt, tpw);
+  hipStream_t st = (hipStream_t)stream;
+  if (oc) {
+    if (d->arith == 2) hipLaunchKernelGGL((resblock_thin_outc_kernel<2, 2, 2>), dim3(grid), dim3(256), 0, st, a, *oc, tiles_x, tiles_y, (int)nt, tpw);
+    else hipLaunchKernelGGL((resblock_thin_outc_kernel<3, 1, 2>), dim3(grid), dim3(256), 0, st, a, *oc, tiles_x, tiles_y, (int)nt, tpw);
+  } else if (C == 32) hipLaunchKernelGGL(resblock_thin32_kernel, dim3(grid), dim3(NT32), 0, st, a, tiles_x, tiles_y, (int)nt, tpw);
+  else if (d->arith == 2) hipLaunchKernelGGL((resblock_thin_kernel<2, 2, 2>), dim3(grid), dim3(256), 0, st, a, tiles_x, tiles_y, (int)nt, tpw);
+  else hipLaunchKernelGGL((resblock_thin_kernel<3, 1, 2>), dim3(grid), dim3(256), 0, st, a, tiles_x, tiles_y, (int)nt, tpw);
   return vs_launch_status();
 }
+
+extern "C" int vs_resblock_thin(const vs_resblock_thin_desc_t* d, void* stream) { return launch_thin(d, nullptr, stream); }
+
+extern "C" int vs_resblock_thin_outc_supported(int cin_ld, int cmid, int cout, int out_ch) {
+  return cmid == 16 && cout == 16 && out_ch >= 1 && out_ch <= 4 && vs_resblock_thin_supported(cin_ld, cmid, cout);
+}
+
+extern "C" int vs_resblock_thin_outc(const vs_resblock_thin_desc_t* d, const float* outc_w, const float* outc_b, int out_ch, int use_tanh, float* delta,
+                                     void* stream) {
+  const OutcArgs oc{outc_w, outc_b, out_ch, use_tanh ? 1 : 0, delta};
+  return launch_thin(d, &oc, stream);
+}
diff --git a/videoseal_amd/csrc/resblock_thin_body.inc b/videoseal_amd/csrc/resblock_thin_body.inc
--- /dev/null
+++ b/videoseal_amd/csrc/resblock_thin_body.inc
@@ -0,0 +1,216 @@
+  using AR = Arith<NP>;
+  using A16 = Arith16<NP>;
+  constexpr int XP_BYTES = NP * X_PX * ROWB16;
+  constexpr int TT_BYTES = NP * T_PX * ROWB16;
+  constexpr int OC_BYTES = OUTC ? 4 * 16 * 4 : 0;
+  __shared__ __attribute__((aligned(16))) unsigned char smem[NBUF * XP_BYTES + TT_BYTES + OC_BYTES];
+  unsigned char* const Tt = smem + NBUF * XP_BYTES;
+  const int tid = threadIdx.x;
+  const int lane = tid & 63;
+  const int wave = tid >> 6;
+  const int n = lane & 15, kb = lane >> 4;
+  const int hi = kb >> 1;
+  const int kh = (kb & 1) * 8;
+
+  bf16x8 w0f[5][NP], w1f[5][NP], wrf[NP];
+#pragma unroll
+  for (int s = 0; s < 5; ++s) {
+    const int tap = 2 * s + hi;
+#pragma unroll
+    for (int p = 0; p < NP; ++p) {
+      if (tap < 9) {
+        w0f[s][p] = *reinterpret_cast<const bf16x8*>(static_cast<const char*>(d.w0) + ((int64_t)p * 16 * 144 + n * 144 + tap * 16 + kh) * 2);
+        w1f[s][p] = *reinterpret_cast<const bf16x8*>(static_cast<const char*>(d.w1) + ((int64_t)p * 16 * 144 + n * 144 + tap * 16 + kh) * 2);
+      } else {
+        w0f[s][p] = zero_frag();
+        w1f[s][p] = zero_frag();
+      }
+    }
+  }
+#pragma unroll
+  for (int p = 0; p < NP; ++p)
+    wrf[p] = hi == 0 ? *reinterpret_cast<const bf16x8*>(static_cast<const char*>(d.wr) + ((int64_t)p * 16 * 16 + n * 16 + kh) * 2) : zero_frag();
+  float b0v[4], b1v[4], brv[4];
+#pragma unroll
+  for (int e = 0; e < 4; ++e) {
+    b0v[e] = d.b0 ? d.b0[4 * kb + e] : 0.f;
+    b1v[e] = d.b1 ? d.b1[4 * kb + e] : 0.f;
+    brv[e] = d.br ? d.br[4 * kb + e] : 0.f;
+  }
+
+  int p_dy[NXI], p_dx[NXI], p_lds[NXI];
+  bool p_have[NXI];
+  const int k4 = (tid & 3) * 4;
+  const bool cok = k4 < d.Cin;
+#pragma unroll
+  for (int i = 0; i < NXI; ++i) {
+    const int item = tid + i * 256;
+    p_have[i] = item < XITEMS;
+    const int prow = p_have[i] ? item >> 2 : 0;
+    p_dy[i] = prow / X_W - 2;
+    p_dx[i] = prow % X_W - 2;
+    p_lds[i] = prow * ROWB16 + k4 * 2;
+  }
+  int toffx[5], tofft[5];
+#pragma unroll
+  for (int s5 = 0; s5 < 5; ++s5) {
+    const int tap = 2 * s5 + hi < 9 ? 2 * s5 + hi : 8;
+    toffx[s5] = ((tap / 3) * X_W + tap % 3) * ROWB16;
+    tofft[s5] = ((tap / 3) * T_W + tap % 3) * ROWB16;
+  }
+  int a0[G0_PER_WAVE], t_i[G0_PER_WAVE];
+#pragma unroll
+  for (int gi = 0; gi < G0_PER_WAVE; ++gi) {
+    int i = 16 * (wave * G0_PER_WAVE + gi) + n;
+    t_i[gi] = i;
+    i = i < T_PX ? i : T_PX - 1;
+    a0[gi] = ((i / T_W) * X_W + (i % T_W)) * ROWB16 + kh * 2;
+  }
+  int a1[G1_PER_WAVE], ar[G1_PER_WAVE];
+#pragma unroll
+  for (int gi = 0; gi < G1_PER_WAVE; ++gi) {
+    const int row = wave * G1_PER_WAVE + gi;
+    a1[gi] = (row * T_W + n) * ROWB16 + kh * 2;
+    ar[gi] = ((row + 2) * X_W + (n + 2)) * ROWB16 + kh * 2;
+  }
+  const float amul = NP == 2 ? d.a_mul : 1.f;
+  const float am0 = NP == 2 ? d.acc_mul0 : 1.f, am1 = NP == 2 ? d.acc_mul1 : 1.f, amr = NP == 2 ? d.acc_mulr : 1.f;
+  const float* const ocw = OUTC ? reinterpret_cast<const float*>(smem + NBUF * XP_BYTES + TT_BYTES) + 16 * kb : nullptr;
+  float ocb = 0.f;
+  if (OUTC) {
+    if (tid < 64) reinterpret_cast<float*>(smem + NBUF * XP_BYTES + TT_BYTES)[tid] = tid < 16 * oc.out_ch ? oc.w[tid] : 0.f;
+    ocb = kb < oc.out_ch ? oc.bias[kb] : 0.f;
+  }
+
+  f32x4 rp[NXI];
+  auto load_tile = [&](const int fb, const int y0, const int x0) __attribute__((always_inline)) {
+#pragma unroll
+    for (int i = 0; i < NXI; ++i) {
+      const int iy = y0 + p_dy[i], ix = x0 + p_dx[i];
+      const bool ok = p_have[i] && cok && iy >= 0 && iy < d.H && ix >= 0 && ix < d.W;
+      const int cy = iy < 0 ? 0 : (iy >= d.H ? d.H - 1 : iy), cx = ix < 0 ? 0 : (ix >= d.W ? d.W - 1 : ix);
+      const f32x4 v = *reinterpret_cast<const f32x4*>(d.x + (int64_t)fb * d.x_sb + (int64_t)cy * d.x_sy + (int64_t)cx * d.x_sx + (cok ? k4 : 0));
+      rp[i] = ok ? v : f32x4{0.f, 0.f, 0.f, 0.f};
+    }
+  };
+  auto store_tile = [&](const int buf) __attribute__((always_inline)) {
+    unsigned char* Ps = smem + buf * XP_BYTES;
+#pragma unroll
+    for (int i = 0; i < NXI; ++i)
+      if (p_have[i]) {
+        u32x2 pl[NP];
+        split4n<NP>(rp[i], amul, pl);
+#pragma unroll
+        for (int p = 0; p < NP; ++p) *reinterpret_cast<u32x2*>(Ps + p * X_PX * ROWB16 + p_lds[i]) = pl[p];
+      }
+  };
+
+  const int t_begin = blockIdx.x * tiles_per_wg;
+  const int t_end = min(ntiles_total, t_begin + tiles_per_wg);
+  if (t_begin >= t_end) return;
+  int tx = t_begin % tiles_x, ty = (t_begin / tiles_x) % tiles_y, fb = t_begin / (tiles_x * tiles_y);
+  load_tile(fb, ty * TH, tx * TW);
+  store_tile(0);
+  __syncthreads();
+  for (int t = t_begin; t < t_end; ++t) {
+    const int buf = NBUF == 2 ? (t - t_begin) & 1 : 0;
+    int ntx = tx + 1, nty = ty, nfb = fb;
+    if (ntx == tiles_x) { ntx = 0; if (++nty == tiles_y) { nty = 0; ++nfb; } }
+    {
+      const bool more = t + 1 < t_end;
+      load_tile(more ? nfb : fb, (more ? nty : ty) * TH, (more ? ntx : tx) * TW);
+    }
+    const unsigned char* Ps = smem + buf * XP_BYTES;
+    const int y0 = ty * TH, x0 = tx * TW;
+
+#pragma unroll
+    for (int gi = 0; gi < G0_PER_WAVE; ++gi) {
+      f32x4 acc = {0.f, 0.f, 0.f, 0.f};
+#pragma unroll
+      for (int s = 0; s < 5; ++s) {
+        const int off = a0[gi] + toffx[s];
+        bf16x8 xf[NP];
+#pragma unroll
+        for (int p = 0; p < NP; ++p) xf[p] = *reinterpret_cast<const bf16x8*>(Ps + p * X_PX * ROWB16 + off);
+#pragma unroll
+        for (int q = 0; q < AR::NPROD; ++q) acc = A16::mfma(w0f[s][AR::PB[q]], xf[AR::PA[q]], acc);
+      }
+      const int i = t_i[gi];
+      if (i < T_PX) {
+        const int gy = y0 - 1 + i / T_W, gx = x0 - 1 + i % T_W;
+        const bool in = gy >= 0 && gy < d.H && gx >= 0 && gx < d.W;
+        f32x4 v;
+#pragma unroll
+        for (int e = 0; e < 4; ++e) {
+          const float a = NP == 2 ? acc[e] * am0 : acc[e];
+          v[e] = in ? vs_relu(a + b0v[e]) : 0.f;
+        }
+        u32x2 pl[NP];
+        split4n<NP>(v, amul, pl);
+#pragma unroll
+        for (int p = 0; p < NP; ++p) *reinterpret_cast<u32x2*>(Tt + p * T_PX * ROWB16 + i * ROWB16 + 8 * kb) = pl[p];
+      }
+    }
+    if (NBUF == 2 && t + 1 < t_end) store_tile(buf ^ 1);
+    __syncthreads();
+
+#pragma unroll
+    for (int gi = 0; gi < G1_PER_WAVE; ++gi) {
+      f32x4 acc = {0.f, 0.f, 0.f, 0.f}, accr = {0.f, 0.f, 0.f, 0.f};
+#pragma unroll
+      for (int s = 0; s < 5; ++s) {
+        const int off = a1[gi] + tofft[s];
+        bf16x8 tf[NP];
+#pragma unroll
+        for (int p = 0; p < NP; ++p) tf[p] = *reinterpret_cast<const bf16x8*>(Tt + p * T_PX * ROWB16 + off);
+#pragma unroll
+        for (int q = 0; q < AR::NPROD; ++q) acc = A16::mfma(w1f[s][AR::PB[q]], tf[AR::PA[q]], acc);
+      }
+      {
+        bf16x8 xf[NP];
+#pragma unroll
+        for (int p = 0; p < NP; ++p) xf[p] = *reinterpret_cast<const bf16x8*>(Ps + p * X_PX * ROWB16 + ar[gi]);
+#pragma unroll
+        for (int q = 0; q < AR::NPROD; ++q) accr = A16::mfma(wrf[AR::PB[q]], xf[AR::PA[q]], accr);
+      }
+      const int y = y0 + wave * G1_PER_WAVE + gi, x = x0 + n;
+      if (!OUTC) {
+        if (y < d.H && x < d.W) {
+          f32x4 v;
+#pragma unroll
+          for (int e = 0; e < 4; ++e) {
+            const float a = NP == 2 ? acc[e] * am1 : acc[e];
+            const float r = NP == 2 ? accr[e] * amr : accr[e];
+            v[e] = vs_relu(a + b1v[e]) + (r + brv[e]);
+          }
+          *reinterpret_cast<f32x4*>(d.out + (((int64_t)fb * d.H + y) * d.W + x) * d.out_ld + 4 * kb) = v;
+        }
+      } else {
+        f32x4 v;
+#pragma unroll
+        for (int e = 0; e < 4; ++e) {
+          const float a = NP == 2 ? acc[e] * am1 : acc[e];
+          const float r = NP == 2 ? accr[e] * amr : accr[e];
+          v[e] = vs_relu(a + b1v[e]) + (r + brv[e]);
+        }
+        float dot = 0.f;
+#pragma unroll
+        for (int k = 0; k < 4; ++k) {
+          f32x4 u;
+#pragma unroll
+          for (int e = 0; e < 4; ++e) u[e] = __shfl(v[e], n + 16 * k, 64);
+          const f32x4 wk = *reinterpret_cast<const f32x4*>(ocw + 4 * k);
+          const float wv[4] = {wk[0], wk[1], wk[2], wk[3]};
+          dot = vs_outc_mac4(dot, u, wv, 4);
+        }
+        if (y < d.H && x < d.W && kb < oc.out_ch)
+          oc.delta[(((int64_t)fb * oc.out_ch + kb) * d.H + y) * d.W + x] = vs_outc_act(dot, ocb, oc.use_tanh);
+      }
+    }
+    if (NBUF == 1) {
+      __syncthreads();
+      if (t + 1 < t_end) store_tile(0);
+    }
+    __syncthreads();
+    tx = ntx; ty = nty; fb = nfb;
+  }
diff --git a/videoseal_amd/csrc/upconv_fused.hip b/videoseal_amd/csrc/upconv_fused.hip
--- a/videoseal_amd/csrc/upconv_fused.hip
+++ b/videoseal_amd/csrc/upconv_fused.hip
@@ -2,6 +2,7 @@
 #include <cstdlib>
 
 #include "conv_common.h"
+#include "upconv_gather.h"
 
 namespace {
 
@@ -16,7 +17,7 @@
                                                            int C2, int64_t ld2, float sscale, const unsigned short* __restrict__ wsplit,
                                                            int H, int W, int Co, const float* __restrict__ lnw,
                                                            const float* __restrict__ lnb, float eps, int act, float* __restrict__ out,
-                                                           int64_t old, int tiles_x, int tiles_y, int nblk, int abl, float a_mul, float acc_mul) {
+                                                           int64_t old, int tiles_x, int tiles_y, int nblk, int abl, float a_mul, float acc_mul, int per_pixel) {
   using AR = Arith<NP>;
   constexpr int BN = NB * 32;
   constexpr int A_BYTES = NP * UROWS * ROWB;
@@ -144,11 +145,36 @@
   }
   const int H2 = 2 * H, W2 = 2 * W;
   const float invC = 1.0f / (float)Co;
-  for (int it = tid >> 2; it < ((abl & 2) ? 0 : 4 * UT * UT); it += 64) {
-    const int oy = it / (2 * UT), ox = it % (2 * UT);
-    const int Y = (y0 + 1) * 2 + oy, X = (x0 + 1) * 2 + ox;
-    const bool live = Y < H2 && X < W2;
-    const int Yc = min(Y, H2 - 1), Xc = min(X, W2 - 1);
+  auto ln_store = [&](const f32x4 (&v)[NV], const bool live, float* const orow) __attribute__((always_inline)) {
+#pragma clang fp contract(off)
+    float s = 0.f;
+#pragma unroll
+    for (int j = 0; j < NV; ++j) s += (v[j][0] + v[j][1]) + (v[j][2] + v[j][3]);
+    s += __shfl_xor(s, 1, 64);
+    s += __shfl_xor(s, 2, 64);
+    f32x4 dl[NV];
+    float var = 0.f;
+#pragma unroll
+    for (int j = 0; j < NV; ++j)
+#pragma unroll
+      for (int e = 0; e < 4; ++e) {
+        dl[j][e] = __builtin_fmaf(-s, invC, v[j][e]);
+        var = (j == 0 && e == 0) ? dl[j][e] * dl[j][e] : __builtin_fmaf(dl[j][e], dl[j][e], var);
+      }
+    var += __shfl_xor(var, 1, 64);
+    var += __shfl_xor(var, 2, 64);
+    const float den = sqrtf(__builtin_fmaf(var, invC, eps));
+    if (!live) return;
+#pragma unroll
+    for (int j = 0; j < NV; ++j) {
+      const f32x4 wv = lwv[j], bv = lbv[j];
+      f32x4 o;
+#pragma unroll
+      for (int e = 0; e < 4; ++e) o[e] = vs_apply_act(__builtin_fmaf(wv[e], dl[j][e] / den, bv[e]), act);
+      *reinterpret_cast<f32x4*>(orow + 4 * j) = o;
+    }
+  };
+  auto pixel = [&](const int Yc, const int Xc, const bool live) __attribute__((always_inline)) {
     int ys[3][2], xs[3][2];
     float wy[3][2], wx[3][2];
 #pragma unroll
@@ -179,32 +205,45 @@
             const float w = wy[ky][a] * wx[kx][c];
             const float* qz = zr + xs[kx][c] * ZS + kx * Co;
 #pragma unroll
-            for (int j = 0; j < NV; ++j) v[j] += w * *reinterpret_cast<const f32x4*>(qz + 4 * j);
+            for (int j = 0; j < NV; ++j) v[j] = vs_upconv_fma(w, *reinterpret_cast<const f32x4*>(qz + 4 * j), v[j]);
           }
       }
-    float s = 0.f;
-#pragma unroll
-    for (int j = 0; j < NV; ++j) s += (v[j][0] + v[j][1]) + (v[j][2] + v[j][3]);
-    s += __shfl_xor(s, 1, 64);
-    s += __shfl_xor(s, 2, 64);
-    const float mean = s * invC;
-    float var = 0.f;
-#pragma unroll
-    for (int j = 0; j < NV; ++j)
-#pragma unroll
-      for (int e = 0; e < 4; ++e) { const float dl = v[j][e] - mean; var += dl * dl; }
-    var += __shfl_xor(var, 1, 64);
-    var += __shfl_xor(var, 2, 64);
-    const float den = sqrtf(var * invC + eps);
-    if (!live) continue;
-    float* orow = out + (((int64_t)b * H2 + Y) * W2 + X) * old + q4 * CG;
-#pragma unroll
-    for (int j = 0; j < NV; ++j) {
-      const f32x4 wv = lwv[j], bv = lbv[j];
-      f32x4 o;
-#pragma unroll
-      for (int e = 0; e < 4; ++e) o[e] = vs_apply_act(wv[e] * ((v[j][e] - mean) / den) + bv[e], act);
-      *reinterpret_cast<f32x4*>(orow + 4 * j) = o;
+    ln_store(v, live, out + (((int64_t)b * H2 + Yc) * W2 + Xc) * old + q4 * CG);
+  };
+  if (abl & 2) return;
+  if (per_pixel) {
+    for (int it = tid >> 2; it < 4 * UT * UT; it += 64) {
+      const int Y = (y0 + 1) * 2 + it / (2 * UT), X = (x0 + 1) * 2 + it % (2 * UT);
+      pixel(min(Y, H2 - 1), min(X, W2 - 1), Y < H2 && X < W2);
+    }
+    return;
+  }
+  {
+    const int cy = tid >> 5, cx = (tid >> 2) & 7;
+    const int gi = y0 + 1 + cy, gj = x0 + 1 + cx;
+    if (gi >= 1 && gi <= H - 2 && gj >= 1 && gj <= W - 2) {
+      f32x4 acc[4][NV];
+#pragma unroll
+      for (int q = 0; q < 4; ++q)
+#pragma unroll
+        for (int j = 0; j < NV; ++j) acc[q][j] = f32x4{0.f, 0.f, 0.f, 0.f};
+      vs_upconv_gather_cell<NV, true, int>(Z + ((cy + 1) * UH + cx + 1) * ZS + q4 * CG, UH * ZS, ZS, Co, acc);
+      float* const o00 = out + (((int64_t)b * H2 + 2 * gi) * W2 + 2 * gj) * old + q4 * CG;
+#pragma unroll
+      for (int q = 0; q < 4; ++q) ln_store(acc[q], true, o00 + ((int64_t)(q >> 1) * W2 + (q & 1)) * old);
+    }
+  }
+  {
+    const int ry = y0 + 1 + (lane >> 3), rx = x0 + 1 + (lane & 7);
+    const unsigned long long mask = __ballot(ry < H && rx < W && (ry == 0 || ry == H - 1 || rx == 0 || rx == W - 1));
+    const int nrp = 4 * __popcll(mask);
+    for (int k0 = 0; k0 < nrp; k0 += 64) {
+      const int k = k0 + (tid >> 2);
+      const bool live = k < nrp;
+      unsigned long long m = mask;
+      for (int n = live ? k >> 2 : 0; n > 0; --n) m &= m - 1;
+      const int c = __ffsll(m) - 1;
+      pixel(2 * (y0 + 1 + (c >> 3)) + ((k >> 1) & 1), 2 * (x0 + 1 + (c & 7)) + (k & 1), live);
     }
   }
 }
@@ -227,7 +266,8 @@
   if (nblk >= (1 << 30)) return VS_ERR_UNSUPPORTED;
   static const int abl = [] { const char* e = getenv("VS_UPCONV_ABL"); return e ? atoi(e) : 0; }();
   hipLaunchKernelGGL(kern, dim3((unsigned)((nblk + 7) / 8 * 8)), dim3(256), smem, st, x, C1, ld1, skip, C2, ld2, s,
-                     static_cast<const unsigned short*>(wsplit), H, W, Co, lnw, lnb, eps, act, out, old, tiles_x, tiles_y, (int)nblk, abl, a_mul, acc_mul);
+                     static_cast<const unsigned short*>(wsplit), H, W, Co, lnw, lnb, eps, act, out, old, tiles_x, tiles_y, (int)nblk, abl, a_mul, acc_mul,
+                     vs_debug_get(VS_DBG_UPCONV_GATHER) == 1 ? 1 : 0);
   return vs_launch_status();
 }
 
diff --git a/videoseal_amd/csrc/upconv_gather.h b/videoseal_amd/csrc/upconv_gather.h
--- /dev/null
+++ b/videoseal_amd/csrc/upconv_gather.h
@@ -0,0 +1,51 @@
+#pragma once
+#include "vs_common.h"
+
+__device__ __forceinline__ f32x4 vs_upconv_fma(const float w, const f32x4 z, const f32x4 acc) {
+  return __builtin_elementwise_fma(f32x4{w, w, w, w}, z, acc);
+}
+
+template <int NV, bool PF, typename IT>
+__device__ __forceinline__ void vs_upconv_gather_cell(const float* __restrict__ zc, const IT rs, const IT cs, const int Co, f32x4 (&acc)[4][NV]) {
+  constexpr int RK[7] = {0, 0, 1, 1, 1, 2, 2}, RR[7] = {-1, 0, -1, 0, 1, 0, 1};
+  f32x4 zv[PF ? 2 : 1][3][3][NV];
+  auto load_row = [&](const int n, const int buf) __attribute__((always_inline)) {
+    const float* zr = zc + (IT)RR[n] * rs + RK[n] * 3 * Co;
+#pragma unroll
+    for (int kx = 0; kx < 3; ++kx)
+#pragma unroll
+      for (int cc = -1; cc <= 1; ++cc) {
+        if ((kx == 0 && cc == 1) || (kx == 2 && cc == -1)) continue;
+#pragma unroll
+        for (int j = 0; j < NV; ++j) zv[buf][kx][cc + 1][j] = *reinterpret_cast<const f32x4*>(zr + (IT)cc * cs + kx * Co + 4 * j);
+      }
+  };
+  if (PF) load_row(0, 0);
+#pragma unroll
+  for (int n = 0; n < 7; ++n) {
+    const int buf = PF ? n & 1 : 0;
+    if (PF) { if (n + 1 < 7) load_row(n + 1, buf ^ 1); }
+    else load_row(n, 0);
+    __builtin_amdgcn_sched_barrier(0);
+    const int ky = RK[n], r = RR[n];
+#pragma unroll
+    for (int kx = 0; kx < 3; ++kx)
+#pragma unroll
+      for (int py = 0; py < 2; ++py) {
+        const int ty = py + ky, a = r - ((ty >> 1) - 1);
+        if (a < 0 || a > 1) continue;
+        const float wya = ((ty & 1) != 0) == (a != 0) ? 0.75f : 0.25f;
+#pragma unroll
+        for (int px = 0; px < 2; ++px) {
+          const int tx = px + kx, c0 = (tx >> 1) - 1;
+#pragma unroll
+          for (int c = 0; c < 2; ++c) {
+            const float w = wya * (((tx & 1) != 0) == (c != 0) ? 0.75f : 0.25f);
+#pragma unroll
+            for (int j = 0; j < NV; ++j) acc[2 * py + px][j] = vs_upconv_fma(w, zv[buf][kx][c0 + c + 1][j], acc[2 * py + px][j]);
+          }
+        }
+      }
+    __builtin_amdgcn_sched_barrier(0);
+  }
+}
diff --git a/videoseal_amd/csrc/vs_common.h b/videoseal_amd/csrc/vs_common.h
--- a/videoseal_amd/csrc/vs_common.h
+++ b/videoseal_amd/csrc/vs_common.h
@@ -29,7 +29,7 @@
   return a;
 }
 
-enum { VS_DBG_RESIZE_FORM = 0 , VS_DBG_RESIZE_STRIP = 1 , VS_DBG_TAIL_STRIP = 2 , VS_DBG_JPEG_FORM = 3 , VS_DBG_CROP_RESIZE_FORM = 4 , VS_DBG_TO_PLANES_FORM = 5 , VS_DBG_DWCONV_ROWS = 6 , VS_DBG_LN_FORM = 7 , VS_DBG_SPLITK_EPI = 8 , VS_DBG_COUNT = 9 };
+enum { VS_DBG_RESIZE_FORM = 0 , VS_DBG_RESIZE_STRIP = 1 , VS_DBG_TAIL_STRIP = 2 , VS_DBG_JPEG_FORM = 3 , VS_DBG_CROP_RESIZE_FORM = 4 , VS_DBG_TO_PLANES_FORM = 5 , VS_DBG_DWCONV_ROWS = 6 , VS_DBG_LN_FORM = 7 , VS_DBG_SPLITK_EPI = 8 , VS_DBG_UPCONV_GATHER = 9 , VS_DBG_COUNT = 10 };
 int vs_debug_get(int key);
 
 static inline int vs_max_lds_bytes() {
@@ -105,6 +105,18 @@
   }
 }
 
+__device__ __forceinline__ float vs_outc_mac4(float acc, const f32x4 v, const float* __restrict__ wr, const int nch) {
+  acc = __builtin_fmaf(v[0], wr[0], acc);
+  if (nch > 1) acc = __builtin_fmaf(v[1], wr[1], acc);
+  if (nch > 2) acc = __builtin_fmaf(v[2], wr[2], acc);
+  if (nch > 3) acc = __builtin_fmaf(v[3], wr[3], acc);
+  return acc;
+}
+__device__ __forceinline__ float vs_outc_act(const float acc, const float bias, const int use_tanh) {
+  const float v = acc + bias;
+  return use_tanh ? tanhf(v) : v;
+}
+
 __device__ __forceinline__ float wave_sum(float v) {
 #pragma unroll
   for (int o = 32; o > 0; o >>= 1) v += __shfl_xor(v, o, 64);
diff --git a/videoseal_amd/engine.py b/videoseal_amd/engine.py
--- a/videoseal_amd/engine.py
+++ b/videoseal_amd/engine.py
@@ -756,17 +756,39 @@
         return (x.ld <= k and p["c0"].CinP == k and p["c1"].CinP == k and p["res"].CinP == k and (out is None or out.ld == c) and
                 (c == 16 or self.arith == 2) and bool(self.lib.vs_resblock_thin_supported(x.ld, c, c)))
 
-    def resblock_thin(self, x: Act, p, tag: str, out: Optional[Act] = None) -> Act:
+    def _thin_desc(self, x: Act, p) -> "N.ResblockThinDesc":
         ar, c = self.arith, p["cout"]
         c0, c1, cr = p["c0"].with_split(ar), p["c1"].with_split(ar), p["res"].with_split(ar)
-        if out is None:
-            out = self.new_act(tag + ".o", x.B, x.H, x.W, c)
         d = N.ResblockThinDesc()
         d.x, d.x_ld, d.B, d.H, d.W, d.Cin = N.ptr(x.t), x.ld, x.B, x.H, x.W, x.ld
         d.w0_split, d.w1_split, d.wr_split = N.ptr(c0.split), N.ptr(c1.split), N.ptr(cr.split)
         d.b0, d.b1, d.br = N.ptr(c0.bias), N.ptr(c1.bias), N.ptr(cr.bias)
         d.arith, d.Cout, d.a_mul = ar, c, A_MUL
         d.acc_mul0, d.acc_mul1, d.acc_mulr = 1.0 / (A_MUL * c0.w_mul), 1.0 / (A_MUL * c1.w_mul), 1.0 / (A_MUL * cr.w_mul)
+        return d
+
+    def _thin_outc_ok(self, x: Act, p, out_ch: int) -> bool:
+        return self._thin_ok(x, p, None) and bool(self.lib.vs_resblock_thin_outc_supported(x.ld, p["cout"], p["cout"], out_ch))
+
+    def resblock_thin_outc(self, x: Act, p, outc_w: torch.Tensor, outc_b: torch.Tensor, out_ch: int, use_tanh: bool, delta: torch.Tensor) -> None:
+        d = self._thin_desc(x, p)
+        c = p["cout"]
+        timed = self.kernel_timers is not None and self.time_all_convs and not torch.cuda.is_current_stream_capturing()
+        if timed:
+            ev0, ev1 = torch.cuda.Event(enable_timing=True), torch.cuda.Event(enable_timing=True)
+            ev0.record()
+        N.check(self.lib.vs_resblock_thin_outc(C.byref(d), N.ptr(outc_w), N.ptr(outc_b), out_ch, 1 if use_tanh else 0, N.ptr(delta), N.stream()),
+                "vs_resblock_thin_outc")
+        if timed:
+            ev1.record()
+            self.kernel_timers.append((f"resblock_thin+outc {x.C}->{c}->{c}->{out_ch} @{x.H}x{x.W}", ev0, ev1,
+                                       2.0 * x.rows * c * (2 * 9 * c + c + out_ch)))
+
+    def resblock_thin(self, x: Act, p, tag: str, out: Optional[Act] = None) -> Act:
+        c = p["cout"]
+        d = self._thin_desc(x, p)
+        if out is None:
+            out = self.new_act(tag + ".o", x.B, x.H, x.W, c)
         d.out, d.out_ld = N.ptr(out.t), out.ld
         timed = self.kernel_timers is not None and self.time_all_convs and not torch.cuda.is_current_stream_capturing()
         if timed:
@@ -992,6 +1014,10 @@
                 ln = self.new_act(f"up{k}.ln", B, cat.H, cat.W, up["conv"].N)
                 self.layernorm(cv, up["lnw"], up["lnb"], ln, act=up_act)
             lc = lowres_cat(k + 1, ln)
+            if k == nlev - 1 and lc is None and not bn_train and not rms and self._thin_outc_ok(ln, up["rb"], c.out_ch):
+                delta = self.buf("delta", B * c.out_ch * ln.H * ln.W)
+                self.resblock_thin_outc(ln, up["rb"], E["outc_w"], E["outc_b"], c.out_ch, c.last_tanh, delta)
+                return delta.view(B, c.out_ch, ln.H, ln.W)
             xcur = self.resblock(ln, up["rb"], f"up{k}", out=(Act(lc.t, B, lc.H, lc.W, up["rb"]["cout"], lc.ld) if lc else None))
         delta = self.buf("delta", B * c.out_ch * xcur.H * xcur.W)
         N.check(L.vs_outc_tanh(N.ptr(xcur.t), xcur.H * xcur.W, B, xcur.C, xcur.ld, N.ptr(E["outc_w"]), N.ptr(E["outc_b"]), c.out_ch,
diff --git a/videoseal_amd/native.py b/videoseal_amd/native.py
--- a/videoseal_amd/native.py
+++ b/videoseal_amd/native.py
@@ -29,7 +29,7 @@
     "vs_resize_nchw_bwd", "vs_embed_tail_bwd", "vs_tail_key_reduce", "vs_aug_crop_flip_bwd", "vs_mask_mul", "vs_aug_color_bwd_scratch_floats",
     "vs_aug_color_bwd", "vs_clamp01_bwd", "vs_nhwc_to_nchw_scaled", "vs_percep_partial_doubles", "vs_percep_mse", "vs_percep_mse_grad",
     "vs_ssim_partial_doubles", "vs_ssim_stats", "vs_ssim_grad", "vs_avgpool2_pad", "vs_jnd_loss_partial_doubles", "vs_jnd_loss", "vs_jnd_loss_grad",
-    "vs_split_block", "vs_check_finite", "vs_absmax", "vs_resblock_thin", "vs_resblock_thin_supported", "vs_cnx_block_supported", "vs_cnx_block_image_bytes", "vs_cnx_block",
+    "vs_split_block", "vs_check_finite", "vs_absmax", "vs_resblock_thin", "vs_resblock_thin_supported", "vs_resblock_thin_outc", "vs_resblock_thin_outc_supported", "vs_cnx_block_supported", "vs_cnx_block_image_bytes", "vs_cnx_block",
 ]
 
 
@@ -200,6 +200,8 @@
         "vs_absmax": [P, I64, P, P],
         "vs_resblock_thin": [P, P],
         "vs_resblock_thin_supported": [I, I, I],
+        "vs_resblock_thin_outc": [P, P, P, I, I, P, P],
+        "vs_resblock_thin_outc_supported": [I, I, I, I],
         "vs_cnx_block": [P, P, I, I64, I, I, F, F, P, I64, P, P, I64, P, I64, P, P],
         "vs_cnx_block_supported": [I, I64, I],
     }
```

After: 4128 frames/s (median of 6 runs). +1.3%, better.
